# aalobaidi/ggRMCP

Measured on NVIDIA H100. Metric: tools_call_transcodes_per_sec, higher is better.
Workload: dtype u8

## Files before the change

__graft_entry__.py:

```python
import os
import subprocess
import sys

ROOT = os.path.dirname(os.path.abspath(__file__))
for p in (ROOT, os.path.join(ROOT, "tests")):
    if p not in sys.path:
        sys.path.insert(0, p)


def build():
    from ggrmcp_b200 import build as gbuild
    gbuild.build()
    subprocess.check_call(["make", "-s", "-C", os.path.join(ROOT, "oracle")])
    import benchgen
    benchgen.build()
    subprocess.check_call(["make", "-s", "-C", os.path.join(ROOT, "tests", "hostsim")])
    import ggrmcp_b200


def smoke():
    import numpy as np
    import cases
    import orc
    import ggrmcp_b200
    from ggrmcp_b200.engine import pack, unpack
    import benchgen

    fds = open(os.path.join(ROOT, "tests", "golden", "schemas.binpb"), "rb").read()
    eng = ggrmcp_b200.Engine(0)
    sch = eng.register(fds)
    O = orc.Schema(fds)
    ids = np.array([sch.message(n) for n, _, _ in cases.K_REQUESTS], np.int32)
    data, off = pack([j for _, j, _ in cases.K_REQUESTS])
    out, ooff, st = eng.encode_batch(sch, ids, data, off)
    assert list(st) == [0] * len(ids), st
    assert [o.hex() for o in unpack(out, ooff)] == [w for _, _, w in cases.K_REQUESTS]
    ids = np.array([sch.message(n) for n, _, _ in cases.K_REPLIES], np.int32)
    data, off = pack([bytes.fromhex(w) for _, w, _ in cases.K_REPLIES])
    out, ooff, st = eng.decode_batch(sch, ids, data, off)
    assert list(st) == [0] * len(ids), st
    assert unpack(out, ooff) == [j for _, _, j in cases.K_REPLIES]
    wl = benchgen.nested(512, sch.message)
    wire, woff, st = eng.encode_batch(sch, wl.req_msg, wl.req_json, wl.req_off)
    js, joff, st2 = eng.decode_batch(sch, wl.rep_msg, wl.rep_wire, wl.rep_off)
    assert (st == 0).all() and (st2 == 0).all()
    names = {sch.message(n): O.msg(n) for n in ("com.example.complex.ProcessNodeRequest", "com.example.complex.CreateDocumentRequest",
                                                 "com.example.complex.Node", "com.example.complex.GetUserProfileResponse")}
    ow, owoff, _ = O.encode_batch(np.array([names[int(i)] for i in wl.req_msg], np.int32), wl.req_json, wl.req_off)
    oj, ojoff, _ = O.decode_batch(np.array([names[int(i)] for i in wl.rep_msg], np.int32), wl.rep_wire, wl.rep_off)
    assert wire.tobytes() == ow.tobytes() and (woff == owoff).all()
    assert js.tobytes() == oj.tobytes() and (joff == ojoff).all()
    print("smoke ok: %d kernel launches, %d + %d items bit-exact vs oracle" % (eng.launch_count(), len(cases.K_REQUESTS) + len(cases.K_REPLIES), 2 * wl.n))
    eng.close()


if __name__ == "__main__":
    build()
    if "--smoke" in sys.argv:
        smoke()
```

ggrmcp_b200/csrc/ggr_engine.cu:

```cuda
#include <cuda_runtime.h>
#include <sched.h>

#include <cstdio>
#include <cstdlib>
#include <cstring>
#include <atomic>
#include <chrono>
#include <mutex>
#include <string>
#include <vector>

#include "../../include/ggrmcp_b200.h"
#include "ggr_kernels.h"
#include "ggr_schema.h"
#include "ggr_tables.h"

typedef uint8_t u8;
typedef uint32_t u32;
typedef uint64_t u64;
typedef int32_t i32;
#define GGR_BLOCK 128

__global__ void __launch_bounds__(1024) k_scan_blocks(u64* __restrict__ sums, long long nb, u64* __restrict__ total_out) {
  __shared__ u64 part[1024];
// ... 305 lines not shown
  int n = 0;
  for (int c : e->node_cpus)
    if (c < CPU_SETSIZE && CPU_ISSET(c, &old)) {
      CPU_SET(c, &want);
      n++;
    }
  if (n) sched_setaffinity(0, sizeof want, &want);
  return GGR_SUCCESS;
}
int ggr_host_alloc(ggr_engine* e, size_t bytes, void** out) {
  if (!e || !out) return GGR_ERR_INVALID_ARGUMENT;
  *out = nullptr;
  DeviceGuard dg(e->device);
  NodeBind nb(e);
  void* p = nullptr;
  if (!cuda_ok(e, cudaHostAlloc(&p, bytes ? bytes : 1, cudaHostAllocDefault), "cudaHostAlloc")) return GGR_ERR_CUDA;
  for (size_t o = 0; o < bytes; o += 4096) ((volatile char*)p)[o] = 0;
  *out = p;
  return GGR_SUCCESS;
}
void ggr_host_free(ggr_engine* e, void* p) {
  if (!e || !p) return;
  DeviceGuard dg(e->device);
  cudaFreeHost(p);
}

const char* ggr_status_string(int32_t st) {
  static const char* names[] = {"ok", "syntax", "unknown_field", "invalid_value", "range", "invalid_utf8", "duplicate",
                                "oneof_conflict", "depth", "too_large", "bad_wire", "unsupported", "no_space", "internal"};
  if (st < 0 || st > 13) return "?";
  return names[st];
}

int ggr_engine_create(const ggr_config* cfg, ggr_engine** out) {
  if (!out) return GGR_ERR_INVALID_ARGUMENT;
  *out = nullptr;
  int ndev = 0;
  if (cudaGetDeviceCount(&ndev) != cudaSuccess || ndev == 0) return GGR_ERR_NO_DEVICE;
  int dev = cfg ? cfg->device : 0;
  if (dev < 0 || dev >= ndev) return GGR_ERR_INVALID_ARGUMENT;
  if (cudaSetDevice(dev) != cudaSuccess) return GGR_ERR_NO_DEVICE;
  cudaFuncAttributes fa;
  if (cudaFuncGetAttributes(&fa, ggr_kernel_encode_parse()) != cudaSuccess) {
    cudaGetLastError();
    return GGR_ERR_NO_DEVICE;
  }
  ggr_engine* e = new ggr_engine();
  e->device = dev;
  cudaDeviceGetAttribute(&e->sm_count, cudaDevAttrMultiProcessorCount, dev);
  if (e->sm_count <= 0) e->sm_count = 132;
  find_numa(e);
  if (const char* nc = getenv("GGR_COOP")) e->use_coop = nc[0] != '0';
  if (const char* nc = getenv("GGR_COOP_ENC")) e->use_coop_enc = nc[0] != '0';
  if (const char* nc = getenv("GGR_WALK")) e->use_walk = nc[0] != '0';
  if (const char* pz = getenv("GGR_POISON")) e->poison = pz[0] == '1';
  if (const char* nc = getenv("GGR_TRACE")) e->trace = nc[0] != '0';
  if (const char* nc = getenv("GGR_LOCKSTEP_MIN_BYTES")) e->min_json = e->min_wire = (uint32_t)strtoul(nc, nullptr, 10);
  if (const char* nc = getenv("GGR_SPREAD_MIN_BYTES")) e->spread_min = (uint32_t)strtoul(nc, nullptr, 10);
  if (const char* nc = getenv("GGR_SLOTS")) {
    int v = atoi(nc);
    if (v >= 1 && v <= GGR_MAX_SLOTS) e->n_slots = v;
  }
  if (const char* nc = getenv("GGR_CHUNK_ITEMS")) {
    long long v = atoll(nc);
    if (v >= 128) e->chunk_items = v;
  }
  if (const char* nc = getenv("GGR_CHUNK_RAMP")) e->chunk_ramp = nc[0] != '0';
  e->blocking_sync = usable_cpus() < 4 * ndev;
  if (const char* nc = getenv("GGR_BLOCKING_SYNC")) e->blocking_sync = nc[0] != '0';
  if (const char* nc = getenv("GGR_CHUNK_BYTES")) {
    long long v = atoll(nc);
    if (v >= (1 << 16)) e->chunk_bytes = (uint64_t)v;
  }
  e->order = (cfg && cfg->wire_order == GGR_ORDER_GO_LEGACY) ? ggr::ORDER_GO_LEGACY : ggr::ORDER_FIELD_NUMBER;
  e->short_names = cfg && cfg->tool_naming == GGR_NAMES_DESCRIPTOR_SET;
  if (ggr_encode_coop_init() != 0 || ggr_encode_walk_init() != 0 || ggr_decode_coop_init() != 0) {
    cudaGetLastError();
    delete e;
    return GGR_ERR_CUDA;
  }
  if (cudaStreamCreateWithFlags(&e->stream, cudaStreamNonBlocking) != cudaSuccess) {
    delete e;
    return GGR_ERR_CUDA;
  }
  {
    size_t want = 4096 + (size_t)(ggr_decode_max_rec() + 1) * 4096, cur = 0;
    if (const char* ev = getenv("GGR_STACK_BYTES")) want = (size_t)strtoull(ev, nullptr, 10);
    cudaDeviceGetLimit(&cur, cudaLimitStackSize);
    if (cur < want) {
      cudaError_t rc = cudaDeviceSetLimit(cudaLimitStackSize, want);
      if (rc != cudaSuccess) {
        e->err = std::string("cudaDeviceSetLimit(stack): ") + cudaGetErrorString(rc);
        cudaStreamDestroy(e->stream);
        delete e;
        return GGR_ERR_CUDA;
      }
    }
    if (getenv("GGR_DEBUG")) {
      size_t now = 0;
      cudaDeviceGetLimit(&now, cudaLimitStackSize);
      fprintf(stderr, "[ggr] stack limit was %zu, wanted %zu, now %zu\n", cur, want, now);
    }
  }
  *out = e;
  return GGR_SUCCESS;
}

void ggr_engine_destroy(ggr_engine* e) {
  if (!e) return;
  cudaSetDevice(e->device);
  cudaStreamSynchronize(e->stream);
  auto free_scratch = [](Scratch& sc) {
    DevBuf* bufs[] = {&sc.ir, &sc.size, &sc.aux, &sc.sums, &sc.pend, &sc.ioff, &sc.nn, &sc.wtext, &sc.woff, &sc.wsize, &sc.sortpool, &sc.spread, &sc.tabpool, &sc.taboff};
    for (DevBuf* b : bufs)
      if (b->p) cudaFree(b->p);
  };
  free_scratch(e->dev_sc[0]);
  free_scratch(e->dev_sc[1]);

  for (int i = 0; i < 2 * GGR_MAX_SLOTS; i++) {
    Slot& sl = e->slots[i / GGR_MAX_SLOTS][i % GGR_MAX_SLOTS];
    if (sl.st) cudaStreamSynchronize(sl.st);
    free_scratch(sl.sc);
    DevBuf* bufs[] = {&sl.d_in, &sl.d_off, &sl.d_msg, &sl.d_out, &sl.d_out_off, &sl.d_status, &sl.d_ids, &sl.d_ids_off};
    for (DevBuf* b : bufs)
      if (b->p) cudaFree(b->p);
    if (sl.h_total) cudaFreeHost(sl.h_total);
    if (sl.ready) cudaEventDestroy(sl.ready);
    if (sl.ev_in) cudaEventDestroy(sl.ev_in);
    if (sl.ev_k) cudaEventDestroy(sl.ev_k);
    if (sl.ev_out) cudaEventDestroy(sl.ev_out);
    if (sl.st) cudaStreamDestroy(sl.st);
  }
  for (int d = 0; d < 2; d++) {
    if (e->s_in[d]) cudaStreamDestroy(e->s_in[d]);
    if (e->s_out[d]) cudaStreamDestroy(e->s_out[d]);
  }
  for (cudaEvent_t ev : e->ev_pool) cudaEventDestroy(ev);
  cudaStreamDestroy(e->stream);
  delete e;
}

const char* ggr_last_error(const ggr_engine* e) { return e ? e->err.c_str() : "null engine"; }
uint64_t ggr_launch_count(const ggr_engine* e) { return e ? e->launches.load() : 0; }

int ggr_schema_register(ggr_engine* e, const uint8_t* fds, size_t n, ggr_schema** out) {
  if (!e || !fds || !out) return GGR_ERR_INVALID_ARGUMENT;
  *out = nullptr;
  ggr_schema* s = new ggr_schema();
  s->eng = e;
  s->d_blob = nullptr;
  std::string err;
  if (!ggr::compile_schema(fds, n, e->order, &s->cs, &err, e->short_names)) {
    e->err = err;
    delete s;
    return GGR_ERR_SCHEMA;
  }
  cudaSetDevice(e->device);
  if (!cuda_ok(e, cudaMalloc((void**)&s->d_blob, s->cs.blob.size() + 256), "cudaMalloc(schema)") ||
      !cuda_ok(e, cudaMemset(s->d_blob, 0, s->cs.blob.size() + 256), "cudaMemset(schema)") ||
      !cuda_ok(e, cudaMemcpy(s->d_blob, s->cs.blob.data(), s->cs.blob.size(), cudaMemcpyHostToDevice), "cudaMemcpy(schema)")) {
    if (s->d_blob) cudaFree(s->d_blob);
    delete s;
    return GGR_ERR_CUDA;
  }
  *out = s;
  return GGR_SUCCESS;
}
void ggr_schema_release(ggr_schema* s) {
  if (!s) return;
  cudaSetDevice(s->eng->device);
  cudaStreamSynchronize(s->eng->stream);
  cudaFree(s->d_blob);
  delete s;
}
int32_t ggr_message_lookup(const ggr_schema* s, const char* full_name) {
  if (!s || !full_name) return -1;
  auto it = s->cs.msg_index.find(full_name);
  return it == s->cs.msg_index.end() ? -1 : it->second;
}
int32_t ggr_method_count(const ggr_schema* s) { return s ? (int32_t)s->cs.methods.size() : 0; }
int ggr_method_get(const ggr_schema* s, int32_t i, ggr_method_info* o) {
  if (!s || !o || i < 0 || i >= (int32_t)s->cs.methods.size()) return GGR_ERR_INVALID_ARGUMENT;
  const ggr::MethodInfo& m = s->cs.methods[i];
  o->name = m.name.c_str();
  o->full_name = m.full_name.c_str();
  o->service_name = m.service_name.c_str();
  o->tool_name = m.tool_name.c_str();
  o->grpc_path = m.grpc_path.c_str();
  o->input_msg = m.input_msg;
  o->output_msg = m.output_msg;
  o->client_streaming = m.client_streaming;
  o->server_streaming = m.server_streaming;
  return GGR_SUCCESS;
}
int32_t ggr_tool_lookup(const ggr_schema* s, const char* tool) {
  if (!s || !tool) return -1;
  auto it = s->cs.tool_index.find(tool);
  return it == s->cs.tool_index.end() ? -1 : it->second;
}

int ggr_profile_enable(ggr_engine* e, int on) {
  if (!e) return GGR_ERR_INVALID_ARGUMENT;
  std::lock_guard<std::mutex> g(e->mu);
  e->profiling = on != 0;
  return GGR_SUCCESS;
}
int ggr_profile_read(ggr_engine* e, double* ms, uint64_t* launches) {
  if (!e || !ms || !launches) return GGR_ERR_INVALID_ARGUMENT;
  std::lock_guard<std::mutex> g(e->mu);
  cudaSetDevice(e->device);
  cudaDeviceSynchronize();
  for (int i = 0; i < GGR_PROFILE_SLOTS; i++) { ms[i] = 0; launches[i] = 0; }
  for (auto& sp : e->spans) {
    float t = 0;
    if (cudaEventElapsedTime(&t, e->ev_pool[sp.a], e->ev_pool[sp.b]) == cudaSuccess) {
      ms[sp.slot] += t;
      launches[sp.slot]++;
    }
  }
  e->spans.clear();
  e->ev_used = 0;
  return GGR_SUCCESS;
}

int ggr_debug_paths(ggr_engine* e, int64_t n, uint32_t* reply_mode, uint32_t* request_counts) {
  if (!e) return GGR_ERR_INVALID_ARGUMENT;
  DeviceGuard dg(e->device);
  cudaDeviceSynchronize();
  if (reply_mode && e->dev_sc[1].aux.p && e->dev_sc[1].aux.cap >= (size_t)n * 4)
    cudaMemcpy(reply_mode, e->dev_sc[1].aux.p, (size_t)n * 4, cudaMemcpyDeviceToHost);
  if (request_counts && e->dev_sc[0].pend.p) {
    uint32_t c[16];
    cudaMemcpy(c, e->dev_sc[0].pend.p, sizeof c, cudaMemcpyDeviceToHost);
    request_counts[0] = c[0];
    request_counts[1] = c[4];
    request_counts[2] = c[8];
  }
  return GGR_SUCCESS;
}

int ggr_synchronize(ggr_engine* e) {
  if (!e) return GGR_ERR_INVALID_ARGUMENT;
  cudaSetDevice(e->device);
  return cuda_ok(e, cudaStreamSynchronize(e->stream), "cudaStreamSynchronize") ? GGR_SUCCESS : GGR_ERR_CUDA;
}

static int run_dev_kernels(ggr_engine* e, const ggr_schema* s, Scratch& sc, bool encode, int64_t n, const int32_t* msg_id, const uint8_t* in,
                           const uint64_t* in_off, uint64_t in_bytes, uint8_t* out, uint64_t out_cap, uint64_t* out_off,
                           int32_t* status, uint32_t flags, cudaStream_t st);
static int run_dev(ggr_engine* e, const ggr_schema* s, Scratch& sc, bool encode, int64_t n, const int32_t* msg_id, const uint8_t* in,
                   const uint64_t* in_off, uint64_t in_bytes, uint8_t* out, uint64_t out_cap, uint64_t* out_off,
                   int32_t* status, uint32_t flags, cudaStream_t st) {
  const int rc = run_dev_kernels(e, s, sc, encode, n, msg_id, in, in_off, in_bytes, out, out_cap, out_off, status, flags, st);
  if (e && e->poison) {
    DevBuf* bufs[] = {&sc.ir, &sc.size, &sc.aux, &sc.sums, &sc.pend, &sc.ioff, &sc.nn};
    for (DevBuf* b : bufs) {
      const size_t n16 = b->cap / 16;
      if (b->p && n16) k_poison<<<(unsigned)((n16 + 255) / 256), 256, 0, st>>>((uint4*)b->p, n16);
    }
  }
  return rc;
}
static int run_dev_kernels(ggr_engine* e, const ggr_schema* s, Scratch& sc, bool encode, int64_t n, const int32_t* msg_id, const uint8_t* in,
                           const uint64_t* in_off, uint64_t in_bytes, uint8_t* out, uint64_t out_cap, uint64_t* out_off,
                           int32_t* status, uint32_t flags, cudaStream_t st) {
  if (!e || !s || n < 0 || (n > 0 && (!msg_id || !in || !in_off || !out_off || !status))) return GGR_ERR_INVALID_ARGUMENT;
  if (((uintptr_t)in & 15) || ((uintptr_t)out & 7)) return GGR_ERR_INVALID_ARGUMENT;
  DeviceGuard dg(e->device);
  if (n == 0) {
    return cuda_ok(e, cudaMemsetAsync(out_off, 0, sizeof(uint64_t), st), "memset") ? GGR_SUCCESS : GGR_ERR_CUDA;
  }
  long long nb = (n + GGR_BLOCK - 1) / GGR_BLOCK;
  if (!ensure(e, sc.size, (size_t)n * 4) || !ensure(e, sc.aux, (size_t)n * 4) || !ensure(e, sc.sums, (size_t)nb * 8)) return GGR_ERR_CUDA;
  if (encode && !ensure(e, sc.ir, (size_t)in_bytes * 8 + (size_t)n * 128 + 256)) return GGR_ERR_CUDA;
  u32 n_msgs = (u32)s->cs.msg_names.size();
  const bool prof = e->profiling && e->ev_used + 16 <= 65536;
  const u32 frame = (encode && (flags & GGR_F_GRPC_FRAME)) ? 5u : 0u;
  size_t m0 = 0, m1 = 0, m2 = 0, m3 = 0, mx = 0;
  bool have_mx = false;
  if (prof) prof_mark(e, st, &m0);
  if (encode) {
    if (e->use_coop_enc) {
      if (!ensure(e, sc.pend, (size_t)n * 20 + 128) || !ensure(e, sc.ioff, (size_t)in_bytes * 2 + (size_t)n * 32 + 64) ||
          !ensure(e, sc.nn, (size_t)n * 4))
        return GGR_ERR_CUDA;
      u32* counters = (u32*)sc.pend.p;
      u32* big = counters + 32;
      u32* pend1 = big + n;
      u32* pend2 = pend1 + n;
      u32* pend1b = pend2 + n;
      u32* pend1c = pend1b + n;
      size_t c0 = 0, c1 = 0;
      if (!cuda_ok(e, cudaMemsetAsync(counters, 0, 128, st), "memset") ||
          !cuda_ok(e, cudaMemsetAsync(sc.nn.p, 0, (size_t)n * 4, st), "memset"))
        return GGR_ERR_CUDA;
      if (prof) prof_mark(e, st, &m0);
      k_route<<<(unsigned)((n + 255) / 256), 256, 0, st>>>(n, in_off, e->min_json, 65000u - 16u, big, counters, pend2, counters + 8, nullptr);
      size_t t1 = 0, t_tok = 0;
      if (e->use_walk) {
        ggr_launch_encode_tok2(st, n, in, in_off, (u8*)sc.ir.p, big, counters, e->sm_count);
        if (prof) prof_mark(e, st, &t1);
        t_tok = t1;
        ggr_launch_encode_place(st, n, in_off, (u8*)sc.ir.p, big, counters, e->sm_count);
        size_t t2 = 0, t3 = 0;
        if (prof) prof_mark(e, st, &t2);
        ggr_launch_encode_type(st, 0, n, s->d_blob, n_msgs, msg_id, in, in_off, (u8*)sc.ir.p, (u32*)sc.size.p, (u32*)sc.aux.p, status,
                               (u32*)sc.ioff.p, (u32*)sc.nn.p, big, counters, pend1b, counters + 12, e->sm_count);
        ggr_launch_encode_type(st, 1, n, s->d_blob, n_msgs, msg_id, in, in_off, (u8*)sc.ir.p, (u32*)sc.size.p, (u32*)sc.aux.p, status,
                               (u32*)sc.ioff.p, (u32*)sc.nn.p, pend1b, counters + 12, pend1c, counters + 16, e->sm_count);
        ggr_launch_encode_type(st, 2, n, s->d_blob, n_msgs, msg_id, in, in_off, (u8*)sc.ir.p, (u32*)sc.size.p, (u32*)sc.aux.p, status,
                               (u32*)sc.ioff.p, (u32*)sc.nn.p, pend1c, counters + 16, pend1, counters + 4, e->sm_count);
        if (prof) {
          prof_mark(e, st, &t3);
          e->spans.push_back({12, t1, t2});
          e->spans.push_back({13, t2, t3});
          t1 = t3;
        }
      } else {
        ggr_launch_encode_coop_tok(st, n, in, in_off, (u8*)sc.ir.p, big, counters, e->sm_count);
        if (prof) prof_mark(e, st, &t1);
        t_tok = t1;
        ggr_launch_encode_coop_parse(st, 0, n, s->d_blob, n_msgs, msg_id, in, in_off, (u8*)sc.ir.p, (u32*)sc.size.p,
                                     (u32*)sc.aux.p, status, (u32*)sc.ioff.p, (u32*)sc.nn.p, big, counters, pend1, counters + 4, e->sm_count, nullptr, nullptr, -1);
      }
      ggr_launch_encode_coop_parse(st, 1, n, s->d_blob, n_msgs, msg_id, in, in_off, (u8*)sc.ir.p, (u32*)sc.size.p,
                                   (u32*)sc.aux.p, status, (u32*)sc.ioff.p, (u32*)sc.nn.p, pend1, counters + 4, pend2, counters + 8, e->sm_count, nullptr, nullptr, -1);
      if (prof) prof_mark(e, st, &c0);
      if (e->spread_min) {
        size_t max_big = (size_t)(in_bytes / e->spread_min) + 1;
        if (max_big > GGR_SPREAD_CAP) max_big = GGR_SPREAD_CAP;
        if (!ensure(e, sc.spread, (max_big * 32 + (size_t)n) * 4 + 64)) return GGR_ERR_CUDA;
        u32* sp_cnt = (u32*)sc.spread.p;
        u32* sp_list = sp_cnt + 16;
        u32* sp_small = sp_list + max_big * 32;
        if (!cuda_ok(e, cudaMemsetAsync(sp_cnt, 0, 64, st), "memset") || !cuda_ok(e, cudaMemsetAsync(sp_list, 0xFF, max_big * 32 * 4, st), "memset"))
          return GGR_ERR_CUDA;
        for (int phase = 0; phase < 2; phase++)
          k_spread<<<(unsigned)((n + 255) / 256), 256, 0, st>>>(phase, n, in_off, e->spread_min, pend2, counters + 8, nullptr, sp_small, sp_list, sp_cnt, (u32)max_big);
        ggr_launch_encode_parse(st, (unsigned)((max_big * 32 + GGR_BLOCK - 1) / GGR_BLOCK), s->d_blob, n, n_msgs, msg_id, in, in_off, (u8*)sc.ir.p,
                                (u32*)sc.size.p, (u32*)sc.aux.p, status, (u64*)sc.sums.p, sp_list, sp_cnt);
        ggr_launch_encode_parse(st, (unsigned)nb, s->d_blob, n, n_msgs, msg_id, in, in_off, (u8*)sc.ir.p, (u32*)sc.size.p,
                                (u32*)sc.aux.p, status, (u64*)sc.sums.p, sp_small, sp_cnt + 1);
        e->launches += 3;
      } else {
        ggr_launch_encode_parse(st, (unsigned)nb, s->d_blob, n, n_msgs, msg_id, in, in_off, (u8*)sc.ir.p, (u32*)sc.size.p,
                                (u32*)sc.aux.p, status, (u64*)sc.sums.p, pend2, counters + 8);
      }
      if (prof) prof_mark(e, st, &c1);
      if (frame) ggr_launch_frame_sizes(st, n, (u32*)sc.size.p, status);
      ggr_launch_block_sums(st, (unsigned)nb, n, (const u32*)sc.size.p, (u64*)sc.sums.p);
      if (prof) {
        e->spans.push_back({11, m0, t_tok});
        e->spans.push_back({8, t1, c0});
        e->spans.push_back({0, c0, c1});
        prof_mark(e, st, &m1);
        e->spans.push_back({9, c1, m1});
      }
      e->launches += e->use_walk ? 8 : 5;
    } else {
      ggr_launch_encode_parse(st, (unsigned)nb, s->d_blob, n, n_msgs, msg_id, in, in_off, (u8*)sc.ir.p, (u32*)sc.size.p,
                              (u32*)sc.aux.p, status, (u64*)sc.sums.p, nullptr, nullptr);
      if (frame) {
        ggr_launch_frame_sizes(st, n, (u32*)sc.size.p, status);
        ggr_launch_block_sums(st, (unsigned)nb, n, (const u32*)sc.size.p, (u64*)sc.sums.p);
      }
      if (prof) prof_mark(e, st, &m1);
    }
    k_scan_blocks<<<1, 1024, 0, st>>>((u64*)sc.sums.p, nb, out_off + n);
    if (prof) prof_mark(e, st, &m2);
    ggr_launch_encode_emit(st, (unsigned)nb, n, in, in_off, (const u8*)sc.ir.p, (const u32*)sc.size.p,
                           (const u32*)sc.aux.p, status, (const u64*)sc.sums.p, out, out_cap, out_off,
                           e->use_coop_enc ? (const u32*)sc.nn.p : nullptr, frame);
    if (e->use_coop_enc) {
      size_t x1 = 0;
      if (prof) {
        prof_mark(e, st, &mx);
        have_mx = true;
      }
      ggr_launch_encode_coop_emit(st, n, in, in_off, (const u8*)sc.ir.p, (const u32*)sc.ioff.p, (const u32*)sc.nn.p,
                                  (const u32*)sc.size.p, status, out, out_off, e->sm_count, (const u32*)sc.pend.p + 32,
                                  (const u32*)sc.pend.p, frame);
      if (prof) {
        prof_mark(e, st, &x1);
        e->spans.push_back({10, mx, x1});
      }
      e->launches += 1;
    }
  } else {
    const bool coop = e->use_coop;
    size_t c0 = 0, c1 = 0;
    const uint64_t want_recs = in_bytes / 4 * 3 + 1024;
    const uint32_t sort_cap = (uint32_t)(want_recs > 0x3FFFFFFFull ? 0x3FFFFFFFull : want_recs);
    if (!ensure(e, sc.sortpool, (size_t)sort_cap * 16 + 16)) return GGR_ERR_CUDA;
    if (!cuda_ok(e, cudaMemsetAsync(sc.sortpool.p, 0, 16, st), "memset")) return GGR_ERR_CUDA;
    if (coop) {
      const uint64_t want_ent = in_bytes / 2 + 4096;
      const uint32_t pool_cap = (uint32_t)(want_ent > (4ull << 20) ? (4ull << 20) : want_ent);
      if (!ensure(e, sc.ir, ggr_decode_coop_table_bytes(n)) || !ensure(e, sc.nn, (size_t)n * 4) ||
          !ensure(e, sc.pend, (size_t)n * 8 + 64) || !ensure(e, sc.tabpool, (size_t)pool_cap * 32 + 32) || !ensure(e, sc.taboff, (size_t)n * 4))
        return GGR_ERR_CUDA;
      u32* counters = (u32*)sc.pend.p;
      u32* big = counters + 16;
      if (!cuda_ok(e, cudaMemsetAsync(counters, 0, 64, st), "memset") || !cuda_ok(e, cudaMemsetAsync(sc.tabpool.p, 0, 32, st), "memset")) return GGR_ERR_CUDA;
      k_route<<<(unsigned)((n + 255) / 256), 256, 0, st>>>(n, in_off, e->min_wire, 0x3FFFFF00u, big, counters, nullptr, nullptr, (u32*)sc.aux.p);
      ggr_launch_decode_coop_size(st, n, s->d_blob, n_msgs, msg_id, in, in_off, flags, (u32*)sc.size.p, (u32*)sc.aux.p, status,
                                  sc.ir.p, (u32*)sc.nn.p, e->sm_count, big, counters, big + n, counters + 4, sc.tabpool.p, pool_cap, (u32*)sc.taboff.p);
      if (prof) {
        prof_mark(e, st, &c0);
        e->spans.push_back({6, m0, c0});
        m0 = c0;
      }
    }
    const bool spread = coop && e->spread_min != 0;
    size_t max_big = spread ? (size_t)(in_bytes / e->spread_min) + 1 : 0;
    if (max_big > GGR_SPREAD_CAP) max_big = GGR_SPREAD_CAP;
    u32* sp_cnt = nullptr;
    if (spread) {
      if (!ensure(e, sc.spread, max_big * 32 * 4 + 64)) return GGR_ERR_CUDA;
      sp_cnt = (u32*)sc.spread.p;
      if (!cuda_ok(e, cudaMemsetAsync(sp_cnt, 0, 64, st), "memset") || !cuda_ok(e, cudaMemsetAsync(sp_cnt + 16, 0xFF, max_big * 32 * 4, st), "memset"))
        return GGR_ERR_CUDA;
      for (int phase = 0; phase < 2; phase++)
        k_spread<<<(unsigned)((n + 255) / 256), 256, 0, st>>>(phase, n, in_off, e->spread_min, nullptr, nullptr, (const u32*)sc.aux.p, nullptr, sp_cnt + 16, sp_cnt, (u32)max_big);
      ggr_launch_decode_size(st, (unsigned)((max_big * 32 + GGR_BLOCK - 1) / GGR_BLOCK), s->d_blob, n, n_msgs, msg_id, in, in_off, flags,
                             (u32*)sc.size.p, (u32*)sc.aux.p, status, (u64*)sc.sums.p, 1, sc.sortpool.p, sort_cap, sp_cnt + 16, sp_cnt);
      e->launches += 4;
    }
    ggr_launch_decode_size(st, (unsigned)nb, s->d_blob, n, n_msgs, msg_id, in, in_off, flags, (u32*)sc.size.p,
                           (u32*)sc.aux.p, status, (u64*)sc.sums.p, coop ? 1 : 0, sc.sortpool.p, sort_cap);
    if (prof) prof_mark(e, st, &m1);
    k_scan_blocks<<<1, 1024, 0, st>>>((u64*)sc.sums.p, nb, out_off + n);
    if (prof) prof_mark(e, st, &m2);
    ggr_launch_decode_write(st, (unsigned)nb, s->d_blob, n, msg_id, in, in_off, flags, (const u32*)sc.size.p,
                            (const u32*)sc.aux.p, status, (const u64*)sc.sums.p, out, out_cap, out_off, sc.sortpool.p, sort_cap);
    if (spread)
      ggr_launch_decode_write(st, (unsigned)((max_big * 32 + GGR_BLOCK - 1) / GGR_BLOCK), s->d_blob, n, msg_id, in, in_off, flags,
                              (const u32*)sc.size.p, (const u32*)sc.aux.p, status, (const u64*)sc.sums.p, out, out_cap, out_off, sc.sortpool.p,
                              sort_cap, sp_cnt + 16, sp_cnt);
    if (coop) {
      if (prof) prof_mark(e, st, &c1);
      ggr_launch_decode_coop_write(st, n, s->d_blob, in, in_off, flags, (const u32*)sc.size.p, (const u32*)sc.aux.p, status, sc.ir.p,
                                   (const u32*)sc.nn.p, out, out_off, e->sm_count, (const u32*)sc.pend.p + 16, (const u32*)sc.pend.p, sc.tabpool.p,
                                   (const u32*)sc.taboff.p);
      if (prof) {
        prof_mark(e, st, &m3);
        e->spans.push_back({3, m0, m1});
        e->spans.push_back({4, m1, m2});
        e->spans.push_back({5, m2, c1});
        e->spans.push_back({7, c1, m3});
      }
      e->launches += 7;
      return cuda_ok(e, cudaGetLastError(), "kernel launch") ? GGR_SUCCESS : GGR_ERR_CUDA;
    }
  }
  if (prof) {
    prof_mark(e, st, &m3);
    int base = encode ? 0 : 3;
    if (!(encode && e->use_coop_enc)) e->spans.push_back({base + 0, m0, m1});
    e->spans.push_back({base + 1, m1, m2});
    e->spans.push_back({base + 2, m2, have_mx ? mx : m3});
  }
  e->launches += 3;
  return cuda_ok(e, cudaGetLastError(), "kernel launch") ? GGR_SUCCESS : GGR_ERR_CUDA;
}

int ggr_encode_diagnose(ggr_engine* e, const ggr_schema* s, int32_t msg_id, const uint8_t* json, uint64_t json_len, uint32_t flags,
                        int32_t* status, uint32_t* err_pos, uint32_t* err_len, char* text, size_t text_cap) {
  (void)flags;
  if (!e || !s || (!json && json_len) || !status) return GGR_ERR_INVALID_ARGUMENT;
  if (json_len > 0x1FFFF0ull) return GGR_ERR_TOO_LARGE;
  std::lock_guard<std::mutex> g(e->mu);
  DeviceGuard dg(e->device);
  const size_t in_cap = ((size_t)json_len + 15) / 16 * 16 + 64;
  const size_t ir_bytes = (size_t)json_len * 8 + 128 + 256;
  const size_t o_off = in_cap, o_msg = o_off + 16, o_res = o_msg + 16, o_sums = o_res + 16, o_ir = o_sums + 16;
  uint8_t* d = nullptr;
  if (!cuda_ok(e, cudaMalloc((void**)&d, o_ir + ir_bytes), "cudaMalloc(diagnose)")) return GGR_ERR_CUDA;
  std::vector<uint8_t> h(o_ir, 0);
  if (json_len) memcpy(h.data(), json, (size_t)json_len);
  const uint64_t offs[2] = {0, json_len};
  memcpy(h.data() + o_off, offs, 16);
  memcpy(h.data() + o_msg, &msg_id, 4);
  cudaStream_t st = e->stream;
  int rc = GGR_SUCCESS;
  uint32_t res[4] = {0, 0, 0, 0};
  if (!cuda_ok(e, cudaMemcpyAsync(d, h.data(), o_ir, cudaMemcpyHostToDevice, st), "H2D(diagnose)")) rc = GGR_ERR_CUDA;
  if (rc == GGR_SUCCESS) {
    ggr_launch_encode_parse(st, 1, s->d_blob, 1, (u32)s->cs.msg_names.size(), (const int32_t*)(d + o_msg), d, (const uint64_t*)(d + o_off), d + o_ir,
                            (u32*)(d + o_res), (u32*)(d + o_res + 4), (int32_t*)(d + o_res + 8), (uint64_t*)(d + o_sums), nullptr, nullptr,
                            (u32*)(d + o_res + 12));
    e->launches += 1;
    if (!cuda_ok(e, cudaGetLastError(), "kernel launch") ||
        !cuda_ok(e, cudaMemcpyAsync(res, d + o_res, 16, cudaMemcpyDeviceToHost, st), "D2H(diagnose)") ||
        !cuda_ok(e, cudaStreamSynchronize(st), "sync(diagnose)"))
      rc = GGR_ERR_CUDA;
  }
  cudaFree(d);
  if (rc != GGR_SUCCESS) return rc;
  const int32_t stt = (int32_t)res[2];
  *status = stt;
  uint32_t pos = stt != GGR_ST_OK ? res[3] : 0, len = 0;
  if (pos > json_len) pos = (uint32_t)json_len;
  if (stt != GGR_ST_OK && pos < json_len && json[pos] == '"') {
    uint64_t q = pos + 1;
    while (q < json_len && json[q] != '"') q += json[q] == '\\' ? 2 : 1;
    if (q < json_len) len = (uint32_t)(q + 1 - pos);
  }
  if (err_pos) *err_pos = pos;
  if (err_len) *err_len = len;
  if (text && text_cap) {
    std::string t;
    if (stt == GGR_ST_OK) {
      t = "";
    } else {
      uint32_t line = 1, col = 1;
      for (uint32_t k = 0; k < pos; k++) {
        if (json[k] == '\n') { line++; col = 1; }
        else col++;
      }
      t = "proto: (line " + std::to_string(line) + ":" + std::to_string(col) + "): ";
      const std::string tok = len ? std::string((const char*)json + pos, len) : std::string();
      if (stt == GGR_ST_UNKNOWN_FIELD && len) t += "unknown field " + tok;
      else if (stt == GGR_ST_DUPLICATE && len) t += "duplicate field " + tok;
      else if (stt == GGR_ST_ONEOF && len) t += "error parsing " + tok + ", oneof is already set";
      else t += ggr_status_string(stt);
    }
    const size_t k = t.size() < text_cap - 1 ? t.size() : text_cap - 1;
    memcpy(text, t.data(), k);
    text[k] = 0;
  }
  return GGR_SUCCESS;
}

int ggr_encode_batch_dev(ggr_engine* e, const ggr_schema* s, int64_t n, const int32_t* msg_id, const uint8_t* in,
                         const uint64_t* in_off, uint64_t in_bytes, uint8_t* out, uint64_t out_cap, uint64_t* out_off,
                         int32_t* status, uint32_t flags, void* stream) {
  if (!e) return GGR_ERR_INVALID_ARGUMENT;
  std::lock_guard<std::mutex> g(e->mu);
  return run_dev(e, s, e->dev_sc[0], true, n, msg_id, in, in_off, in_bytes, out, out_cap, out_off, status, flags,
                 stream ? (cudaStream_t)stream : e->stream);
}
int ggr_decode_batch_dev(ggr_engine* e, const ggr_schema* s, int64_t n, const int32_t* msg_id, const uint8_t* in,
                         const uint64_t* in_off, uint64_t in_bytes, uint8_t* out, uint64_t out_cap, uint64_t* out_off,
                         int32_t* status, uint32_t flags, void* stream) {
  if (!e) return GGR_ERR_INVALID_ARGUMENT;
  std::lock_guard<std::mutex> g(e->mu);
  return run_dev(e, s, e->dev_sc[1], false, n, msg_id, in, in_off, in_bytes, out, out_cap, out_off, status, flags,
                 stream ? (cudaStream_t)stream : e->stream);
}

static int run_request_dev(ggr_engine* e, const ggr_schema* s, Scratch& sc, int64_t n, const uint8_t* in, const uint64_t* in_off,
                           uint64_t in_bytes, uint8_t* out, uint64_t out_cap, uint64_t* out_off, int32_t* method, uint32_t* id_span,
                           int32_t* status, cudaStream_t st) {
  if (!e || !s || n < 0 || (n > 0 && (!in || !in_off || !out_off || !status || !method || !id_span))) return GGR_ERR_INVALID_ARGUMENT;
  if (((uintptr_t)in & 15) || ((uintptr_t)out & 7)) return GGR_ERR_INVALID_ARGUMENT;
  DeviceGuard dg(e->device);
  if (n == 0) return cuda_ok(e, cudaMemsetAsync(out_off, 0, sizeof(uint64_t), st), "memset") ? GGR_SUCCESS : GGR_ERR_CUDA;
  const long long nb = (n + GGR_BLOCK - 1) / GGR_BLOCK;
  if (!ensure(e, sc.size, (size_t)n * 4) || !ensure(e, sc.aux, (size_t)n * 4) || !ensure(e, sc.sums, (size_t)nb * 8) ||
      !ensure(e, sc.ir, (size_t)in_bytes * 8 + (size_t)n * 128 + 256) || !ensure(e, sc.pend, (size_t)n * 12 + 64) ||
      !ensure(e, sc.ioff, (size_t)in_bytes * 2 + (size_t)n * 32 + 64) || !ensure(e, sc.nn, (size_t)n * 4))
    return GGR_ERR_CUDA;
  u32* counters = (u32*)sc.pend.p;
  u32* big = counters + 16;
  u32* pend1 = big + n;
  u32* rest = pend1 + n;
  if (!cuda_ok(e, cudaMemsetAsync(counters, 0, 64, st), "memset") || !cuda_ok(e, cudaMemsetAsync(sc.nn.p, 0, (size_t)n * 4, st), "memset"))
    return GGR_ERR_CUDA;
  const u32 n_msgs = (u32)s->cs.msg_names.size();
  k_route<<<(unsigned)((n + 255) / 256), 256, 0, st>>>(n, in_off, 0u, 65000u - 16u, big, counters, rest, counters + 8, nullptr);
  ggr_launch_encode_coop_tok(st, n, in, in_off, (u8*)sc.ir.p, big, counters, e->sm_count);
  ggr_launch_encode_coop_parse(st, 0, n, s->d_blob, n_msgs, nullptr, in, in_off, (u8*)sc.ir.p, (u32*)sc.size.p, (u32*)sc.aux.p, status,
                               (u32*)sc.ioff.p, (u32*)sc.nn.p, big, counters, pend1, counters + 4, e->sm_count, method, id_span, -1);
  ggr_launch_encode_coop_parse(st, 1, n, s->d_blob, n_msgs, nullptr, in, in_off, (u8*)sc.ir.p, (u32*)sc.size.p, (u32*)sc.aux.p, status,
                               (u32*)sc.ioff.p, (u32*)sc.nn.p, pend1, counters + 4, rest, counters + 8, e->sm_count, method, id_span,
                               GGR_ST_UNSUPPORTED);
  k_mark<<<(unsigned)((n + 255) / 256), 256, 0, st>>>(rest, counters + 8, status, (u32*)sc.size.p, (u32*)sc.aux.p, GGR_ST_UNSUPPORTED);
  ggr_launch_block_sums(st, (unsigned)nb, n, (const u32*)sc.size.p, (u64*)sc.sums.p);
  k_scan_blocks<<<1, 1024, 0, st>>>((u64*)sc.sums.p, nb, out_off + n);
  ggr_launch_encode_emit(st, (unsigned)nb, n, in, in_off, (const u8*)sc.ir.p, (const u32*)sc.size.p, (const u32*)sc.aux.p, status,
                         (const u64*)sc.sums.p, out, out_cap, out_off, (const u32*)sc.nn.p, 0);
  ggr_launch_encode_coop_emit(st, n, in, in_off, (const u8*)sc.ir.p, (const u32*)sc.ioff.p, (const u32*)sc.nn.p, (const u32*)sc.size.p,
                              status, out, out_off, e->sm_count, big, counters, 0);
  e->launches += 9;
  return cuda_ok(e, cudaGetLastError(), "kernel launch") ? GGR_SUCCESS : GGR_ERR_CUDA;
}

static int run_wrap_dev(ggr_engine* e, const ggr_schema* s, Scratch& sc, int64_t n, const int32_t* msg_id, const uint8_t* in,
                        const uint64_t* in_off, uint64_t in_bytes, const uint8_t* ids, const uint64_t* ids_off, uint8_t* out,
                        uint64_t out_cap, uint64_t* out_off, int32_t* status, uint32_t flags, cudaStream_t st) {
  if (n > 0 && (!ids || !ids_off)) return GGR_ERR_INVALID_ARGUMENT;
  if (n == 0) return run_dev(e, s, sc, false, n, msg_id, in, in_off, in_bytes, out, out_cap, out_off, status, flags, st);
  if (!ensure(e, sc.wtext, (size_t)out_cap + 64) || !ensure(e, sc.woff, (size_t)(n + 1) * 8) || !ensure(e, sc.wsize, (size_t)n * 4))
    return GGR_ERR_CUDA;
  int rc = run_dev(e, s, sc, false, n, msg_id, in, in_off, in_bytes, (uint8_t*)sc.wtext.p, out_cap, (uint64_t*)sc.woff.p, status, flags, st);
  if (rc != GGR_SUCCESS) return rc;
  const long long nb = (n + GGR_BLOCK - 1) / GGR_BLOCK;
  ggr_launch_wrap_size(st, n, (const uint8_t*)sc.wtext.p, (const uint64_t*)sc.woff.p, status, ids_off, (u32*)sc.wsize.p, e->sm_count);
  ggr_launch_block_sums(st, (unsigned)nb, n, (const u32*)sc.wsize.p, (u64*)sc.sums.p);
  k_scan_blocks<<<1, 1024, 0, st>>>((u64*)sc.sums.p, nb, out_off + n);
  ggr_launch_offsets(st, (unsigned)nb, n, (const u32*)sc.wsize.p, (const u64*)sc.sums.p, out_off);
  ggr_launch_wrap_write(st, n, (const uint8_t*)sc.wtext.p, (const uint64_t*)sc.woff.p, status, ids, ids_off, (const u32*)sc.wsize.p, out,
                        out_cap, out_off, e->sm_count);
  e->launches += 5;
  return cuda_ok(e, cudaGetLastError(), "kernel launch") ? GGR_SUCCESS : GGR_ERR_CUDA;
}
// ... 323 lines not shown
```

ggrmcp_b200/csrc/ggr_kernels.h:

```cpp
#pragma once
#include <cuda_runtime.h>
#include <stdint.h>

void ggr_launch_encode_parse(cudaStream_t st, unsigned nb, const uint8_t* blob, long long n, uint32_t n_msgs, const int32_t* msg_id,
                             const uint8_t* in, const uint64_t* in_off, uint8_t* ir, uint32_t* size, uint32_t* first,
                             int32_t* status, uint64_t* block_sums, const uint32_t* list, const uint32_t* list_n,
                             uint32_t* err_pos = nullptr);
void ggr_launch_block_sums(cudaStream_t st, unsigned nb, long long n, const uint32_t* size, uint64_t* block_sums);
void ggr_launch_encode_coop_tok(cudaStream_t st, long long n, const uint8_t* in, const uint64_t* in_off, uint8_t* ir,
                                const uint32_t* list, const uint32_t* list_n, int sm_count);
void ggr_launch_encode_coop_parse(cudaStream_t st, int tier, long long n, const uint8_t* blob, uint32_t n_msgs,
                                  const int32_t* msg_id, const uint8_t* in, const uint64_t* in_off, uint8_t* ir, uint32_t* size,
                                  uint32_t* first, int32_t* status, uint32_t* ioff, uint32_t* nnodes, const uint32_t* list,
                                  const uint32_t* list_n, uint32_t* pending, uint32_t* n_pending, int sm_count, int32_t* method,
                                  uint32_t* id_span, int32_t final_status);
void ggr_launch_encode_coop_emit(cudaStream_t st, long long n, const uint8_t* in, const uint64_t* in_off, const uint8_t* ir,
                                 const uint32_t* ioff, const uint32_t* nnodes, const uint32_t* size, const int32_t* status,
                                 uint8_t* out, const uint64_t* out_off, int sm_count, const uint32_t* list,
                                 const uint32_t* list_n, uint32_t frame);
void ggr_launch_encode_tok2(cudaStream_t st, long long n, const uint8_t* in, const uint64_t* in_off, uint8_t* ir, const uint32_t* list,
                            const uint32_t* list_n, int sm_count);
void ggr_launch_encode_place(cudaStream_t st, long long n, const uint64_t* in_off, uint8_t* ir, const uint32_t* list, const uint32_t* list_n,
                             int sm_count);
void ggr_launch_encode_type(cudaStream_t st, int tier, long long n, const uint8_t* blob, uint32_t n_msgs, const int32_t* msg_id, const uint8_t* in,
                            const uint64_t* in_off, uint8_t* ir, uint32_t* size, uint32_t* first, int32_t* status, uint32_t* ioff,
                            uint32_t* nnodes, const uint32_t* list, const uint32_t* list_n, uint32_t* pending, uint32_t* n_pending,
                            int sm_count);
int ggr_encode_walk_init();
int ggr_encode_coop_init();
void ggr_launch_encode_emit(cudaStream_t st, unsigned nb, long long n, const uint8_t* in, const uint64_t* in_off, const uint8_t* ir,
                            const uint32_t* size, const uint32_t* first, int32_t* status, const uint64_t* block_prefix,
                            uint8_t* out, uint64_t out_cap, uint64_t* out_off, const uint32_t* skip, uint32_t frame);
void ggr_launch_frame_sizes(cudaStream_t st, long long n, uint32_t* size, const int32_t* status);
void ggr_launch_decode_size(cudaStream_t st, unsigned nb, const uint8_t* blob, long long n, uint32_t n_msgs, const int32_t* msg_id,
                            const uint8_t* in, const uint64_t* in_off, uint32_t flags, uint32_t* size, uint32_t* mode,
                            int32_t* status, uint64_t* block_sums, int after_coop, void* sort_pool, uint32_t sort_cap,
                            const uint32_t* list = nullptr, const uint32_t* list_n = nullptr);
void ggr_launch_decode_write(cudaStream_t st, unsigned nb, const uint8_t* blob, long long n, const int32_t* msg_id,
                             const uint8_t* in, const uint64_t* in_off, uint32_t flags, const uint32_t* size,
                             const uint32_t* mode, int32_t* status, const uint64_t* block_prefix, uint8_t* out,
                             uint64_t out_cap, uint64_t* out_off, void* sort_pool, uint32_t sort_cap, const uint32_t* list = nullptr,
                             const uint32_t* list_n = nullptr);
void ggr_launch_decode_coop_size(cudaStream_t st, long long n, const uint8_t* blob, uint32_t n_msgs, const int32_t* msg_id,
                                 const uint8_t* in, const uint64_t* in_off, uint32_t flags, uint32_t* size, uint32_t* mode,
                                 int32_t* status, void* tab, uint32_t* nent, int sm_count, const uint32_t* list,
                                 const uint32_t* list_n, uint32_t* pending, uint32_t* n_pending, void* pool, uint32_t pool_cap,
                                 uint32_t* tab_off);
void ggr_launch_decode_coop_write(cudaStream_t st, long long n, const uint8_t* blob, const uint8_t* in, const uint64_t* in_off,
                                  uint32_t flags, const uint32_t* size, const uint32_t* mode, int32_t* status, const void* tab,
                                  const uint32_t* nent, uint8_t* out, const uint64_t* out_off, int sm_count,
                                  const uint32_t* list, const uint32_t* list_n, const void* pool, const uint32_t* tab_off);
size_t ggr_decode_coop_table_bytes(long long n);
int ggr_decode_coop_init();
void ggr_launch_wrap_size(cudaStream_t st, long long n, const uint8_t* text, const uint64_t* text_off, const int32_t* status,
                          const uint64_t* ids_off, uint32_t* size, int sm_count);
void ggr_launch_offsets(cudaStream_t st, unsigned nb, long long n, const uint32_t* size, const uint64_t* block_prefix,
                        uint64_t* out_off);
void ggr_launch_wrap_write(cudaStream_t st, long long n, const uint8_t* text, const uint64_t* text_off, int32_t* status,
                           const uint8_t* ids, const uint64_t* ids_off, const uint32_t* size, uint8_t* out, uint64_t out_cap,
                           const uint64_t* out_off, int sm_count);
const void* ggr_kernel_encode_parse();
int ggr_decode_max_rec();
```

ggrmcp_b200/csrc/ggr_kernels_walk.cu:

```cuda
#include "ggr_kernels.h"
#include "ggr_walk.cuh"

#define CW_WARPS 4
#define CW_TOK_BLOCKS 8
#define CW_PLACE_BLOCKS 12
#define CW_WALK_BLOCKS 6

__global__ void __launch_bounds__(CW_WARPS * 32, CW_TOK_BLOCKS)
k_encode_tok3(const u8* __restrict__ in, const u64* __restrict__ in_off, u8* __restrict__ ir, const u32* __restrict__ list,
              const u32* __restrict__ list_n) {
  __shared__ CwLut lut;
  __shared__ CwTile tiles[CW_WARPS];
  const u32 warp = threadIdx.x >> 5;
  cw_lut_init(lut, threadIdx.x, CW_WARPS * 32);
  if ((threadIdx.x & 31u) == 0) cw_tile_init(&tiles[warp]);
  __syncthreads();
  u32 ph = 0;
  const long long total = (long long)*list_n;
  const u64 a0 = in_off[0];
  u32* ticket = const_cast<u32*>(list_n) + 1;
  u32 drawn = wp_ticket_draw(ticket);
  for (long long slot = wp_ticket_take(drawn); slot < total; slot = wp_ticket_take(drawn)) {
    drawn = wp_ticket_draw(ticket);
    const long long item = (long long)list[slot];
    const u64 a = in_off[item], b = in_off[item + 1];
    if (b < a || b - a > (u64)CE_MAX_INPUT - 16u) continue;
    const u64 node_off = ((a - a0) >> 1) + 8ull * (u64)item;
    const u32 cap = (u32)((((b - a0) >> 1) + 8ull * (u64)(item + 1)) - node_off);
    const u32 s0 = (u32)(a & 15ull);
    cw_tok_item(&tiles[warp], ph, lut, in + (a & ~15ull), s0, s0 + (u32)(b - a), ir + node_off * 16, cap);
  }
}

__global__ void __launch_bounds__(CW_WARPS * 32, CW_PLACE_BLOCKS)
k_encode_place(const u64* __restrict__ in_off, u8* __restrict__ ir, const u32* __restrict__ list, const u32* __restrict__ list_n) {
  __shared__ CwPlaceSh S[CW_WARPS];
  const u32 warp = threadIdx.x >> 5;
  const long long total = (long long)*list_n;
  const u64 a0 = in_off[0];
  u32* ticket = const_cast<u32*>(list_n) + 3;
  u32 drawn = wp_ticket_draw(ticket);
  for (long long slot = wp_ticket_take(drawn); slot < total; slot = wp_ticket_take(drawn)) {
    drawn = wp_ticket_draw(ticket);
    const long long item = (long long)list[slot];
    const u64 a = in_off[item], b = in_off[item + 1];
    if (b <= a || b - a > (u64)CE_MAX_INPUT - 16u) continue;
    const u64 node_off = ((a - a0) >> 1) + 8ull * (u64)item;
    const u32 cap = (u32)((((b - a0) >> 1) + 8ull * (u64)(item + 1)) - node_off);
    cw_place_item(S[warp], ir + node_off * 16, cap, CoopWalkHuge::MAX_NODE);
  }
}

template <class SH, bool FULL, int WARPS>
__global__ void __launch_bounds__(WARPS * 32, FULL ? 1 : CW_WALK_BLOCKS)
k_encode_type(const u8* __restrict__ blob, u32 n_msgs, const i32* __restrict__ msg_id, const u8* __restrict__ in,
              const u64* __restrict__ in_off, u8* __restrict__ ir, u32* __restrict__ size, u32* __restrict__ first,
              i32* __restrict__ status, u32* __restrict__ ioff, u32* __restrict__ nnodes, const u32* __restrict__ list,
              const u32* __restrict__ list_n, u32* __restrict__ pending, u32* __restrict__ n_pending) {
  extern __shared__ __align__(16) unsigned char smem[];
  SH* S = reinterpret_cast<SH*>(smem);
  const u32 warp = threadIdx.x >> 5, lane = threadIdx.x & 31;
  const long long total = (long long)*list_n;
  const Tables T = ggr_tables(blob);
  const u64 a0 = in_off[0];
  u32* ticket = const_cast<u32*>(list_n) + 2;
  u32 drawn = wp_ticket_draw(ticket);
  long long slot = wp_ticket_take(drawn);
  drawn = wp_ticket_draw(ticket);
  while (slot < total) {
    const long long next = wp_ticket_take(drawn);
    drawn = wp_ticket_draw(ticket);
    const long long item = (long long)list[slot];
    const u64 a = in_off[item], b = in_off[item + 1];
    const i32 m = msg_id[item];
    bool ok = false;
    EncResult res;
    res.size = 0;
    res.n_nodes = 0;
    res.method = 0;
    if (m >= 0 && (u32)m < n_msgs && b >= a && b - a <= (u64)CE_MAX_INPUT - 16u) {
      const u64 node_off = ((a - a0) >> 1) + 8ull * (u64)item;
      const u32 cap = (u32)((((b - a0) >> 1) + 8ull * (u64)(item + 1)) - node_off);
      const u32 s0 = (u32)(a & 15ull);
      ok = cw_type_item<SH, FULL>(S[warp], T, (u32)m, in + (a & ~15ull), s0, s0 + (u32)(b - a), ir + node_off * 16, ioff + node_off, cap, &res);
    }
    if (lane == 0) {
      if (ok) {
        size[item] = res.size;
        first[item] = GGR_NIL;
        status[item] = GST_OK;
        nnodes[item] = res.n_nodes | (res.method << 16);
      } else {
        size[item] = 0;
        nnodes[item] = 0;
        first[item] = GGR_NIL;
        pending[atomicAdd(n_pending, 1u)] = (u32)item;
      }
    }
    slot = next;
  }
}

int ggr_encode_walk_init() {
  return (cudaFuncSetAttribute(k_encode_type<CoopWalk, false, CW_WARPS>, cudaFuncAttributeMaxDynamicSharedMemorySize, (int)(sizeof(CoopWalk) * CW_WARPS)) == cudaSuccess &&
          cudaFuncSetAttribute(k_encode_type<CoopWalkBig, true, CW_WARPS>, cudaFuncAttributeMaxDynamicSharedMemorySize, (int)(sizeof(CoopWalkBig) * CW_WARPS)) == cudaSuccess &&
          cudaFuncSetAttribute(k_encode_type<CoopWalkHuge, true, 1>, cudaFuncAttributeMaxDynamicSharedMemorySize, (int)sizeof(CoopWalkHuge)) == cudaSuccess)
             ? 0
             : -1;
}

static unsigned cw_grid(const void* fn, int threads, size_t smem, long long n, int sm_count) {
  int per_sm = 0;
  if (cudaOccupancyMaxActiveBlocksPerMultiprocessor(&per_sm, fn, threads, smem) != cudaSuccess || per_sm < 1) per_sm = 1;
  const long long want = (n + CW_WARPS - 1) / CW_WARPS, cap = (long long)sm_count * per_sm;
  return (unsigned)(want < cap ? (want > 0 ? want : 1) : cap);
}

void ggr_launch_encode_tok2(cudaStream_t st, long long n, const uint8_t* in, const uint64_t* in_off, uint8_t* ir, const uint32_t* list,
                            const uint32_t* list_n, int sm_count) {
  static unsigned per_sm = 0;
  if (!per_sm) per_sm = cw_grid((const void*)k_encode_tok3, CW_WARPS * 32, 0, 1ll << 40, 1);
  const long long want = (n + CW_WARPS - 1) / CW_WARPS, cap = (long long)sm_count * per_sm;
  k_encode_tok3<<<(unsigned)(want < cap ? want : cap), CW_WARPS * 32, 0, st>>>(in, (const u64*)in_off, ir, list, list_n);
}

void ggr_launch_encode_place(cudaStream_t st, long long n, const uint64_t* in_off, uint8_t* ir, const uint32_t* list, const uint32_t* list_n,
                             int sm_count) {
  static unsigned per_sm = 0;
  if (!per_sm) per_sm = cw_grid((const void*)k_encode_place, CW_WARPS * 32, 0, 1ll << 40, 1);
  const long long want = (n + CW_WARPS - 1) / CW_WARPS, cap = (long long)sm_count * per_sm;
  k_encode_place<<<(unsigned)(want < cap ? want : cap), CW_WARPS * 32, 0, st>>>((const u64*)in_off, ir, list, list_n);
}

void ggr_launch_encode_type(cudaStream_t st, int tier, long long n, const uint8_t* blob, uint32_t n_msgs, const int32_t* msg_id, const uint8_t* in,
                            const uint64_t* in_off, uint8_t* ir, uint32_t* size, uint32_t* first, int32_t* status, uint32_t* ioff,
                            uint32_t* nnodes, const uint32_t* list, const uint32_t* list_n, uint32_t* pending, uint32_t* n_pending,
                            int sm_count) {
  if (tier == 0) {
    static unsigned per_sm = 0;
    const size_t smem = sizeof(CoopWalk) * CW_WARPS;
    if (!per_sm) per_sm = cw_grid((const void*)k_encode_type<CoopWalk, false, CW_WARPS>, CW_WARPS * 32, smem, 1ll << 40, 1);
    const long long want = (n + CW_WARPS - 1) / CW_WARPS, cap = (long long)sm_count * per_sm;
    k_encode_type<CoopWalk, false, CW_WARPS><<<(unsigned)(want < cap ? want : cap), CW_WARPS * 32, smem, st>>>(
        blob, n_msgs, msg_id, in, (const u64*)in_off, ir, size, first, status, ioff, nnodes, list, list_n, pending, n_pending);
  } else if (tier == 2) {
    k_encode_type<CoopWalkHuge, true, 1><<<(unsigned)sm_count, 32, sizeof(CoopWalkHuge), st>>>(
        blob, n_msgs, msg_id, in, (const u64*)in_off, ir, size, first, status, ioff, nnodes, list, list_n, pending, n_pending);
  } else {
    static unsigned per_sm = 0;
    const size_t smem = sizeof(CoopWalkBig) * CW_WARPS;
    if (!per_sm) per_sm = cw_grid((const void*)k_encode_type<CoopWalkBig, true, CW_WARPS>, CW_WARPS * 32, smem, 1ll << 40, 1);
    k_encode_type<CoopWalkBig, true, CW_WARPS><<<(unsigned)sm_count * per_sm, CW_WARPS * 32, smem, st>>>(
        blob, n_msgs, msg_id, in, (const u64*)in_off, ir, size, first, status, ioff, nnodes, list, list_n, pending, n_pending);
  }
}
```

ggrmcp_b200/csrc/ggr_prim.cuh:

```cuda
#pragma once
#include <stdint.h>
#include <string.h>

#include "ggr_tables.h"

#if defined(__CUDACC__)
#define GGR_DEV __device__ __forceinline__
#define GGR_DEVN static __device__ __noinline__
#else
#define GGR_DEV inline
#define GGR_DEVN inline
#endif

#if defined(__CUDA_ARCH__)
#define GGR_FULL_MASK 0xFFFFFFFFu
__device__ __forceinline__ bool ggr_any(unsigned mask, bool p) { return __any_sync(mask, p) != 0; }
__device__ __forceinline__ unsigned ggr_activemask() { return __activemask(); }
#else
#define GGR_FULL_MASK 1u
inline bool ggr_any(unsigned, bool p) { return p; }
inline unsigned ggr_activemask() { return 1u; }
#endif
#define GGR_STEP_CONT (-1)

typedef uint8_t u8;
typedef uint16_t u16;
typedef uint32_t u32;
typedef uint64_t u64;
typedef int32_t i32;
typedef int64_t i64;

struct U4 {
  u32 x, y, z, w;
};

GGR_DEV U4 ggr_ld16(const u8* p) {
#if defined(__CUDA_ARCH__)
  uint4 v = __ldg(reinterpret_cast<const uint4*>(p));
  U4 r = {v.x, v.y, v.z, v.w};
  return r;
#else
  U4 r;
  memcpy(&r, p, 16);
  return r;
#endif
}
GGR_DEV U4 ggr_ld16_rw(const u8* p) {
#if defined(__CUDA_ARCH__)
  uint4 v = *reinterpret_cast<const uint4*>(p);
  U4 r = {v.x, v.y, v.z, v.w};
  return r;
#else
  U4 r;
  memcpy(&r, p, 16);
  return r;
#endif
}
GGR_DEV void ggr_st16(u8* p, U4 v) {
#if defined(__CUDA_ARCH__)
  *reinterpret_cast<uint4*>(p) = make_uint4(v.x, v.y, v.z, v.w);
#else
  memcpy(p, &v, 16);
#endif
}
GGR_DEV void ggr_st8(u8* p, u64 v) {
#if defined(__CUDA_ARCH__)
  *reinterpret_cast<unsigned long long*>(p) = v;
#else
  memcpy(p, &v, 8);
#endif
}
GGR_DEV u32 ggr_ld4_rw(const u8* p) {
#if defined(__CUDA_ARCH__)
  return *reinterpret_cast<const u32*>(p);
#else
  u32 v;
  memcpy(&v, p, 4);
  return v;
#endif
}
GGR_DEV void ggr_st4(u8* p, u32 v) {
#if defined(__CUDA_ARCH__)
  *reinterpret_cast<u32*>(p) = v;
#else
  memcpy(p, &v, 4);
#endif
}
GGR_DEV u32 ggr_ld4(const u8* p) {
#if defined(__CUDA_ARCH__)
  return __ldg(reinterpret_cast<const u32*>(p));
#else
  u32 v;
  memcpy(&v, p, 4);
  return v;
#endif
}
GGR_DEV u32 ggr_ld2(const u8* p) {
#if defined(__CUDA_ARCH__)
  return __ldg(reinterpret_cast<const u16*>(p));
#else
  u16 v;
  memcpy(&v, p, 2);
  return v;
#endif
}
GGR_DEV int ggr_clz64(u64 v) {
#if defined(__CUDA_ARCH__)
  return __clzll((long long)v);
#else
  return v ? __builtin_clzll(v) : 64;
#endif
}
GGR_DEV int ggr_ctz32(u32 v) {
#if defined(__CUDA_ARCH__)
  return __ffs((int)v) - 1;
#else
  return __builtin_ctz(v);
#endif
}
GGR_DEV u64 ggr_mulhi64(u64 a, u64 b) {
#if defined(__CUDA_ARCH__)
  return __umul64hi(a, b);
#else
  return (u64)(((unsigned __int128)a * b) >> 64);
#endif
}

struct Rd {
  const u8* base;
  u32 pos, end;
  u32 fetch;
  int avail;
  u64 cur;
  U4 ch;
  u32 rw;

  GGR_DEV u32 word() const {
    u32 i = (fetch >> 2) & 3u;
    u32 lo = (i & 1u) ? ch.y : ch.x;
    u32 hi = (i & 1u) ? ch.w : ch.z;
    return (i & 2u) ? hi : lo;
  }
  GGR_DEV void fill() {
    if (avail <= 4) {
      if ((fetch & 15u) == 0) ch = rw ? ggr_ld16_rw(base + fetch) : ggr_ld16(base + fetch);
      u32 w = word();
      fetch += 4;
      cur |= (u64)w << (8 * avail);
      avail += 4;
    }
  }
  GGR_DEV void init(const u8* b, u32 start, u32 e, u32 written_by_me = 0) {
    base = b;
    pos = start;
    end = e;
    rw = written_by_me;
    fetch = start & ~3u;
    ch = rw ? ggr_ld16_rw(base + (start & ~15u)) : ggr_ld16(base + (start & ~15u));
    u32 w = word();
    fetch += 4;
    int drop = (int)(start & 3u);
    cur = (u64)(w >> (8 * drop));
    avail = 4 - drop;
    fill();
  }
  GGR_DEV bool eof() const { return pos >= end; }
  GGR_DEV u32 left() const { return end - pos; }
  GGR_DEV u32 peek() const { return (u32)cur & 0xFFu; }
  GGR_DEV u32 peek4() const { return (u32)cur; }
  GGR_DEV void skip(int k) {
    cur >>= 8 * k;
    avail -= k;
    pos += (u32)k;
    fill();
  }
  GGR_DEV u32 get() const { return eof() ? 0u : peek(); }
};

GGR_DEVN void wr_flush_partial(u8* a, u64 acc, u32 skip) {
  for (u32 i = skip; i < 8; i++) a[i] = (u8)(acc >> (8 * i));
}
struct Wr {
  u8* base;
  u32 pos;
  int n;
  u32 skip;
  u64 acc;

  GGR_DEV void init(u8* b, u32 start) {
    base = b;
    pos = start;
    n = (int)(start & 7u);
    skip = (u32)n;
    acc = 0;
  }
  GGR_DEV void flush_group() {
    u8* a = base + (pos - (u32)n);
    if (skip) {
      wr_flush_partial(a, acc, skip);
      skip = 0;
    } else {
      ggr_st8(a, acc);
    }
  }
  GGR_DEV void put(u32 v, int k) {
    acc |= (u64)v << (8 * n);
    int n2 = n + k;
    if (n2 >= 8) {
      flush_group();
      acc = (n2 > 8) ? (u64)(v >> (8 * (8 - n))) : 0ull;
      n2 -= 8;
    }
    pos += (u32)k;
    n = n2;
  }
  GGR_DEV void put1(u32 b) { put(b & 0xFFu, 1); }
  GGR_DEV void finish() {
    if ((u32)n > skip) {
      u8* a = base + (pos - (u32)n);
      for (u32 i = skip; i < (u32)n; i++) a[i] = (u8)(acc >> (8 * i));
    }
  }
};

struct Cnt {
  u32 pos;
  GGR_DEV void init(u8*, u32 start) { pos = start; }
  GGR_DEV void put(u32, int k) { pos += (u32)k; }
  GGR_DEV void put1(u32) { pos += 1; }
  GGR_DEV void finish() {}
};

template <class W>
GGR_DEV void put_varint(W& w, u64 v) {
  while (v >= 0x80) {
    w.put1((u32)(v & 0x7F) | 0x80u);
    v >>= 7;
  }
  w.put1((u32)v);
}
GGR_DEV u32 varint_size(u64 v) {
  int bits = 64 - ggr_clz64(v | 1);
  return (u32)((bits * 9 + 64) >> 6);
}
template <class W>
GGR_DEV void put_lit(W& w, const char* s, int n) {
  for (int i = 0; i < n; i++) w.put1((u32)(u8)s[i]);
}

struct Tables {
  const u8* msgs;
  const u8* fields;
  const u8* enums;
  const u8* evals;
  const u8* hash;
  const u8* u16s;
  const u8* pool;
  const u8* tools;
};
GGR_DEV Tables ggr_tables(const u8* blob) {
  U4 h0 = ggr_ld16(blob), h1 = ggr_ld16(blob + 16), h2 = ggr_ld16(blob + 32), h3 = ggr_ld16(blob + 48);
  Tables t;
  t.tools = blob + h0.y - 16;
  t.msgs = blob + h0.w;
  t.fields = blob + h1.y;
  t.enums = blob + h1.w;
  t.evals = blob + h2.y;
  t.hash = blob + h2.w;
  t.u16s = blob + h3.y;
  t.pool = blob + h3.w;
  return t;
}
struct MsgD {
  u32 field_first, n_fields, wkt, flags, key_hash_first, key_hash_mask, decl_first, lut_first, lut_n, n_oneofs;
};
GGR_DEV MsgD ggr_msg(const Tables& t, u32 idx) {
  const u8* p = t.msgs + (size_t)idx * 32;
  U4 a = ggr_ld16(p), b = ggr_ld16(p + 16);
  MsgD m;
  m.field_first = a.x;
  m.n_fields = a.y & 0xFFFFu;
  m.wkt = (a.y >> 16) & 0xFFu;
  m.flags = a.y >> 24;
  m.key_hash_first = a.z;
  m.key_hash_mask = a.w;
  m.decl_first = b.x;
  m.lut_first = b.y;
  m.lut_n = b.z;
  m.n_oneofs = b.w;
  return m;
}
struct FieldD {
  u32 number, tag, tag_len, kind, flags, wt, decl_index;
  i32 oneof, child;
  u32 name_off, name_len;
};
GGR_DEV FieldD ggr_field(const Tables& t, u32 idx) {
  const u8* p = t.fields + (size_t)idx * 32;
  U4 a = ggr_ld16(p), b = ggr_ld16(p + 16);
  FieldD f;
  f.number = a.x;
  f.tag = a.y;
  f.tag_len = a.z & 0xFFu;
  f.kind = (a.z >> 8) & 0xFFu;
  f.flags = (a.z >> 16) & 0xFFu;
  f.wt = a.z >> 24;
  f.oneof = (i32)(int16_t)(a.w & 0xFFFFu);
  f.decl_index = a.w >> 16;
  f.child = (i32)b.x;
  f.name_off = b.y;
  f.name_len = b.z & 0xFFFFu;
  return f;
}
GGR_DEV u32 ggr_u16(const Tables& t, u32 idx) { return ggr_ld2(t.u16s + (size_t)idx * 2); }

GGR_DEV u32 ggr_atomic_add_u32(u32* p, u32 v) {
#if defined(__CUDA_ARCH__)
  return atomicAdd(p, v);
#else
  u32 o = *p;
  *p = o + v;
  return o;
#endif
}

GGR_DEV int ggr_frame_check(const u8* in, u64 a, u64 b) {
  if (b - a < 5ull) return GST_BAD_WIRE;
  const u8* p = in + a;
  if (p[0] == 1u) return GST_UNSUPPORTED;
  if (p[0] != 0u) return GST_BAD_WIRE;
  const u64 len = ((u64)p[1] << 24) | ((u64)p[2] << 16) | ((u64)p[3] << 8) | (u64)p[4];
  return len == b - a - 5ull ? GST_OK : GST_BAD_WIRE;
}
GGR_DEV bool ggr_is_ws(u32 c) { return c == ' ' || c == '\n' || c == '\r' || c == '\t'; }
GGR_DEV bool ggr_not_delim(u32 c) {
  return c == '-' || c == '+' || c == '.' || c == '_' || (c - 'a') < 26u || (c - 'A') < 26u || (c - '0') < 10u;
}
```

ggrmcp_b200/csrc/ggr_schema.cc:

```cpp
#include "ggr_schema.h"

#include <algorithm>
#include <cstring>

namespace ggr {

uint32_t key_hash(const uint8_t* p, size_t n) {
  uint32_t h = 0x811C9DC5u;
  for (size_t i = 0; i < n; i += 4) {
    uint32_t w = 0;
    for (size_t j = 0; j < 4 && i + j < n; j++) w |= (uint32_t)p[i + j] << (8 * j);
    h = (h ^ w) * 0x9E3779B1u;
    h ^= h >> 15;
  }
  h ^= (uint32_t)n;
  h *= 0x85EBCA6Bu;
  return h ^ (h >> 13);
}

namespace {

struct Cur {
  const uint8_t* p;
  const uint8_t* e;
  bool ok = true;
  Cur(const uint8_t* b, size_t n) : p(b), e(b + n) {}
  bool more() const { return ok && p < e; }
  uint64_t varint() {
    uint64_t v = 0;
    for (int s = 0; s < 70; s += 7) {
      if (p >= e) { ok = false; return 0; }
      uint8_t c = *p++;
      v |= (uint64_t)(c & 0x7f) << s;
      if (!(c & 0x80)) return v;
    }
    ok = false;
    return 0;
  }
  bool field(uint32_t* num, int* wt, uint64_t* val, const uint8_t** lp, size_t* ln) {
    uint64_t tag = varint();
    if (!ok) return false;
    *num = (uint32_t)(tag >> 3);
    *wt = (int)(tag & 7);
    *val = 0; *lp = nullptr; *ln = 0;
    switch (*wt) {
      case 0: *val = varint(); return ok;
      case 1: if (e - p < 8) return ok = false; memcpy(val, p, 8); p += 8; return true;
      case 5: if (e - p < 4) return ok = false; { uint32_t x; memcpy(&x, p, 4); *val = x; } p += 4; return true;
      case 2: {
        uint64_t l = varint();
        if (!ok || (uint64_t)(e - p) < l) return ok = false;
        *lp = p; *ln = (size_t)l; p += l;
        return true;
      }
      default: return ok = false;
    }
  }
};
#define FOR_FIELDS(cur) \
  uint32_t num; int wt; uint64_t val; const uint8_t* lp; size_t ln; \
  while ((cur).more() && (cur).field(&num, &wt, &val, &lp, &ln))

struct FieldIn {
  std::string name, json_name, type_name;
  int32_t number = 0;
  int label = 1, type = 0;
  int oneof_index = -1;
  bool proto3_optional = false, have_json = false;
  int packed_opt = 0;
  int decl = 0;
  int child = -1;
};
struct MsgIn {
  std::string full_name;
  std::vector<FieldIn> fields;
  int n_oneofs = 0;
  bool map_entry = false, proto3 = true;
};
struct EnumIn {
  std::string full_name;
  std::vector<std::pair<std::string, int32_t>> values;
};
struct MethodIn {
  std::string service, name, in, out;
  bool cs = false, ss = false;
};

struct Parser {
  std::vector<MsgIn> msgs;
  std::vector<EnumIn> enums;
  std::vector<MethodIn> methods;
  bool bad = false;

  static std::string str(const uint8_t* p, size_t n) { return std::string((const char*)p, n); }
  static std::string join(const std::string& scope, const std::string& name) { return scope.empty() ? name : scope + "." + name; }

  void parse_enum(const uint8_t* b, size_t n, const std::string& scope) {
    EnumIn e;
    Cur c(b, n);
    FOR_FIELDS(c) {
      if (num == 1 && wt == 2) e.full_name = join(scope, str(lp, ln));
      else if (num == 2 && wt == 2) {
        Cur v(lp, ln);
        std::string nm; int32_t number = 0;
        { FOR_FIELDS(v) { if (num == 1 && wt == 2) nm = str(lp, ln); else if (num == 2 && wt == 0) number = (int32_t)val; } }
        if (!v.ok) bad = true;
        e.values.push_back({nm, number});
      }
    }
    if (!c.ok) bad = true;
    enums.push_back(e);
  }

  void parse_field(const uint8_t* b, size_t n, FieldIn& f) {
    Cur c(b, n);
    FOR_FIELDS(c) {
      switch (num) {
        case 1: f.name = str(lp, ln); break;
        case 3: f.number = (int32_t)val; break;
        case 4: f.label = (int)val; break;
        case 5: f.type = (int)val; break;
        case 6: f.type_name = str(lp, ln); break;
        case 8: {
          Cur o(lp, ln);
          { FOR_FIELDS(o) { if (num == 2 && wt == 0) f.packed_opt = val ? 1 : 2; } }
          break;
        }
        case 9: f.oneof_index = (int)val; break;
        case 10: f.json_name = str(lp, ln); f.have_json = true; break;
        case 17: f.proto3_optional = val != 0; break;
        default: break;
      }
    }
    if (!c.ok) bad = true;
  }

  void parse_message(const uint8_t* b, size_t n, const std::string& scope, bool proto3) {
    MsgIn m;
    m.proto3 = proto3;
    std::vector<std::pair<const uint8_t*, size_t>> nested, nenums;
    Cur c(b, n);
    std::string simple;
    FOR_FIELDS(c) {
      switch (num) {
        case 1: simple = str(lp, ln); break;
        case 2: {
          FieldIn f;
          parse_field(lp, ln, f);
          f.decl = (int)m.fields.size();
          m.fields.push_back(f);
          break;
        }
        case 3: nested.push_back({lp, ln}); break;
        case 4: nenums.push_back({lp, ln}); break;
        case 7: {
          Cur o(lp, ln);
          { FOR_FIELDS(o) { if (num == 7 && wt == 0) m.map_entry = val != 0; } }
          break;
        }
        case 8: m.n_oneofs++; break;
        default: break;
      }
    }
    if (!c.ok) bad = true;
    m.full_name = join(scope, simple);
    std::string fq = m.full_name;
    msgs.push_back(m);
    for (auto& e : nenums) parse_enum(e.first, e.second, fq);
    for (auto& s : nested) parse_message(s.first, s.second, fq, proto3);
  }

  void parse_file(const uint8_t* b, size_t n) {
    std::string pkg, syntax;
    {
      Cur c(b, n);
      FOR_FIELDS(c) {
        if (num == 2 && wt == 2) pkg = str(lp, ln);
        else if (num == 12 && wt == 2) syntax = str(lp, ln);
      }
      if (!c.ok) bad = true;
    }
    bool proto3 = syntax == "proto3";
    Cur c(b, n);
    FOR_FIELDS(c) {
      if (num == 4 && wt == 2) parse_message(lp, ln, pkg, proto3);
      else if (num == 5 && wt == 2) parse_enum(lp, ln, pkg);
      else if (num == 6 && wt == 2) {
        std::string sname;
        std::vector<std::pair<const uint8_t*, size_t>> ms;
        Cur s(lp, ln);
        { FOR_FIELDS(s) { if (num == 1 && wt == 2) sname = str(lp, ln); else if (num == 2 && wt == 2) ms.push_back({lp, ln}); } }
        for (auto& mm : ms) {
          MethodIn mi;
          mi.service = join(pkg, sname);
          Cur q(mm.first, mm.second);
          FOR_FIELDS(q) {
            if (num == 1 && wt == 2) mi.name = str(lp, ln);
            else if (num == 2 && wt == 2) mi.in = str(lp, ln);
            else if (num == 3 && wt == 2) mi.out = str(lp, ln);
            else if (num == 5 && wt == 0) mi.cs = val != 0;
            else if (num == 6 && wt == 0) mi.ss = val != 0;
          }
          methods.push_back(mi);
        }
      }
    }
  }
};

std::string default_json_name(const std::string& s) {
  std::string o;
  bool up = false;
  for (char ch : s) {
    if (ch == '_') { up = true; continue; }
    if (up && ch >= 'a' && ch <= 'z') ch = (char)(ch - 32);
    up = false;
    o.push_back(ch);
  }
  return o;
}

std::string json_quote(const std::string& s) {
  static const char hex[] = "0123456789abcdef";
  std::string o = "\"";
  for (unsigned char c : s) {
    if (c == '"' || c == '\\') { o.push_back('\\'); o.push_back((char)c); }
    else if (c == '\b') o += "\\b";
    else if (c == '\f') o += "\\f";
    else if (c == '\n') o += "\\n";
    else if (c == '\r') o += "\\r";
    else if (c == '\t') o += "\\t";
    else if (c < 0x20) { o += "\\u00"; o.push_back(hex[c >> 4]); o.push_back(hex[c & 15]); }
    else o.push_back((char)c);
  }
  o.push_back('"');
  return o;
}

int wire_type_for(int kind) {
  switch (kind) {
    case GK_DOUBLE: case GK_FIXED64: case GK_SFIXED64: return 1;
    case GK_FLOAT: case GK_FIXED32: case GK_SFIXED32: return 5;
    case GK_STRING: case GK_BYTES: case GK_MESSAGE: return 2;
    case GK_GROUP: return 3;
    default: return 0;
  }
}
int varint_len(uint64_t v) { int n = 1; while (v >= 0x80) { v >>= 7; n++; } return n; }

struct Blob {
  std::vector<GgrMsg> msgs;
  std::vector<GgrField> fields;
  std::vector<GgrEnum> enums;
  std::vector<GgrEnumValue> evals;
  std::vector<GgrHashEnt> hash;
  std::vector<uint16_t> u16;
  std::string pool;
  uint32_t intern(const std::string& s) {
    uint32_t off = (uint32_t)pool.size();
    pool += s;
    return off;
  }
  uint32_t add_table(const std::vector<std::pair<std::string, int32_t>>& items, uint32_t* mask) {
    uint32_t size = 4;
    while (size < items.size() * 2 + 1) size <<= 1;
    uint32_t first = (uint32_t)hash.size();
    GgrHashEnt empty = {0, 0, 0xFFFFFFFFu, -1, {0, 0, 0, 0}};
    hash.resize(first + size, empty);
    for (auto& it : items) {
      uint32_t h = key_hash((const uint8_t*)it.first.data(), it.first.size());
      uint32_t slot = h & (size - 1);
      while (hash[first + slot].name_len != 0xFFFFFFFFu) slot = (slot + 1) & (size - 1);
      GgrHashEnt& e = hash[first + slot];
      e.hash = h;
      e.name_off = intern(it.first);
      e.name_len = (uint32_t)it.first.size();
      e.value = it.second;
      for (size_t j = 0; j < 16 && j < it.first.size(); j++) e.w[j / 4] |= (uint32_t)(uint8_t)it.first[j] << (8 * (j % 4));
    }
    *mask = size - 1;
    return first;
  }
};

template <class T>
uint32_t append_section(std::vector<uint8_t>& out, const T* p, size_t n_bytes) {
  while (out.size() % 16) out.push_back(0);
  uint32_t off = (uint32_t)out.size();
  out.insert(out.end(), (const uint8_t*)p, (const uint8_t*)p + n_bytes);
  return off;
}

}

bool compile_schema(const uint8_t* fds, size_t n, WireOrder order, CompiledSchema* out, std::string* err, bool short_service_names) {
  Parser P;
  {
    Cur c(fds, n);
    FOR_FIELDS(c) {
      if (num == 1 && wt == 2) P.parse_file(lp, ln);
    }
    if (!c.ok || P.bad) { *err = "malformed FileDescriptorSet"; return false; }
  }
  if (P.msgs.size() > 65535) { *err = "too many message types"; return false; }
  std::map<std::string, int> msg_by, enum_by;
  for (size_t i = 0; i < P.msgs.size(); i++) msg_by[P.msgs[i].full_name] = (int)i;
  for (size_t i = 0; i < P.enums.size(); i++) enum_by[P.enums[i].full_name] = (int)i;
  auto strip = [](const std::string& s) { return (!s.empty() && s[0] == '.') ? s.substr(1) : s; };

  Blob B;
  for (auto& e : P.enums) {
    GgrEnum ge;
    std::vector<std::pair<int32_t, std::string>> by_num;
    for (auto& v : e.values) {
      bool seen = false;
      for (auto& x : by_num) if (x.first == v.second) seen = true;
      if (!seen) by_num.push_back({v.second, v.first});
    }
    std::stable_sort(by_num.begin(), by_num.end(), [](const std::pair<int32_t, std::string>& a, const std::pair<int32_t, std::string>& b) { return a.first < b.first; });
    ge.val_first = (uint32_t)B.evals.size();
    ge.n_vals = (uint32_t)by_num.size();
    for (auto& x : by_num) {
      GgrEnumValue ev = {x.first, B.intern(x.second), (uint32_t)x.second.size(), 0};
      B.evals.push_back(ev);
    }
    std::vector<std::pair<std::string, int32_t>> items;
    for (auto& v : e.values) {
      bool dup = false;
      for (auto& it : items) if (it.first == v.first) dup = true;
      if (!dup) items.push_back({v.first, v.second});
    }
    ge.hash_first = B.add_table(items, &ge.hash_mask);
    B.enums.push_back(ge);
  }
  out->max_msg_fields = 0;
  for (size_t mi = 0; mi < P.msgs.size(); mi++) {
    MsgIn& m = P.msgs[mi];
    if (m.fields.size() > 4096) { *err = "message " + m.full_name + " has too many fields"; return false; }
    for (auto& f : m.fields) {
      if (f.type == GK_MESSAGE || f.type == GK_GROUP) {
        auto it = msg_by.find(strip(f.type_name));
        if (it == msg_by.end()) { *err = "unresolved type " + f.type_name; return false; }
        f.child = it->second;
      } else if (f.type == GK_ENUM) {
        auto it = enum_by.find(strip(f.type_name));
        if (it == enum_by.end()) { *err = "unresolved enum " + f.type_name; return false; }
        f.child = it->second;
      }
      if (!f.have_json) f.json_name = default_json_name(f.name);
    }
  }
  for (size_t mi = 0; mi < P.msgs.size(); mi++) {
    MsgIn& m = P.msgs[mi];
    GgrMsg gm;
    memset(&gm, 0, sizeof gm);
    std::vector<int> emit(m.fields.size());
    for (size_t i = 0; i < emit.size(); i++) emit[i] = (int)i;
    auto real_oneof = [&](const FieldIn& f) { return f.oneof_index >= 0 && !f.proto3_optional; };
    if (order == ORDER_GO_LEGACY) {
      std::stable_sort(emit.begin(), emit.end(), [&](int a, int b) {
        const FieldIn& x = m.fields[a]; const FieldIn& y = m.fields[b];
        bool ox = real_oneof(x), oy = real_oneof(y);
        if (ox != oy) return !ox && oy;
        if (ox && oy && x.oneof_index != y.oneof_index) return x.oneof_index < y.oneof_index;
        return x.number < y.number;
      });
    } else {
      std::stable_sort(emit.begin(), emit.end(), [&](int a, int b) { return m.fields[a].number < m.fields[b].number; });
    }
    gm.field_first = (uint32_t)B.fields.size();
    gm.n_fields = (uint16_t)m.fields.size();
    gm.n_oneofs = (uint32_t)m.n_oneofs;
    if (m.map_entry) gm.flags |= GM_MAP_ENTRY;
    if (m.full_name == "google.protobuf.Timestamp") gm.wkt = GGR_WKT_TIMESTAMP;
    else if (m.full_name == "google.protobuf.Duration") gm.wkt = GGR_WKT_DURATION;
    else if (m.full_name == "google.protobuf.Empty") gm.wkt = GGR_WKT_EMPTY;
    else if (m.full_name == "google.protobuf.FieldMask" && m.fields.size() == 1 && m.fields[0].number == 1) gm.wkt = GGR_WKT_FIELDMASK;
    else if (m.full_name.rfind("google.protobuf.", 0) == 0) {
      static const char* wr[] = {"DoubleValue", "FloatValue", "Int64Value", "UInt64Value", "Int32Value", "UInt32Value", "BoolValue",
                                 "StringValue", "BytesValue"};
      for (const char* w : wr)
        if (m.full_name == std::string("google.protobuf.") + w && m.fields.size() == 1 && m.fields[0].number == 1) gm.wkt = GGR_WKT_WRAPPER;
      static const char* wk[] = {"Any", "Struct", "Value", "ListValue"};
      for (const char* w : wk) if (m.full_name == std::string("google.protobuf.") + w) gm.wkt = GGR_WKT_UNSUPPORTED;
    }
    bool decl_is_emit = true;
    std::vector<uint16_t> decl_perm(m.fields.size());
    uint32_t max_num = 0;
    for (size_t ei = 0; ei < emit.size(); ei++) {
      const FieldIn& f = m.fields[emit[ei]];
      if ((size_t)f.decl != ei) decl_is_emit = false;
      decl_perm[f.decl] = (uint16_t)ei;
      GgrField gf;
      memset(&gf, 0, sizeof gf);
      gf.number = (uint32_t)f.number;
      gf.kind = (uint8_t)f.type;
      gf.wt = (uint8_t)wire_type_for(f.type);
      bool repeated = f.label == 3;
      bool is_map = repeated && f.type == GK_MESSAGE && P.msgs[f.child].map_entry;
      bool packable = repeated && f.type != GK_STRING && f.type != GK_BYTES && f.type != GK_MESSAGE && f.type != GK_GROUP;
      bool packed = packable && (m.proto3 ? f.packed_opt != 2 : f.packed_opt == 1);
      if (repeated) gf.flags |= GF_REPEATED;
      if (is_map) gf.flags |= GF_MAP;
      if (packable) gf.flags |= GF_PACKABLE;
      if (packed) gf.flags |= GF_PACKED;
      if (!repeated) {
        if (f.type == GK_MESSAGE || f.type == GK_GROUP || f.oneof_index >= 0 || !m.proto3) gf.flags |= GF_PRESENCE;
      }
      gf.tag = ((uint32_t)f.number << 3) | (uint32_t)(packed ? 2 : gf.wt);
      gf.tag_len = (uint8_t)varint_len(gf.tag);
      gf.oneof = real_oneof(f) ? (int16_t)f.oneof_index : (int16_t)-1;
      gf.decl_index = (uint16_t)f.decl;
      gf.child = f.child;
      std::string key = json_quote(f.json_name) + ":";
      gf.name_off = B.intern(key);
      gf.name_len = (uint16_t)key.size();
      B.fields.push_back(gf);
      if ((uint32_t)f.number > max_num) max_num = (uint32_t)f.number;
    }
    if (decl_is_emit) gm.flags |= GM_DECL_IS_EMIT;
    gm.decl_first = (uint32_t)B.u16.size();
    B.u16.insert(B.u16.end(), decl_perm.begin(), decl_perm.end());
    uint32_t lut_n = max_num + 1 > 1024 ? 1024 : max_num + 1;
    gm.lut_first = (uint32_t)B.u16.size();
    gm.lut_n = lut_n;
    B.u16.resize(B.u16.size() + lut_n, 0);
    for (size_t ei = 0; ei < emit.size(); ei++) {
      const FieldIn& f = m.fields[emit[ei]];
      if ((uint32_t)f.number < lut_n && B.u16[gm.lut_first + f.number] == 0) B.u16[gm.lut_first + f.number] = (uint16_t)(ei + 1);
    }
    std::map<std::string, int> by_json, by_text;
    for (auto& f : m.fields) {
      if (!by_json.count(f.json_name)) by_json[f.json_name] = f.decl;
      if (!by_text.count(f.name)) by_text[f.name] = f.decl;
    }
    std::vector<std::pair<std::string, int32_t>> items;
    for (auto& kv : by_json) items.push_back({kv.first, (int32_t)decl_perm[kv.second]});
    for (auto& kv : by_text) if (!by_json.count(kv.first)) items.push_back({kv.first, (int32_t)decl_perm[kv.second]});
    gm.key_hash_first = B.add_table(items, &gm.key_hash_mask);
    B.msgs.push_back(gm);
    if (m.fields.size() > out->max_msg_fields) out->max_msg_fields = (uint32_t)m.fields.size();
    out->msg_index[m.full_name] = (int32_t)mi;
    out->msg_names.push_back(m.full_name);
  }
  for (auto& mi : P.methods) {
    MethodInfo M;
    M.name = mi.name;
    M.service_name = mi.service;
    if (short_service_names) {
      size_t d2 = mi.service.rfind('.');
      if (d2 != std::string::npos && d2 > 0) {
        size_t d1 = mi.service.rfind('.', d2 - 1);
        if (d1 != std::string::npos) M.service_name = mi.service.substr(d1 + 1);
      }
    }
    M.full_name = mi.service + "." + mi.name;
    M.input_type = mi.in;
    M.output_type = mi.out;
    auto a = msg_by.find(strip(mi.in));
    auto b = msg_by.find(strip(mi.out));
    if (a == msg_by.end() || b == msg_by.end()) { *err = "unresolved method type in " + M.full_name; return false; }
    M.input_msg = a->second;
    M.output_msg = b->second;
    M.client_streaming = mi.cs;
    M.server_streaming = mi.ss;
    std::string t = M.service_name;
    for (auto& ch : t) { if (ch == '.') ch = '_'; else if (ch >= 'A' && ch <= 'Z') ch = (char)(ch + 32); }
    std::string mn = mi.name;
    for (auto& ch : mn) if (ch >= 'A' && ch <= 'Z') ch = (char)(ch + 32);
    M.tool_name = t + "_" + mn;
    M.grpc_path = "/" + mi.service + "/" + mi.name;
    out->tool_index[M.tool_name] = (int32_t)out->methods.size();
    out->methods.push_back(M);
  }
  uint32_t tool_hash_first = 0, tool_hash_mask = 0, tool_methods_first = 0;
  {
    std::vector<std::pair<std::string, int32_t>> items;
    for (size_t m = 0; m < out->methods.size(); m++) items.push_back({out->methods[m].tool_name, (int32_t)m});
    tool_hash_first = B.add_table(items, &tool_hash_mask);
    tool_methods_first = (uint32_t)B.u16.size();
    for (auto& M : out->methods)
      B.u16.push_back((M.client_streaming || M.server_streaming || M.input_msg >= 0xFFFF) ? (uint16_t)0xFFFF : (uint16_t)M.input_msg);
  }
  GgrSchemaHdr h;
  memset(&h, 0, sizeof h);
  std::vector<uint8_t>& o = out->blob;
  o.clear();
  o.resize(sizeof h, 0);
  h.magic = GGR_SCHEMA_MAGIC;
  h.n_msgs = (uint32_t)B.msgs.size();
  h.msgs_off = append_section(o, B.msgs.data(), B.msgs.size() * sizeof(GgrMsg));
  h.n_fields = (uint32_t)B.fields.size();
  h.fields_off = append_section(o, B.fields.data(), B.fields.size() * sizeof(GgrField));
  h.n_enums = (uint32_t)B.enums.size();
  h.enums_off = append_section(o, B.enums.data(), B.enums.size() * sizeof(GgrEnum));
  h.n_evals = (uint32_t)B.evals.size();
  h.evals_off = append_section(o, B.evals.data(), B.evals.size() * sizeof(GgrEnumValue));
  h.n_hash = (uint32_t)B.hash.size();
  h.hash_off = append_section(o, B.hash.data(), B.hash.size() * sizeof(GgrHashEnt));
  h.n_u16 = (uint32_t)B.u16.size();
  h.u16_off = append_section(o, B.u16.data(), B.u16.size() * sizeof(uint16_t));
  B.pool.append(32, '\0');
  h.pool_bytes = (uint32_t)B.pool.size();
  h.pool_off = append_section(o, B.pool.data(), B.pool.size());
  while (o.size() % 16) o.push_back(0);
  {
    GgrToolsTrailer tt = {tool_hash_first, tool_hash_mask, tool_methods_first, (uint32_t)out->methods.size()};
    append_section(o, &tt, sizeof tt);
  }
  h.total_bytes = (uint32_t)o.size();
  memcpy(o.data(), &h, sizeof h);
  return true;
}

}
```

ggrmcp_b200/csrc/ggr_tables.h:

```cpp
#pragma once
#include <stdint.h>

#define GGR_SCHEMA_MAGIC 0x47475231u

enum {
  GK_DOUBLE = 1, GK_FLOAT = 2, GK_INT64 = 3, GK_UINT64 = 4, GK_INT32 = 5, GK_FIXED64 = 6,
  GK_FIXED32 = 7, GK_BOOL = 8, GK_STRING = 9, GK_GROUP = 10, GK_MESSAGE = 11, GK_BYTES = 12,
  GK_UINT32 = 13, GK_ENUM = 14, GK_SFIXED32 = 15, GK_SFIXED64 = 16, GK_SINT32 = 17, GK_SINT64 = 18
};

enum { GGR_WKT_NONE = 0, GGR_WKT_TIMESTAMP = 1, GGR_WKT_DURATION = 2, GGR_WKT_WRAPPER = 3, GGR_WKT_EMPTY = 4, GGR_WKT_FIELDMASK = 5, GGR_WKT_UNSUPPORTED = 99 };

#define GF_REPEATED 0x01u
#define GF_PACKED 0x02u
#define GF_MAP 0x04u
#define GF_PRESENCE 0x08u
#define GF_PACKABLE 0x10u

#define GM_MAP_ENTRY 0x01u
#define GM_DECL_IS_EMIT 0x02u

struct GgrSchemaHdr {
  uint32_t magic;
  uint32_t total_bytes;
  uint32_t n_msgs, msgs_off;
  uint32_t n_fields, fields_off;
  uint32_t n_enums, enums_off;
  uint32_t n_evals, evals_off;
  uint32_t n_hash, hash_off;
  uint32_t n_u16, u16_off;
  uint32_t pool_bytes, pool_off;
};

struct GgrToolsTrailer {
  uint32_t hash_first, hash_mask;
  uint32_t methods_first;
  uint32_t n_methods;
};

struct GgrMsg {
  uint32_t field_first;
  uint16_t n_fields;
  uint8_t wkt;
  uint8_t flags;
  uint32_t key_hash_first;
  uint32_t key_hash_mask;
  uint32_t decl_first;
  uint32_t lut_first;
  uint32_t lut_n;
  uint32_t n_oneofs;
};

struct GgrField {
  uint32_t number;
  uint32_t tag;
  uint8_t tag_len;
  uint8_t kind;
  uint8_t flags;
  uint8_t wt;
  int16_t oneof;
  uint16_t decl_index;
  int32_t child;
  uint32_t name_off;
  uint16_t name_len;
  uint16_t pad0;
  uint32_t pad1;
};

struct GgrEnum {
  uint32_t val_first;
  uint32_t n_vals;
  uint32_t hash_first;
  uint32_t hash_mask;
};

struct GgrEnumValue {
  int32_t number;
  uint32_t name_off;
  uint32_t name_len;
  uint32_t pad;
};

struct GgrHashEnt {
  uint32_t hash;
  uint32_t name_off;
  uint32_t name_len;
  int32_t value;
  uint32_t w[4];
};

#define GGR_DF_COMMA_SPACE 0x1u
#define GGR_DF_GRPC_FRAME 0x2u
#define GGR_FRAME_BYTES 5u

enum {
  GST_OK = 0, GST_SYNTAX = 1, GST_UNKNOWN_FIELD = 2, GST_INVALID_VALUE = 3, GST_RANGE = 4,
  GST_INVALID_UTF8 = 5, GST_DUPLICATE = 6, GST_ONEOF = 7, GST_DEPTH = 8, GST_TOO_LARGE = 9,
  GST_BAD_WIRE = 10, GST_UNSUPPORTED = 11, GST_NO_SPACE = 12,
  GST_INTERNAL = 13
};
```

ggrmcp_b200/csrc/ggr_walk.cuh:

```cuda
#pragma once
#include "ggr_coop_enc.cuh"

#define CW_LEVELS 16
#if defined(__CUDA_ARCH__) || defined(__CUDACC__)
#define CW_WHY(code) ((void)0)
#else
extern int g_cw_why;
#define CW_WHY(code) (g_cw_why = (code))
#endif
#define CW_NONE 0xFFFFu

enum { K3_LBRACE = 1, K3_RBRACE = 2, K3_LBRACK = 3, K3_RBRACK = 4, K3_STR = 5, K3_SCALAR = 6 };
#define K3_POS(t) ((t) & 0xFFFFu)
#define K3_KIND(t) (((t) >> 16) & 7u)
#define K3_C(t) (((t) >> 19) & 1u)
#define K3_V(t) (((t) >> 20) & 1u)
#define K3_Q(t) (((t) >> 21) << 1)
#define K3_MAX_STR 2047u

struct CwIndex {
  const u32* tok;
  const u8* qend;
  u32 n_tok, n_q;
};
GGR_DEV u32 cw_tok_cap(u32 cap) { return cap >= 4u ? (cap * 8u - 16u) / 4u : 0u; }
GGR_DEV u32 cw_q_cap(u32 cap) { return cap < 2u * K3_MAX_STR ? cap : 2u * K3_MAX_STR; }
GGR_DEV u32 cw_ldg(const u32* p) {
#if defined(__CUDA_ARCH__)
  return __ldg(p);
#else
  return *p;
#endif
}
struct CwQ {
  u32 pos, esc, slow;
};
GGR_DEV CwQ cw_q(const CwIndex& X, u32 k) {
  const u32* p = reinterpret_cast<const u32*>(X.qend - 8u * (k + 1u));
  const u32 a = cw_ldg(p), b = cw_ldg(p + 1);
  CwQ q = {a & 0xFFFFu, a >> 16, b};
  return q;
}
GGR_DEV u32 cw_key_pack(const CwIndex& X, u32 i) {
  const u32 kt = cw_ldg(X.tok + i - 1u);
  const CwQ q0 = cw_q(X, K3_Q(kt)), q1 = cw_q(X, K3_Q(kt) + 1u);
  const u32 kp = K3_POS(kt), len = (q1.pos - kp - 1u) & 0xFFFFu;
  const bool plain = K3_KIND(kt) == K3_STR && q0.slow == q1.slow && q0.esc == q1.esc && len < 0x8000u;
  return plain ? (((kp + 1u) & 0xFFFFu) | (len << 16) | 0x80000000u) : 0u;
}
GGR_DEV u32 cw_rec_off(u32 n_tok) { return (16u + 4u * n_tok + 15u) & ~15u; }

#define CW_LO 0x00000001u
#define CW_LC 0x00000100u
#define CW_LY 0x00010000u
#define CW_LN 0x01000000u
struct CwLut {
  CeLut base;
  u32 cls2[256];
};
GGR_DEV void cw_lut_init(CwLut& L, u32 first, u32 step) {
  ce_lut_init(L.base, first, step);
  for (u32 b = first; b < 256; b += step) {
    u32 c = 0;
    if (b == '{' || b == '[') c |= CW_LO;
    if (b == '}' || b == ']') c |= CW_LC;
    if (b == '{' || b == '}') c |= CW_LY;
    if (b == ':') c |= CW_LN;
    L.cls2[b] = c;
  }
}

GGR_DEV u32 cw_next(u32 T, u32 A) { return ((~T & 0x3FFFFu) + (A << 1)) & T; }

#define CW_TILE 2048u
#define CW_TILE_CHUNKS (CW_TILE / 16u)
struct
#if defined(__CUDACC__)
    __align__(128)
#else
    alignas(128)
#endif
        CwTile {
  u8 buf[2][CW_TILE];
  unsigned long long bar[2];
};
#if defined(__CUDACC__)
GGR_DEV void cw_tile_init(CwTile* tl) {
#if defined(__CUDA_ARCH__)
  const unsigned b0 = (unsigned)__cvta_generic_to_shared(&tl->bar[0]), b1 = (unsigned)__cvta_generic_to_shared(&tl->bar[1]);
  asm volatile("mbarrier.init.shared::cta.b64 [%0], 1;" ::"r"(b0) : "memory");
  asm volatile("mbarrier.init.shared::cta.b64 [%0], 1;" ::"r"(b1) : "memory");
  asm volatile("fence.mbarrier_init.release.cluster;" ::: "memory");
  asm volatile("fence.proxy.async.shared::cta;" ::: "memory");
#endif
}
GGR_DEV void cw_tile_issue(CwTile* tl, u32 stg, const u8* src, u32 bytes) {
#if defined(__CUDA_ARCH__)
  const unsigned bar = (unsigned)__cvta_generic_to_shared(&tl->bar[stg]);
  const unsigned dst = (unsigned)__cvta_generic_to_shared(&tl->buf[stg][0]);
  asm volatile("mbarrier.arrive.expect_tx.shared::cta.b64 _, [%0], %1;" ::"r"(bar), "r"(bytes) : "memory");
  asm volatile("cp.async.bulk.shared::cluster.global.mbarrier::complete_tx::bytes [%0], [%1], %2, [%3];" ::"r"(dst), "l"(src), "r"(bytes),
               "r"(bar)
               : "memory");
#endif
}
GGR_DEV void cw_tile_wait(CwTile* tl, u32 stg, u32 parity) {
#if defined(__CUDA_ARCH__)
  const unsigned bar = (unsigned)__cvta_generic_to_shared(&tl->bar[stg]);
  asm volatile(
      "{\n"
      ".reg .pred p;\n"
      "CW_TILE_WAIT:\n"
      "mbarrier.try_wait.parity.shared::cta.b64 p, [%0], %1;\n"
      "@p bra CW_TILE_DONE;\n"
      "bra CW_TILE_WAIT;\n"
      "CW_TILE_DONE:\n"
      "}\n" ::"r"(bar),
      "r"(parity)
      : "memory");
#endif
}
#endif

GGR_DEV void cw_tok_item(CwTile* tl, u32& ph, const CwLut& LT, const u8* in, u32 start, u32 end, u8* region, u32 cap) {
  const u32 lane = wp_lane();
  if (end > CE_MAX_INPUT || cap < 8u || end == start) return;
  const u32* lut = LT.base.cls;
  const u32* lut2 = LT.cls2;
  u32* const gt = reinterpret_cast<u32*>(region) + 4;
  u8* const gqend = region + (size_t)cap * 16u;
  const u32 tcap = cw_tok_cap(cap), qcap = cw_q_cap(cap);
  const u32 lt = (1u << lane) - 1u;
  const u32 nchunks = (end + 15u) >> 4;
  u32 c_carry = 0, in_carry = 0, n_carry = 0, u_carry = 0;
  u32 k_carry = 0;
  u32 tbase = 0, qbase = 0, dbase = 0, ebase = 0;
  u32 bail = 0;
#if defined(__CUDA_ARCH__)
  const u32 ntiles = (nchunks + CW_TILE_CHUNKS - 1u) / CW_TILE_CHUNKS;
  if (lane == 0) {
    cw_tile_issue(tl, 0, in, (nchunks < CW_TILE_CHUNKS ? nchunks : CW_TILE_CHUNKS) << 4);
    if (ntiles > 1u) cw_tile_issue(tl, 1, in + CW_TILE, ((nchunks - CW_TILE_CHUNKS) < CW_TILE_CHUNKS ? (nchunks - CW_TILE_CHUNKS) : CW_TILE_CHUNKS) << 4);
  }
#else
  (void)tl;
  (void)ph;
  U4 vn;
  vn.x = vn.y = vn.z = vn.w = 0;
  if (lane < nchunks) vn = ggr_ld16(in + (lane << 4));
#endif
  for (u32 cb = 0; cb < nchunks; cb += 32) {
    const u32 ci = cb + lane;
    const u32 off = ci << 4;
    u32 Q = 0, B = 0, X = 0, W = 0xFFFFu, D = 0, HI = 0, XO = 0, XC = 0, XY = 0, XN = 0;
#if defined(__CUDA_ARCH__)
    U4 v;
    v.x = v.y = v.z = v.w = 0;
    {
      const u32 tile = cb / CW_TILE_CHUNKS, stg = tile & 1u, in_tile = cb & (CW_TILE_CHUNKS - 1u);
      if (in_tile == 0) {
        cw_tile_wait(tl, stg, (ph >> stg) & 1u);
        ph ^= 1u << stg;
      }
      if (ci < nchunks) {
        const uint4 q = *reinterpret_cast<const uint4*>(&tl->buf[stg][(in_tile + lane) << 4]);
        v.x = q.x; v.y = q.y; v.z = q.z; v.w = q.w;
      }
      if ((in_tile == CW_TILE_CHUNKS - 32u || cb + 32u >= nchunks) && tile + 2u < ntiles) {
        __syncwarp();
        if (lane == 0) {
          const u32 c0 = (tile + 2u) * CW_TILE_CHUNKS, left = nchunks - c0;
          cw_tile_issue(tl, stg, in + ((size_t)c0 << 4), (left < CW_TILE_CHUNKS ? left : CW_TILE_CHUNKS) << 4);
        }
      }
    }
#else
    const U4 v = vn;
    vn.x = vn.y = vn.z = vn.w = 0;
    if (ci + 32u < nchunks) vn = ggr_ld16(in + off + 512u);
#endif
    if (ci < nchunks) {
      u32 lo = 0, hi = 0, lo2 = 0, hi2 = 0;
#pragma unroll
      for (int j = 0; j < 4; j++) {
        const u32 b0 = (v.x >> (8 * j)) & 0xFFu, b1 = (v.y >> (8 * j)) & 0xFFu, b2 = (v.z >> (8 * j)) & 0xFFu, b3 = (v.w >> (8 * j)) & 0xFFu;
        lo |= lut[b0] << j;
        lo |= lut[b1] << (j + 4);
        hi |= lut[b2] << j;
        hi |= lut[b3] << (j + 4);
        lo2 |= lut2[b0] << j;
        lo2 |= lut2[b1] << (j + 4);
        hi2 |= lut2[b2] << j;
        hi2 |= lut2[b3] << (j + 4);
      }
      Q = (lo & 0xFFu) | ((hi & 0xFFu) << 8);
      B = ((lo >> 8) & 0xFFu) | (((hi >> 8) & 0xFFu) << 8);
      X = ((lo >> 16) & 0xFFu) | (((hi >> 16) & 0xFFu) << 8);
      W = ((lo >> 24) & 0xFFu) | (((hi >> 24) & 0xFFu) << 8);
      XO = (lo2 & 0xFFu) | ((hi2 & 0xFFu) << 8);
      XC = ((lo2 >> 8) & 0xFFu) | (((hi2 >> 8) & 0xFFu) << 8);
      XY = ((lo2 >> 16) & 0xFFu) | (((hi2 >> 16) & 0xFFu) << 8);
      XN = ((lo2 >> 24) & 0xFFu) | (((hi2 >> 24) & 0xFFu) << 8);
      u32 valid = 0xFFFFu;
      if (off < start) valid &= 0xFFFFu << (start - off);
      if (off + 16u > end) valid &= 0xFFFFu >> (off + 16u - end);
      Q &= valid;
      B &= valid;
      X &= valid;
      W = (W | ~valid) & 0xFFFFu;
      D = (ce_pack4(ce_ctrl_flags(v.x)) | (ce_pack4(ce_ctrl_flags(v.y)) << 4) | (ce_pack4(ce_ctrl_flags(v.z)) << 8) |
           (ce_pack4(ce_ctrl_flags(v.w)) << 12)) & valid;
      HI = (ce_pack4(v.x & 0x80808080u) | (ce_pack4(v.y & 0x80808080u) << 4) | (ce_pack4(v.z & 0x80808080u) << 8) |
            (ce_pack4(v.w & 0x80808080u) << 12)) & valid;
    }
    if (WP_ANY(HI != 0) || u_carry) {
      u32 C6 = 0, EC = 0;
      if (HI) {
        C6 = (ce_pack4((v.x << 1) & 0x80808080u) | (ce_pack4((v.y << 1) & 0x80808080u) << 4) |
              (ce_pack4((v.z << 1) & 0x80808080u) << 8) | (ce_pack4((v.w << 1) & 0x80808080u) << 12));
        for (u32 m = HI & C6; m; m &= m - 1u) {
          const u32 j = wp_ffs0(m);
          const u32 b0 = ce_byte16(v, j);
          const u32 b1 = j < 15 ? ce_byte16(v, j + 1) : (ggr_ld4(in + off + 16) & 0xFFu);
          u32 len = b0 < 0xC2u ? 0u : b0 < 0xE0u ? 2u : b0 < 0xF0u ? 3u : b0 < 0xF5u ? 4u : 0u;
          if ((b0 == 0xE0u && b1 < 0xA0u) || (b0 == 0xEDu && b1 >= 0xA0u) || (b0 == 0xF0u && b1 < 0x90u) || (b0 == 0xF4u && b1 >= 0x90u)) len = 0;
          if (len == 0) bail = 1;
          else EC |= ((1u << (len - 1u)) - 1u) << (j + 1u);
        }
      }
      u32 cin = WP_SHFL_UP(EC >> 16, 1);
      if (lane == 0) cin = u_carry;
      u_carry = WP_SHFL(EC >> 16, 31);
      if (((EC & 0xFFFFu) | cin) != (HI & ~C6)) bail = 1;
    }
    u32 E = 0;
    if (WP_ANY(B != 0) || c_carry) {
      u32 co0, co1;
      u32 E0 = ce_escaped(B, 0, &co0);
      u32 E1 = ce_escaped(B, 1, &co1);
      u32 Pm = WP_BALLOT(co0 != co1);
      u32 Gm = WP_BALLOT(co0 != 0);
      u32 np = ~Pm & lt;
      u32 cin = np ? ((Gm >> (31u - wp_clz(np))) & 1u) : c_carry;
      E = cin ? E1 : E0;
      u32 cout = cin ? co1 : co0;
      c_carry = WP_SHFL(cout, 31);
    }
    const u32 RQ = Q & ~E;
    const u32 EI = B & ~E;
    for (u32 m = E; m; m &= m - 1u) {
      u32 j = wp_ffs0(m);
      if (!(LT.base.kind[ce_byte16(v, j)] & 0x80u)) D |= 1u << j;
    }
    const u32 PB = WP_BALLOT((wp_popc(RQ) & 1u) != 0);
    const u32 in0 = (wp_popc(PB & lt) + in_carry) & 1u;
    in_carry = (in_carry + wp_popc(PB)) & 1u;
    const u32 IS = ce_prefix_xor16(RQ) ^ (in0 ? 0xFFFFu : 0u);
    const u32 SO = RQ & IS, SC = RQ & ~IS;
    const u32 ST = X & ~IS;
    const u32 N = ~(W | X | IS | SC) & 0xFFFFu;
    u32 pn = WP_SHFL_UP(N >> 15, 1);
    if (lane == 0) pn = n_carry;
    n_carry = WP_SHFL(N >> 15, 31);
    const u32 NS = N & ~((N << 1) | pn);
    const u32 TF = ST | SO | NS;
    const u32 K1 = ST & XO & XY, K2 = ST & XC & XY, K3 = ST & XO & ~XY, K4 = ST & XC & ~XY, KN = ST & XN;
    const u32 KM = ST & ~(XO | XC | XN);
    u32 lastk = 0;
    if (TF) {
      const u32 top = 1u << (31u - wp_clz(TF));
      lastk = (top & K1) ? 1u : (top & K2) ? 2u : (top & K3) ? 3u : (top & K4) ? 4u : (top & SO) ? 5u : (top & NS) ? 6u : (top & KN) ? 7u : 8u;
    }
    const u32 NZ = WP_BALLOT(TF != 0);
    const u32 below = NZ & lt;
    const u32 src_k = WP_SHFL(lastk, below ? 31u - wp_clz(below) : 0u);
    const u32 kin = below ? src_k : k_carry;
    {
      const u32 last_any = WP_SHFL(lastk, NZ ? 31u - wp_clz(NZ) : 0u);
      if (NZ) k_carry = last_any;
    }
    const u32 T17 = (TF << 1) | 1u;
    const u32 a1 = (K1 << 1) | (kin == 1u), a3 = (K3 << 1) | (kin == 3u), a5 = (SO << 1) | (kin == 5u);
    const u32 ae = ((K2 | K4 | NS) << 1) | (kin == 2u || kin == 4u || kin == 6u);
    const u32 an = (KN << 1) | (kin == 7u), am = (KM << 1) | (kin == 8u);
    const u32 vstart = (SO | NS | K1 | K3) << 1, vfollow = (KM | K2 | K4) << 1;
    const u32 nx_n = cw_next(T17, an), nx_m = cw_next(T17, am);
    u32 wrong = cw_next(T17, a1) & ~((SO | K2) << 1);
    wrong |= cw_next(T17, a3) & ~(vstart | (K4 << 1));
    wrong |= cw_next(T17, a5) & ~(vfollow | (KN << 1));
    wrong |= cw_next(T17, ae) & ~vfollow;
    wrong |= (nx_n | nx_m) & ~vstart;
    if (kin == 0u) wrong |= (T17 & ~1u) & (0u - (T17 & ~1u)) & ~(K1 << 1);
    if (wrong & 0x1FFFEu) bail = 1;
    const u32 CF = (nx_m >> 1) & 0xFFFFu, VF = (nx_n >> 1) & 0xFFFFu;
    const u32 TE = TF & ~(KN | KM);
    u32 tot;
    const u32 ex = WP_EXCL_SCAN(wp_popc(TE) | (wp_popc(RQ) << 16), &tot);
    u32 ti = tbase + (ex & 0xFFFFu), qi = qbase + (ex >> 16);
    tbase += tot & 0xFFFFu;
    qbase += tot >> 16;
    u32 ei = ebase, di = dbase;
    if (WP_ANY((EI | D) != 0)) {
      u32 tot2;
      const u32 ex2 = WP_EXCL_SCAN(wp_popc(EI) | (wp_popc(D) << 16), &tot2);
      ei += ex2 & 0xFFFFu;
      di += ex2 >> 16;
      ebase += tot2 & 0xFFFFu;
      dbase += tot2 >> 16;
    }
    const u32 qi0 = qi;
    for (u32 m = RQ; m; m &= m - 1u) {
      const u32 j = wp_ffs0(m), below_j = (1u << j) - 1u;
      if (qi < qcap) {
        u32* p = reinterpret_cast<u32*>(gqend - 8u * (qi + 1u));
        p[0] = ((off + j) & 0xFFFFu) | ((ei + wp_popc(EI & below_j)) << 16);
        p[1] = (di + wp_popc(D & below_j)) & 0xFFFFu;
      }
      qi++;
    }
    const u32 CL = K2 | K4, SQ = K3 | K4;
    for (u32 m = TE; m; m &= m - 1u) {
      const u32 j = wp_ffs0(m), bit = 1u << j;
      u32 kind = 1u + ((CL >> j) & 1u) + (((SQ >> j) & 1u) << 1);
      if (SO & bit) kind = K3_STR;
      if (NS & bit) kind = K3_SCALAR;
      const u32 sn = (qi0 + wp_popc(RQ & (bit - 1u))) >> 1;
      if (ti < tcap) gt[ti] = (off + j) | (kind << 16) | (((CF >> j) & 1u) << 19) | (((VF >> j) & 1u) << 20) | (sn << 21);
      ti++;
    }
  }
  const bool fail = WP_ANY(bail != 0) || in_carry || u_carry || tbase == 0 || tbase > tcap || qbase > qcap || k_carry != 2u;
  if (lane == 0) {
    U4 h = {tbase, qbase, fail ? 1u : 0u, 0xFFFFFFFFu};
    ggr_st16(region, h);
  }
}

struct CwPlaceSh {
  u32 lo[CW_LEVELS + 2];
};

GGR_DEV bool cw_context_ok(u32 k, u32 c, u32 v, u32 pk, u32 pv, u32 bk, u32 nv) {
  const bool pk_close = pk == K3_RBRACE || pk == K3_RBRACK;
  const bool pk_leaf = pk == K3_STR || pk == K3_SCALAR;
  const bool in_obj = bk == K3_LBRACE, in_arr = bk == K3_LBRACK;
  const bool val_end = pk_close || (pk_leaf && (in_arr || pv));
  const bool first = pk == bk && !c;
  const bool next = val_end && c;
  const bool closes = (k == K3_RBRACE && in_obj) || (k == K3_RBRACK && in_arr);
  const bool is_close = k == K3_RBRACE || k == K3_RBRACK;
  const bool r_close = closes && !c && !v && (pk == bk || val_end);
  const bool r_objval = in_obj && v && !c && pk == K3_STR && !pv;
  const bool r_key = in_obj && !v && k == K3_STR && nv && (first || next);
  const bool r_elem = in_arr && !v && (first || next);
  return is_close ? r_close : (r_objval || r_key || r_elem);
}

GGR_DEV void cw_place_item(CwPlaceSh& S, u8* region, u32 cap, u32 max_rec) {
  const u32 lane = wp_lane();
  const u32 lt = (1u << lane) - 1u, le = lt | (1u << lane);
  if (cap < 8u) return;
  const U4 h = ggr_ld16(region);
  if (h.z != 0 || h.x < 2u || h.x > 0xFFF0u) return;
  const u32 n = h.x;
  const u32* tok = reinterpret_cast<const u32*>(region) + 4;
  const u32 rec_off = cw_rec_off(n);
  const u32 q_bytes = 8u * h.y;
  if (rec_off + q_bytes + 64u >= cap * 16u) return;
  u32 rec_cap = (cap * 16u - q_bytes - rec_off - 32u) / 8u;
  if (rec_cap > max_rec) rec_cap = max_rec;
  u32* recs = reinterpret_cast<u32*>(region + rec_off);
  WP_SYNC();
  if (lane < CW_LEVELS + 2) S.lo[lane] = 0;
  WP_SYNC();
  i32 depth = 0;
  u32 cnt = 0, c_pk = 0, c_pv = 0, c_x = CW_NONE, c_xk = 0, bad = 0;
  for (u32 base = 0; base < n; base += 32) {
    const u32 i = base + lane;
    const bool act = i < n;
    const u32 t = act ? cw_ldg(tok + i) : 0u;
    const u32 k = K3_KIND(t), c = K3_C(t), v = K3_V(t);
    u32 nv = WP_SHFL(v, lane + 1u);
    if (lane == 31) nv = i + 1u < n ? K3_V(cw_ldg(tok + i + 1u)) : 0u;
    u32 pk = WP_SHFL_UP(k, 1), pv = WP_SHFL_UP(v, 1);
    if (lane == 0) { pk = c_pk; pv = c_pv; }
    const bool op = k == K3_LBRACE || k == K3_LBRACK, cl = k == K3_RBRACE || k == K3_RBRACK;
    const u32 OM = WP_BALLOT(op), CM = WP_BALLOT(cl);
    const i32 Ls = depth + (i32)wp_popc(OM & lt) - (i32)wp_popc(CM & lt);
    if (act && (Ls < 0 || Ls >= CW_LEVELS - 1)) bad = 1;
    const u32 L = (u32)Ls & 31u;
    const bool isval = act && (k == K3_STR || k == K3_SCALAR || op) && !(k == K3_STR && nv);
    const u32 VM = WP_BALLOT(isval);
    const u32 r = isval ? cnt + wp_popc(VM & lt) : CW_NONE;
    const u32 mv = act ? (op ? L + 1u : L) : 0x100u + lane;
    const u32 m = WP_MATCH_ANY(mv);
    const u32 cand = m & OM & lt;
    const u32 pl = cand ? 31u - wp_clz(cand) : 0u;
    const u32 r_pl = WP_SHFL(r, pl), k_pl = WP_SHFL(k, pl);
    u32 e_rec = CW_NONE, e_k = 0;
    if (!op && act) {
      if (cand) {
        e_rec = r_pl;
        e_k = k_pl;
      } else if (L >= 1u && L < CW_LEVELS) {
        const u32 w = S.lo[L];
        e_rec = w & 0xFFFFu;
        e_k = w >> 16;
      }
    }
    const u32 mw = (act && (op || cl)) ? (op ? L + 1u : L - 1u) : 0x100u + lane;
    const u32 m2 = WP_MATCH_ANY(mw);
    const u32 cand2 = m2 & OM & lt;
    const u32 pl2 = cand2 ? 31u - wp_clz(cand2) : 0u;
    const u32 r_pl2 = WP_SHFL(r, pl2), k_pl2 = WP_SHFL(k, pl2);
    u32 o_rec = CW_NONE, o_k = 0;
    if (cl) {
      if (cand2) {
        o_rec = r_pl2;
        o_k = k_pl2;
      } else if (L >= 2u && L <= CW_LEVELS) {
        const u32 w = S.lo[L - 1u];
        o_rec = w & 0xFFFFu;
        o_k = w >> 16;
      }
    }
    const u32 x = op ? r : (cl ? o_rec : e_rec), xk = op ? k : (cl ? o_k : e_k);
    u32 px = WP_SHFL_UP(x, 1), pxk = WP_SHFL_UP(xk, 1);
    if (lane == 0) { px = c_x; pxk = c_xk; }
    const u32 bk = op ? pxk : e_k;
    const u32 prec = op ? px : e_rec;
    if (act) {
      if (i == 0) {
        if (k != K3_LBRACE) bad = 1;
      } else if (!cw_context_ok(k, c, v, pk, pv, bk, nv)) {
        bad = 1;
      }
      if (op && !isval) bad = 1;
      if (i == n - 1u && !(k == K3_RBRACE && e_rec == 0u)) bad = 1;
      if (isval && i != 0 && prec == CW_NONE) bad = 1;
    }
    if (isval && r < rec_cap) {
      recs[2u * r] = i | (prec << 16);
      recs[2u * r + 1u] = L;
    }
    if (op && act && L + 1u < CW_LEVELS && (m & OM & ~le) == 0u) S.lo[L + 1u] = (r & 0xFFFFu) | (k << 16);
    WP_SYNC();
    depth += (i32)wp_popc(OM) - (i32)wp_popc(CM);
    cnt += wp_popc(VM);
    c_pk = WP_SHFL(k, 31);
    c_pv = WP_SHFL(v, 31);
    c_x = WP_SHFL(x, 31);
    c_xk = WP_SHFL(xk, 31);
  }
  const bool fail = WP_ANY(bad != 0) || depth != 0 || cnt == 0 || cnt > rec_cap;
  if (lane == 0 && !fail) reinterpret_cast<u32*>(region)[3] = cnt;
}

enum {
  CW_MSG = 0, CW_LIST = 1, CW_LISTP = 2, CW_MAP = 3, CW_EMSG = 4,
  CW_LEAF = 5, CW_ELEAF = 6, CW_SKIP = 7
};

template <int MN>
struct CoopWalkT {
  static const u32 MAX_NODE = MN;
  u16 vtok[MN];
  u16 par[MN];
  u16 first[MN];
  u16 slot[MN];
  u16 gfield[MN];
  u16 aux[MN];
  u8 cls[MN];
  u8 hdr[MN];
  u32 body[MN];
  u32 ssz[MN];
  u32 lvl_beg[CW_LEVELS + 2], lvl_cur[CW_LEVELS + 2];
  u32 bail, n_extra, cap;
};
typedef CoopWalkT<256> CoopWalk;
typedef CoopWalkT<1024> CoopWalkBig;
typedef CoopWalkT<8192> CoopWalkHuge;

GGR_DEVN bool cw_long_name_equals(const u8* in, u32 quote_pos, u32 end, const u8* pool, u32 off, u32 len) {
  return str_equals_pool(in, quote_pos, end, pool, off, len);
}
GGR_DEVN int cw_cmp_decoded(const u8* in, u32 a_pos, u32 b_pos, u32 end) { return cmp_str_tokens(in, a_pos, b_pos, end); }

GGR_DEV u32 cw_funnel(u32 lo, u32 hi, u32 sh) {
#if defined(__CUDA_ARCH__)
  return __funnelshift_r(lo, hi, sh);
#else
  return sh ? (lo >> sh) | (hi << (32u - sh)) : lo;
#endif
}
GGR_DEV void cw_key_info(const u8* in, u32 p, u32 n, KeyInfo* k) {
  const u8* base = in + (p & ~3u);
  const u32 sh = (p & 3u) * 8u;
  u32 h = GGR_KHASH_SEED;
  u32 w[4] = {0, 0, 0, 0};
  const u32 nw = (n + 3u) >> 2;
  u32 lo = ggr_ld4(base);
  for (u32 i = 0; i < nw; i++) {
    const u32 hi = ggr_ld4(base + 4u * (i + 1u));
    u32 x = cw_funnel(lo, hi, sh);
    lo = hi;
    const u32 left = n - 4u * i;
    if (left < 4u) x &= 0xFFFFFFFFu >> (8u * (4u - left));
    h = khash_mix(h, x);
    if (i == 0) w[0] = x;
    else if (i == 1) w[1] = x;
    else if (i == 2) w[2] = x;
    else if (i == 3) w[3] = x;
  }
  k->len = n;
  k->hash = khash_finish(h, n);
  k->w[0] = w[0];
  k->w[1] = w[1];
  k->w[2] = w[2];
  k->w[3] = w[3];
}
GGR_DEV bool cw_hash_lookup(const Tables& t, u32 first, u32 mask, const KeyInfo& k, const u8* in, u32 quote_pos, u32 end, i32* value) {
  u32 slot = k.hash & mask;
  for (u32 probes = 0; probes <= mask; probes++) {
    const u8* ep = t.hash + (size_t)(first + slot) * 32;
    const U4 e = ggr_ld16(ep);
    if (e.z == 0xFFFFFFFFu) return false;
    if (e.x == k.hash && e.z == k.len) {
      const U4 nm = ggr_ld16(ep + 16);
      if (nm.x == k.w[0] && nm.y == k.w[1] && nm.z == k.w[2] && nm.w == k.w[3]) {
        if (k.len <= 16 || cw_long_name_equals(in, quote_pos, end, t.pool, e.y, k.len)) {
          *value = (i32)e.w;
          return true;
        }
      }
    }
    slot = (slot + 1) & mask;
  }
  return false;
}
GGR_DEVN bool cw_enum_by_name(const Tables& T, const u8* in, u32 end, i32 child, u32 pos, u32 close, i32* num) {
  KeyInfo ki;
  cw_key_info(in, pos + 1u, close - pos - 1u, &ki);
  const U4 e = ggr_ld16(T.enums + (size_t)child * 16);
  return cw_hash_lookup(T, e.z, e.w, ki, in, pos, end, num);
}

struct CwLeaf {
  u32 type, a, b, flags, body;
  bool zero;
};

GGR_DEV bool cw_int_literal(const u8* in, u32 pos, u32 end, bool* neg, u64* mag) {
  u32 j = pos;
  const bool n = in[j] == '-';
  if (n) j++;
  const u32 d0 = j;
  u64 v = 0;
  u32 nd = 0;
  while (j < end && nd < 20u) {
    const u32 c = (u32)in[j] - '0';
    if (c >= 10u) break;
    v = v * 10u + c;
    j++;
    nd++;
  }
  if (nd == 0 || nd > 19u || (nd > 1u && in[d0] == '0')) return false;
  if (j < end) {
    const u32 c = in[j];
    if (!(ggr_is_ws(c) || c == ',' || c == '}' || c == ']')) return false;
  }
  *neg = n;
  *mag = v;
  return true;
}
GGR_DEV bool cw_int_value(u32 kind, bool neg, u64 mag, u64* out) {
  const bool sg = kind_is_signed(kind) || kind == GK_ENUM;
  const int bits = kind == GK_ENUM ? 32 : kind_bits(kind);
  if (sg) {
    const u64 lim = bits == 32 ? 0x80000000ull : 0x8000000000000000ull;
    if (neg ? mag > lim : mag >= lim) return false;
    *out = neg ? (u64)(0 - mag) : mag;
    return true;
  }
  if (neg) return false;
  if (bits == 32 && mag > 0xFFFFFFFFull) return false;
  *out = mag;
  return true;
}
GGR_DEV bool cw_scalar_is(const u8* in, u32 pos, u32 end, const char* lit, u32 n) {
  if (end - pos < n) return false;
  for (u32 j = 0; j < n; j++)
    if (in[pos + j] != (u8)lit[j]) return false;
  if (pos + n >= end) return true;
  const u32 c = in[pos + n];
  return ggr_is_ws(c) || c == ',' || c == '}' || c == ']';
}

GGR_DEV bool cw_int_quoted(const u8* in, u32 pos, u32 close, bool* neg, u64* mag) {
  u32 j = pos + 1u;
  const bool n = j < close && in[j] == '-';
  if (n) j++;
  const u32 d0 = j;
  u64 v = 0;
  u32 nd = 0;
  while (j < close && nd < 20u) {
    const u32 c = (u32)in[j] - '0';
    if (c >= 10u) return false;
    v = v * 10u + c;
    j++;
    nd++;
  }
  if (j != close || nd == 0 || nd > 19u || (nd > 1u && in[d0] == '0')) return false;
  *neg = n;
  *mag = v;
  return true;
}

GGR_DEVN bool cw_float_literal(const u8* in, u32 pos, u32 end, u32 lim, bool is32, u64* bits) {
  static const double P10[23] = {1e0, 1e1, 1e2, 1e3, 1e4, 1e5, 1e6, 1e7, 1e8, 1e9, 1e10, 1e11, 1e12, 1e13, 1e14, 1e15, 1e16, 1e17, 1e18, 1e19, 1e20, 1e21, 1e22};
  const u32 stop = lim ? lim : end;
  u32 j = pos;
  bool neg = false;
  if (j < stop && in[j] == '-') { neg = true; j++; }
  u64 m = 0;
  u32 sig = 0, nint = 0;
  const u32 i0 = j;
  while (j < stop && (u32)(in[j] - '0') < 10u) {
    const u32 c = in[j] - '0';
    if (sig || c) { if (sig >= 15u) return false; m = m * 10u + c; sig++; }
    j++;
    nint++;
  }
  if (nint == 0 || (nint > 1u && in[i0] == '0')) return false;
  i32 e10 = 0;
  if (j < stop && in[j] == '.') {
    j++;
    u32 nfrac = 0;
    while (j < stop && (u32)(in[j] - '0') < 10u) {
      const u32 c = in[j] - '0';
      if (sig || c) { if (sig >= 15u) return false; m = m * 10u + c; sig++; }
      e10--;
      j++;
      nfrac++;
    }
    if (nfrac == 0) return false;
  }
  if (j < stop && (in[j] == 'e' || in[j] == 'E')) {
    j++;
    bool eneg = false;
    if (j < stop && (in[j] == '+' || in[j] == '-')) { eneg = in[j] == '-'; j++; }
    u32 ne = 0, ev = 0;
    while (j < stop && (u32)(in[j] - '0') < 10u && ne < 4u) { ev = ev * 10u + (in[j] - '0'); j++; ne++; }
    if (ne == 0 || (j < stop && (u32)(in[j] - '0') < 10u)) return false;
    e10 += eneg ? -(i32)ev : (i32)ev;
  }
  if (lim) {
    if (j != lim) return false;
  } else if (j < end) {
    const u32 c = in[j];
    if (!(ggr_is_ws(c) || c == ',' || c == '}' || c == ']')) return false;
  }
  double d;
  if (m == 0) d = 0.0;
  else if (e10 >= 0 && e10 <= 22) d = (double)m * P10[e10];
  else if (e10 < 0 && e10 >= -22) d = (double)m / P10[-e10];
  else return false;
  if (neg) d = -d;
  if (is32) {
    const float f = (float)d;
    if ((double)f != d) return false;
    u32 b;
    memcpy(&b, &f, 4);
    *bits = b;
  } else {
    memcpy(bits, &d, 8);
  }
  return true;
}

GGR_DEVN bool cw_bytes_leaf(const u8* in, u32 pos, u32 end, u32* n_out, u32* flags) {
  Rd r;
  r.init(in, pos, end);
  StrInfo si;
  if (scan_string<true>(r, &si) != GST_OK) return false;
  StrIter it;
  it.init(in, pos, end);
  const bool url = (si.flags & SF_URLSAFE) != 0;
  u32 n;
  if (!b64_run<false, Cnt>(it, url, si.dec_len, (Cnt*)0, &n)) return false;
  *n_out = n;
  *flags = (url ? NF_URL : 0u) | ((si.dec_len & 3u) ? 0u : NF_PADDED);
  return true;
}

GGR_DEVN bool cw_timestamp(const u8* in, u32 pos, u32 end, i64* secs, i32* nanos) {
  StrIter it;
  it.init(in, pos, end);
  return parse_timestamp(it, secs, nanos) == GST_OK;
}

GGR_DEVN bool cw_slow_key(const u8* in, u32 key_pos, u32 end, u32* dec_len, u32* flags) {
  Rd r;
  r.init(in, key_pos, end);
  StrInfo si;
  if (scan_string<false>(r, &si) != GST_OK) return false;
  *dec_len = si.dec_len;
  *flags = (si.flags & SF_ESCAPES) ? NF_ESC : 0u;
  return true;
}

GGR_DEVN bool cw_leaf_rare(const Tables& T, const CwIndex& X, const u8* in, u32 end, const FieldD& f, u32 t, CwLeaf* l) {
  const u32 k = K3_KIND(t), pos = K3_POS(t);
  switch (f.kind) {
    case GK_STRING: {
      if (k != K3_STR) return false;
      const CwQ q0 = cw_q(X, K3_Q(t)), q1 = cw_q(X, K3_Q(t) + 1u);
      if (q0.slow != q1.slow) {
        Rd r;
        r.init(in, pos, end);
        StrInfo si;
        if (scan_string<false>(r, &si) != GST_OK) return false;
        l->type = N_STR;
        l->a = pos;
        l->b = si.dec_len;
        l->flags = (si.flags & SF_ESCAPES) ? NF_ESC : 0u;
        l->body = varint_size(si.dec_len) + si.dec_len;
        l->zero = si.dec_len == 0;
        return true;
      }
      const u32 nesc = (q1.esc - q0.esc) & 0xFFFFu;
      const u32 len = q1.pos - pos - 1u - nesc;
      l->type = N_STR;
      l->a = pos;
      l->b = len;
      l->flags = nesc ? (NF_ESC | NF_SIMPLE) : 0u;
      l->body = varint_size(len) + len;
      l->zero = len == 0;
      return true;
    }
    case GK_BOOL: {
      if (k != K3_SCALAR) return false;
      Leaf x;
      if (cw_scalar_is(in, pos, end, "true", 4)) leaf_from_int(GK_BOOL, 1, &x);
      else if (cw_scalar_is(in, pos, end, "false", 5)) leaf_from_int(GK_BOOL, 0, &x);
      else return false;
      l->type = x.type; l->a = x.a; l->b = x.b; l->flags = 0; l->body = x.body; l->zero = x.zero;
      return true;
    }
    case GK_INT32: case GK_INT64: case GK_UINT32: case GK_UINT64: case GK_SINT32: case GK_SINT64:
    case GK_FIXED32: case GK_FIXED64: case GK_SFIXED32: case GK_SFIXED64: case GK_ENUM: {
      u64 v;
      if (k == K3_SCALAR) {
        bool neg;
        u64 mag;
        if (!cw_int_literal(in, pos, end, &neg, &mag) || !cw_int_value(f.kind, neg, mag, &v)) return false;
      } else if (k == K3_STR && f.kind != GK_ENUM) {
        const CwQ q0 = cw_q(X, K3_Q(t)), q1 = cw_q(X, K3_Q(t) + 1u);
        bool neg;
        u64 mag;
        if (q0.slow != q1.slow || q0.esc != q1.esc || !cw_int_quoted(in, pos, q1.pos, &neg, &mag) || !cw_int_value(f.kind, neg, mag, &v)) return false;
      } else if (k == K3_STR && f.kind == GK_ENUM) {
        const CwQ q0 = cw_q(X, K3_Q(t)), q1 = cw_q(X, K3_Q(t) + 1u);
        if (q0.slow != q1.slow || q0.esc != q1.esc) return false;
        i32 num;
        if (!cw_enum_by_name(T, in, end, f.child, pos, q1.pos, &num)) return false;
        v = (u64)(i64)num;
      } else {
        return false;
      }
      Leaf x;
      leaf_from_int(f.kind, v, &x);
      l->type = x.type; l->a = x.a; l->b = x.b; l->flags = 0; l->body = x.body; l->zero = x.zero;
      return true;
    }
    case GK_FLOAT: case GK_DOUBLE: {
      const bool is32 = f.kind == GK_FLOAT;
      u64 bits;
      if (k == K3_SCALAR) {
        if (!cw_float_literal(in, pos, end, 0u, is32, &bits)) return false;
      } else if (k == K3_STR) {
        const CwQ q0 = cw_q(X, K3_Q(t)), q1 = cw_q(X, K3_Q(t) + 1u);
        if (q0.slow != q1.slow || q0.esc != q1.esc || q1.pos <= pos + 1u || !cw_float_literal(in, pos + 1u, end, q1.pos, is32, &bits)) return false;
      } else {
        return false;
      }
      l->flags = 0;
      l->zero = bits == 0;
      l->a = (u32)bits;
      if (is32) { l->type = N_FIX32; l->b = 0; l->body = 4; }
      else { l->type = N_FIX64; l->b = (u32)(bits >> 32); l->body = 8; }
      return true;
    }
    case GK_BYTES: {
      if (k != K3_STR) return false;
      u32 n, fl;
      if (!cw_bytes_leaf(in, pos, end, &n, &fl)) return false;
      l->type = N_BYTES;
      l->a = pos;
      l->b = n;
      l->flags = fl;
      l->body = varint_size(n) + n;
      l->zero = n == 0;
      return true;
    }
    default:
      return false;
  }
}

GGR_DEV u32 cw_str_pack(const CwIndex& X, u32 t) {
  const CwQ q0 = cw_q(X, K3_Q(t)), q1 = cw_q(X, K3_Q(t) + 1u);
  const u32 nesc = (q1.esc - q0.esc) & 0xFFFFu, raw = (q1.pos - K3_POS(t) - 1u) & 0xFFFFu;
  return (q0.slow == q1.slow && nesc < 0x8000u) ? (raw | (nesc << 16) | 0x80000000u) : 0u;
}
template <bool FULL>
GGR_DEV bool cw_leaf(const Tables& T, const CwIndex& X, const u8* in, u32 end, const FieldD& f, u32 t, CwLeaf* l) {
  const u32 k = K3_KIND(t), pos = K3_POS(t);
  if (f.kind == GK_STRING) {
    if (k != K3_STR) return false;
    const u32 vinf = cw_str_pack(X, t);
    if (!(vinf >> 31)) return FULL ? cw_leaf_rare(T, X, in, end, f, t, l) : false;
    const u32 nesc = (vinf >> 16) & 0x7FFFu;
    const u32 len = (vinf & 0xFFFFu) - nesc;
    l->type = N_STR;
    l->a = pos;
    l->b = len;
    l->flags = nesc ? (NF_ESC | NF_SIMPLE) : 0u;
    l->body = varint_size(len) + len;
    l->zero = len == 0;
    return true;
  }
  if (k == K3_SCALAR && f.kind != GK_FLOAT && f.kind != GK_DOUBLE && f.kind != GK_BOOL && f.kind != GK_BYTES) {
    bool neg;
    u64 mag, v;
    if (cw_int_literal(in, pos, end, &neg, &mag) && cw_int_value(f.kind, neg, mag, &v)) {
      Leaf x;
      leaf_from_int(f.kind, v, &x);
      l->type = x.type; l->a = x.a; l->b = x.b; l->flags = 0; l->body = x.body; l->zero = x.zero;
      return true;
    }
    return false;
  }
  if (!FULL) return false;
  return cw_leaf_rare(T, X, in, end, f, t, l);
}

GGR_DEV bool cw_plain_less(const u8* in, u32 a_pos, u32 a_end, u32 b_pos, u32 b_end) {
  const u32 na = a_end - a_pos - 1u, nb = b_end - b_pos - 1u;
  const u32 n = na < nb ? na : nb;
  const u8* a = in + a_pos + 1u;
  const u8* b = in + b_pos + 1u;
  for (u32 j = 0; j < n; j++) {
    const u32 x = a[j], y = b[j];
    if (x != y) return x < y;
  }
  return na < nb;
}

GGR_DEVN bool cw_ts_leaf(const CwIndex& X, const u8* in, u32 end, u32 t, u32 tag, u32 tag_len, u8* ir, u32* io, u32 r, u32 n_rec,
                         u32* n_extra, u32 cap, u32* body) {
  const CwQ q0 = cw_q(X, K3_Q(t)), q1 = cw_q(X, K3_Q(t) + 1u);
  i64 secs = 0;
  i32 nanos = 0;
  if (K3_KIND(t) != K3_STR || q0.slow != q1.slow || q0.esc != q1.esc || !cw_timestamp(in, K3_POS(t), end, &secs, &nanos)) return false;
  const u32 x = wp_atomic_add(n_extra, 2u);
  if (n_rec + x + 2u > cap) return false;
  const u32 sidx = n_rec + x, nidx = n_rec + x + 1u;
  u32 payload = 0;
  if (nanos != 0) payload += 1u + varint_size((u64)(u32)nanos);
  if (secs != 0) payload += 1u + varint_size((u64)secs);
  node_store(ir, nidx, (u32)nanos, 0, GGR_NIL, 1, nanos != 0 ? node_meta(N_VARINT, 0, 16) : node_meta(N_SKIP, 0, 0));
  node_store(ir, sidx, (u32)(u64)secs, (u32)((u64)secs >> 32), nanos != 0 ? nidx : GGR_NIL, 0,
             secs != 0 ? node_meta(N_VARINT, 0, 8) : node_meta(N_SKIP, 0, 0));
  const u32 first_child = secs != 0 ? sidx : (nanos != 0 ? nidx : GGR_NIL);
  node_store(ir, r, payload, first_child, GGR_NIL, 0, node_meta(N_MSG, 0, tag));
  io[sidx] = 0xFFFFFFFFu;
  io[nidx] = 0xFFFFFFFFu;
  *body = tag_len + varint_size(payload) + payload;
  return true;
}

GGR_DEV u32 cw_keypart_of(const u8* ir, u32 x) {
  const u32 klen = node_load(ir, x).y;
  return 1u + varint_size(klen) + klen;
}

template <class SH, bool FULL>
GGR_DEV bool cw_type_item(SH& S, const Tables& T, u32 root_msg, const u8* in, u32 start, u32 end, u8* region, u32* ioff, u32 cap,
                          EncResult* res) {
  const u32 lane = wp_lane();
  const u32 lt = (1u << lane) - 1u, le = lt | (1u << lane);
  res->size = 0;
  res->first = GGR_NIL;
  res->n_nodes = 0;
  res->method = 0;
  res->id_pos = res->id_len = 0;
  if (end > CE_MAX_INPUT || cap < 8u || root_msg >= 0xFFFFu) return (CW_WHY(1), false);
  if (end == start) return true;
  CwIndex X;
  u32 n_rec;
  {
    const U4 h = ggr_ld16(region);
    if (h.z != 0 || h.w == 0xFFFFFFFFu || h.w == 0u || h.w > SH::MAX_NODE) return (CW_WHY(2), false);
    X.n_tok = h.x;
    X.n_q = h.y;
    X.tok = reinterpret_cast<const u32*>(region) + 4;
    X.qend = region + (size_t)cap * 16u;
    n_rec = h.w;
  }
  const u32 rec_off = cw_rec_off(X.n_tok);
  const u32 shift = (rec_off + 8u * n_rec + 15u) >> 4;
  const u32 q_nodes = (8u * X.n_q + 15u) >> 4;
  if (shift + q_nodes + 2u >= cap) return (CW_WHY(3), false);
  const u32 node_cap = cap - shift - q_nodes - 1u;
  if (n_rec > node_cap) return (CW_WHY(4), false);
  u8* ir = region + (size_t)shift * 16u;
  u32* io = ioff + shift;
  WP_SYNC();
  if (lane == 0) {
    S.bail = 0;
    S.n_extra = 0;
    S.cap = node_cap;
  }
  if (lane < CW_LEVELS + 2) S.lvl_cur[lane] = 0;
  WP_SYNC();
  {
    const u32* recs = reinterpret_cast<const u32*>(region + rec_off);
    for (u32 r = lane; r < n_rec; r += 32) {
      const u32 a = cw_ldg(recs + 2u * r), l = cw_ldg(recs + 2u * r + 1u) & 15u;
      S.gfield[r] = (u16)a;
      S.aux[r] = (u16)(a >> 16);
      S.cls[r] = (u8)l;
      wp_atomic_add(&S.lvl_cur[l], 1u);
    }
  }
  WP_SYNC();
  u32 max_level;
  {
    const u32 c = lane < CW_LEVELS ? S.lvl_cur[lane] : 0u;
    u32 tot;
    const u32 ex = WP_EXCL_SCAN(c, &tot);
    max_level = 31u - wp_clz(WP_BALLOT(c != 0) | 1u);
    WP_SYNC();
    if (lane <= CW_LEVELS) {
      S.lvl_beg[lane] = ex;
      S.lvl_cur[lane] = ex;
    }
  }
  WP_SYNC();
  if (S.lvl_beg[1] != 1u) return (CW_WHY(5), false);
  for (u32 rb = 0; rb < n_rec; rb += 32) {
    const u32 r = rb + lane;
    const bool act = r < n_rec;
    const u32 l = act ? (u32)S.cls[r] : 0xFFu;
    u32 pos = 0;
    for (u32 rem = WP_BALLOT(act); rem;) {
      const u32 ld = wp_ffs0(rem);
      const u32 lv = WP_SHFL(l, ld);
      const u32 mk = WP_BALLOT(l == lv);
      const u32 b = S.lvl_cur[lv];
      if (l == lv) pos = b + wp_popc(mk & lt);
      WP_SYNC();
      if (lane == ld) S.lvl_cur[lv] = b + wp_popc(mk);
      rem &= ~mk;
    }
    WP_SYNC();
    if (act) {
      S.slot[r] = (u16)pos;
      S.vtok[pos] = S.gfield[r];
    }
  }
  WP_SYNC();
  for (u32 r = lane; r < n_rec; r += 32) {
    const u32 pos = S.slot[r];
    const u32 pd = S.aux[r];
    S.par[pos] = pd == CW_NONE ? (u16)CW_NONE : S.slot[pd];
    if (r + 1u < n_rec && (u32)S.aux[r + 1u] == r) S.first[pos] = S.slot[r + 1u];
  }
  WP_SYNC();
  if (lane == 0) {
    S.cls[0] = CW_MSG;
    S.aux[0] = (u16)root_msg;
    S.gfield[0] = 0;
    S.hdr[0] = 0;
    S.body[0] = 0;
    S.ssz[0] = 0;
    S.slot[0] = 0;
  }
  WP_SYNC();
  if (ggr_msg(T, root_msg).wkt != GGR_WKT_NONE) return (CW_WHY(7), false);
  for (u32 d = 1; d <= max_level; d++) {
    const u32 lb = S.lvl_beg[d], le_ = S.lvl_beg[d + 1];
    for (u32 rb = lb; rb < le_; rb += 32) {
      const u32 r = rb + lane;
      const bool act = r < le_;
      u32 emit = 0, p = 0, pc = CW_SKIP;
      if (act) {
        const u32 i = S.vtok[r];
        p = S.par[r];
        pc = S.cls[p];
        const u32 t = cw_ldg(X.tok + i);
        const u32 k = K3_KIND(t);
        bool ok = true;
        u32 gf = 0, cls = CW_SKIP, aux = 0, hdr = 0, body = 0;
        FieldD f;
        bool in_list = false;
        u32 key_pos = 0, key_end = 0, key_esc = 0, key_dec = 0, key_flags = 0;
        bool key_slow = false;
        bool is_ts = false;
        if (pc == CW_MSG || pc == CW_EMSG) {
          const u32 kinf = cw_key_pack(X, i);
          if (!(kinf >> 31)) ok = (CW_WHY(101), false);
          const MsgD md = ggr_msg(T, S.aux[p]);
          i32 ei = 0;
          if (ok) {
            KeyInfo ki;
            const u32 kpos = kinf & 0xFFFFu;
            cw_key_info(in, kpos, (kinf >> 16) & 0x7FFFu, &ki);
            ok = cw_hash_lookup(T, md.key_hash_first, md.key_hash_mask, ki, in, kpos - 1u, end, &ei);
          }
          if (ok && (u32)ei >= 32u) ok = (CW_WHY(102), false);
          if (ok) {
            emit = (u32)ei;
            gf = md.field_first + emit;
            f = ggr_field(T, gf);
            const u32 bit = 1u << emit;
            if (wp_atomic_or(&S.ssz[p], bit) & bit) ok = (CW_WHY(103), false);
          }
          if (ok) {
            if (gf >= 0xFFFFu) {
              ok = (CW_WHY(104), false);
            } else if (k == K3_SCALAR && cw_scalar_is(in, K3_POS(t), end, "null", 4)) {
              cls = CW_SKIP;
            } else {
              if (f.oneof >= 0 && !(f.flags & (GF_MAP | GF_REPEATED))) {
                const u32 ob = 1u << (f.oneof & 31);
                if (wp_atomic_or(&S.body[p], ob) & ob) ok = (CW_WHY(105), false);
              }
              if (f.flags & GF_MAP) {
                const MsgD ed = ggr_msg(T, (u32)f.child);
                const FieldD kf = ggr_field(T, ed.field_first);
                if (k != K3_LBRACE || kf.kind != GK_STRING) ok = (CW_WHY(106), false);
                cls = CW_MAP;
              } else if (f.flags & GF_REPEATED) {
                if (k != K3_LBRACK) ok = (CW_WHY(107), false);
                if (f.kind == GK_MESSAGE) {
                  const u32 w = ggr_msg(T, (u32)f.child).wkt;
                  if (w != GGR_WKT_NONE && w != GGR_WKT_TIMESTAMP) ok = (CW_WHY(108), false);
                }
                cls = (f.flags & GF_PACKED) ? CW_LISTP : CW_LIST;
                hdr = f.tag_len;
              } else if (f.kind == GK_MESSAGE && ggr_msg(T, (u32)f.child).wkt == GGR_WKT_TIMESTAMP) {
                cls = CW_LEAF;
                is_ts = true;
              } else if (f.kind == GK_MESSAGE) {
                if (k != K3_LBRACE || (u32)f.child >= 0xFFFFu || ggr_msg(T, (u32)f.child).wkt != GGR_WKT_NONE) ok = (CW_WHY(109), false);
                cls = CW_MSG;
                aux = (u32)f.child;
                hdr = f.tag_len;
              } else {
                cls = CW_LEAF;
              }
            }
          }
        } else if (pc == CW_LIST || pc == CW_LISTP) {
          gf = S.gfield[p];
          f = ggr_field(T, gf);
          in_list = true;
          if (f.kind == GK_MESSAGE && ggr_msg(T, (u32)f.child).wkt == GGR_WKT_TIMESTAMP) {
            cls = CW_LEAF;
            is_ts = true;
          } else if (f.kind == GK_MESSAGE) {
            if (k != K3_LBRACE || (u32)f.child >= 0xFFFFu) ok = (CW_WHY(110), false);
            cls = CW_MSG;
            aux = (u32)f.child;
            hdr = f.tag_len;
          } else {
            if (k == K3_SCALAR && cw_scalar_is(in, K3_POS(t), end, "null", 4)) ok = (CW_WHY(111), false);
            cls = CW_LEAF;
          }
        } else if (pc == CW_MAP) {
          gf = S.gfield[p];
          const FieldD mapf = ggr_field(T, gf);
          const MsgD ed = ggr_msg(T, (u32)mapf.child);
          f = ggr_field(T, ed.field_first + 1u);
          const u32 kt = cw_ldg(X.tok + i - 1u);
          const CwQ q0 = cw_q(X, K3_Q(kt)), q1 = cw_q(X, K3_Q(kt) + 1u);
          key_pos = K3_POS(kt);
          key_end = q1.pos;
          key_esc = (q1.esc - q0.esc) & 0xFFFFu;
          key_slow = q0.slow != q1.slow;
          if (key_slow && (!FULL || !cw_slow_key(in, key_pos, end, &key_dec, &key_flags))) ok = (CW_WHY(112), false);
          if (ok && r > (u32)S.first[p]) {
            const u32 pt = cw_ldg(X.tok + (u32)S.vtok[r - 1u] - 1u);
            const CwQ p0 = cw_q(X, K3_Q(pt)), p1 = cw_q(X, K3_Q(pt) + 1u);
            if (p0.slow != p1.slow && !FULL) ok = (CW_WHY(113), false);
            else if (p0.slow == p1.slow && !key_slow && p0.esc == p1.esc && key_esc == 0u) ok = cw_plain_less(in, K3_POS(pt), p1.pos, key_pos, key_end);
            else ok = cw_cmp_decoded(in, K3_POS(pt), key_pos, end) < 0;
          }
          in_list = true;
          if (f.kind == GK_MESSAGE) {
            if (k != K3_LBRACE || (u32)f.child >= 0xFFFFu || ggr_msg(T, (u32)f.child).wkt != GGR_WKT_NONE) ok = (CW_WHY(114), false);
            cls = CW_EMSG;
            aux = (u32)f.child;
          } else {
            if (k == K3_SCALAR && cw_scalar_is(in, K3_POS(t), end, "null", 4)) ok = (CW_WHY(115), false);
            cls = CW_ELEAF;
          }
        } else {
          ok = (CW_WHY(116), false);
        }
        if (ok && is_ts) {
          if (!FULL || !cw_ts_leaf(X, in, end, t, f.tag, f.tag_len, ir, io, r, n_rec, &S.n_extra, S.cap, &body)) ok = (CW_WHY(119), false);
        } else if (ok && (cls == CW_LEAF || cls == CW_ELEAF)) {
          CwLeaf l;
          if ((k != K3_STR && k != K3_SCALAR) || !cw_leaf<FULL>(T, X, in, end, f, t, &l)) {
            ok = (CW_WHY(117), false);
          } else if (cls == CW_LEAF) {
            const bool packed = pc == CW_LISTP;
            const u32 tag = packed ? 0u : f.tag, tag_len = packed ? 0u : f.tag_len;
            const bool live = in_list || (f.flags & GF_PRESENCE) || !l.zero;
            node_store(ir, r, l.a, l.b, GGR_NIL, 0, live ? node_meta(l.type, l.flags, tag) : node_meta(N_SKIP, 0, 0));
            body = live ? tag_len + l.body : 0u;
          } else {
            const u32 x = wp_atomic_add(&S.n_extra, 2u);
            const u32 klen = key_slow ? key_dec : key_end - key_pos - 1u - key_esc;
            const u32 keypart = 1u + varint_size(klen) + klen;
            const u32 payload = keypart + f.tag_len + l.body;
            const FieldD mapf = ggr_field(T, gf);
            if (n_rec + x + 2u > S.cap) {
              ok = (CW_WHY(118), false);
            } else {
              node_store(ir, r, payload, GGR_NIL, GGR_NIL, 0, node_meta(N_ENTRY, 0, mapf.tag));
              node_store(ir, n_rec + x, key_pos, klen, GGR_NIL, 0, node_meta(N_STR, key_slow ? key_flags : (key_esc ? (NF_ESC | NF_SIMPLE) : 0u), 0x0Au));
              node_store(ir, n_rec + x + 1u, l.a, l.b, GGR_NIL, 1, node_meta(l.type, l.flags, f.tag));
              aux = x;
              hdr = mapf.tag_len + varint_size(payload);
              body = mapf.tag_len + varint_size(payload) + payload;
            }
          }
        }
        if (ok && cls == CW_SKIP) node_store(ir, r, 0, 0, GGR_NIL, 0, node_meta(N_SKIP, 0, 0));
        if (!ok) S.bail = 1;
        S.gfield[r] = (u16)gf;
        S.cls[r] = (u8)cls;
        S.aux[r] = (u16)aux;
        S.hdr[r] = (u8)hdr;
        S.body[r] = body;
        S.ssz[r] = 0;
        S.slot[r] = (u16)emit;
      }
    }
    WP_SYNC();
    if (S.bail) return false;
    for (u32 r = lb + lane; r < le_; r += 32) {
      const u32 p = S.par[r];
      const u32 pc = S.cls[p];
      if (pc == CW_MSG || pc == CW_EMSG) S.slot[r] = (u16)((u32)S.first[p] + wp_popc(S.ssz[p] & ((1u << S.slot[r]) - 1u)));
      else S.slot[r] = (u16)r;
    }
    WP_SYNC();
  }
  for (u32 r = lane; r < n_rec; r += 32) {
    const u32 c = S.cls[r];
    if (c <= CW_EMSG) S.body[r] = 0;
  }
  WP_SYNC();
  for (u32 d = max_level; d >= 1; d--) {
    const u32 lb = S.lvl_beg[d], le_ = S.lvl_beg[d + 1];
    for (u32 r = lb + lane; r < le_; r += 32) {
      const u32 c = S.cls[r];
      u32 full;
      if (c >= CW_LEAF) {
        full = S.body[r];
      } else {
        const u32 payload = S.body[r];
        const u32 gf = S.gfield[r];
        const u32 tag = ggr_ld4(T.fields + (size_t)gf * 32 + 4);
        u32 h;
        if (c == CW_MSG) {
          h = (u32)S.hdr[r] + varint_size(payload);
          node_store(ir, r, payload, GGR_NIL, GGR_NIL, 0, node_meta(N_MSG, 0, tag));
          full = h + payload;
        } else if (c == CW_LIST || c == CW_MAP) {
          h = 0;
          node_store(ir, r, payload, GGR_NIL, GGR_NIL, 0, node_meta(payload ? (c == CW_LIST ? N_LIST : N_MAP) : N_SKIP, 0, 0));
          full = payload;
        } else if (c == CW_LISTP) {
          const bool empty = payload == 0;
          h = empty ? 0u : (u32)S.hdr[r] + varint_size(payload);
          node_store(ir, r, payload, GGR_NIL, GGR_NIL, 0, empty ? node_meta(N_SKIP, 0, 0) : node_meta(N_LIST, NF_PACKED, tag));
          full = h + payload;
        } else {
          const u32 i = S.vtok[r];
          const u32 kt = cw_ldg(X.tok + i - 1u);
          const CwQ q0 = cw_q(X, K3_Q(kt)), q1 = cw_q(X, K3_Q(kt) + 1u);
          const u32 key_esc = (q1.esc - q0.esc) & 0xFFFFu;
          const u32 key_pos = K3_POS(kt);
          const bool kslow = q0.slow != q1.slow;
          u32 kdec = 0, kflags = 0;
          if (kslow && (!FULL || !cw_slow_key(in, key_pos, end, &kdec, &kflags))) S.bail = 1;
          const u32 klen = kslow ? kdec : q1.pos - key_pos - 1u - key_esc;
          const u32 keypart = 1u + varint_size(klen) + klen;
          const FieldD mapf = ggr_field(T, gf);
          const MsgD ed = ggr_msg(T, (u32)mapf.child);
          const FieldD vf = ggr_field(T, ed.field_first + 1u);
          const u32 vfull = vf.tag_len + varint_size(payload) + payload;
          const u32 ent = keypart + vfull;
          const u32 x = wp_atomic_add(&S.n_extra, 2u);
          if (n_rec + x + 2u > S.cap) {
            S.bail = 1;
            h = 0;
          } else {
            const u32 eh = mapf.tag_len + varint_size(ent);
            node_store(ir, r, ent, GGR_NIL, GGR_NIL, 0, node_meta(N_ENTRY, 0, mapf.tag));
            node_store(ir, n_rec + x, key_pos, klen, GGR_NIL, 0, node_meta(N_STR, kslow ? kflags : (key_esc ? (NF_ESC | NF_SIMPLE) : 0u), 0x0Au));
            node_store(ir, n_rec + x + 1u, payload, GGR_NIL, GGR_NIL, 1, node_meta(N_MSG, 0, vf.tag));
            S.aux[r] = (u16)x;
            h = eh + keypart + vf.tag_len + varint_size(payload);
            if (h > 255u) S.bail = 1;
            S.vtok[r] = (u16)eh;
          }
          full = h + payload;
        }
        S.hdr[r] = (u8)h;
      }
      S.ssz[S.slot[r]] = full;
    }
    WP_SYNC();
    if (S.bail) return false;
    for (u32 sb = lb; sb < le_; sb += 32) {
      const u32 s = sb + lane;
      const bool act = s < le_;
      const u32 p = act ? (u32)S.par[s] : 0x10000u + lane;
      const u32 v = act ? S.ssz[s] : 0u;
      u32 tot;
      const u32 ex = WP_EXCL_SCAN(v, &tot);
      u32 pp = WP_SHFL_UP(p, 1);
      const bool head = lane == 0 || pp != p;
      const u32 HM = WP_BALLOT(head);
      const u32 s0 = 31u - wp_clz(HM & le);
      const u32 ex0 = WP_SHFL(ex, s0);
      const u32 before = act ? S.body[p] : 0u;
      const bool last = act && (lane == 31 || ((HM >> (lane + 1u)) & 1u) || s + 1u == le_);
      WP_SYNC();
      if (act) S.ssz[s] = before + ex - ex0;
      if (last) S.body[p] = before + ex - ex0 + v;
      WP_SYNC();
    }
  }
  const u32 total = S.body[0];
  if (total > (FULL ? 0x0FFFFFFFu : CE_STAGE)) return (CW_WHY(10), false);
  WP_SYNC();
  if (lane == 0) S.body[0] = 0;
  WP_SYNC();
  for (u32 d = 1; d <= max_level; d++) {
    const u32 lb = S.lvl_beg[d], le_ = S.lvl_beg[d + 1];
    for (u32 r = lb + lane; r < le_; r += 32) {
      const u32 p = S.par[r];
      const u32 a = S.body[p] + (u32)S.hdr[p] + S.ssz[S.slot[r]];
      const u32 c = S.cls[r];
      io[r] = a;
      if (c == CW_ELEAF) {
        const u32 x = n_rec + S.aux[r];
        io[x] = a + (u32)S.hdr[r];
        io[x + 1u] = a + (u32)S.hdr[r] + cw_keypart_of(ir, x);
      } else if (c == CW_EMSG) {
        const u32 x = n_rec + S.aux[r];
        const u32 eh = S.vtok[r];
        io[x] = a + eh;
        io[x + 1u] = a + eh + cw_keypart_of(ir, x);
      }
      if (c <= CW_EMSG) S.body[r] = a;
    }
    WP_SYNC();
  }
  res->size = total;
  res->first = GGR_NIL;
  res->n_nodes = n_rec + S.n_extra;
  res->method = shift;
  return true;
}
```

Measured before the change: 18.81 million.

## Precompute key name IDs in place pass and use schema-wide member hash

The place kernel now hashes each object key once against a global interned-name table and stores a name ID per record. The walk/type kernel then looks up (message, name-id) in a compact member hash instead of rehashing key bytes against per-message tables, falling back to the old path when no ID exists. Field descriptors also gain flags marking Timestamp and other well-known child types, so the message table no longer has to be read just to check wkt. The cost is extra hashing work and table reads in the place kernel, a larger schema blob, and slightly lower place occupancy.

After: 18.98 million (median of 6 runs). Within noise of the previous version (+1.0%).

```diff
diff --git a/__graft_entry__.py b/__graft_entry__.py
--- a/__graft_entry__.py
+++ b/__graft_entry__.py
@@ -15,6 +15,7 @@
     import benchgen
     benchgen.build()
     subprocess.check_call(["make", "-s", "-C", os.path.join(ROOT, "tests", "hostsim")])
+    subprocess.check_call(["make", "-s", "-C", os.path.join(ROOT, "tests", "walknames")])
     import ggrmcp_b200
 
 
diff --git a/ggrmcp_b200/csrc/ggr_engine.cu b/ggrmcp_b200/csrc/ggr_engine.cu
--- a/ggrmcp_b200/csrc/ggr_engine.cu
+++ b/ggrmcp_b200/csrc/ggr_engine.cu
@@ -631,7 +631,7 @@
         ggr_launch_encode_tok2(st, n, in, in_off, (u8*)sc.ir.p, big, counters, e->sm_count);
         if (prof) prof_mark(e, st, &t1);
         t_tok = t1;
-        ggr_launch_encode_place(st, n, in_off, (u8*)sc.ir.p, big, counters, e->sm_count);
+        ggr_launch_encode_place(st, n, s->d_blob, in, in_off, (u8*)sc.ir.p, big, counters, e->sm_count);
         size_t t2 = 0, t3 = 0;
         if (prof) prof_mark(e, st, &t2);
         ggr_launch_encode_type(st, 0, n, s->d_blob, n_msgs, msg_id, in, in_off, (u8*)sc.ir.p, (u32*)sc.size.p, (u32*)sc.aux.p, status,
diff --git a/ggrmcp_b200/csrc/ggr_kernels.h b/ggrmcp_b200/csrc/ggr_kernels.h
--- a/ggrmcp_b200/csrc/ggr_kernels.h
+++ b/ggrmcp_b200/csrc/ggr_kernels.h
@@ -20,8 +20,8 @@
                                  const uint32_t* list_n, uint32_t frame);
 void ggr_launch_encode_tok2(cudaStream_t st, long long n, const uint8_t* in, const uint64_t* in_off, uint8_t* ir, const uint32_t* list,
                             const uint32_t* list_n, int sm_count);
-void ggr_launch_encode_place(cudaStream_t st, long long n, const uint64_t* in_off, uint8_t* ir, const uint32_t* list, const uint32_t* list_n,
-                             int sm_count);
+void ggr_launch_encode_place(cudaStream_t st, long long n, const uint8_t* blob, const uint8_t* in, const uint64_t* in_off, uint8_t* ir,
+                             const uint32_t* list, const uint32_t* list_n, int sm_count);
 void ggr_launch_encode_type(cudaStream_t st, int tier, long long n, const uint8_t* blob, uint32_t n_msgs, const int32_t* msg_id, const uint8_t* in,
                             const uint64_t* in_off, uint8_t* ir, uint32_t* size, uint32_t* first, int32_t* status, uint32_t* ioff,
                             uint32_t* nnodes, const uint32_t* list, const uint32_t* list_n, uint32_t* pending, uint32_t* n_pending,
diff --git a/ggrmcp_b200/csrc/ggr_kernels_walk.cu b/ggrmcp_b200/csrc/ggr_kernels_walk.cu
--- a/ggrmcp_b200/csrc/ggr_kernels_walk.cu
+++ b/ggrmcp_b200/csrc/ggr_kernels_walk.cu
@@ -3,7 +3,7 @@
 
 #define CW_WARPS 4
 #define CW_TOK_BLOCKS 8
-#define CW_PLACE_BLOCKS 12
+#define CW_PLACE_BLOCKS 10
 #define CW_WALK_BLOCKS 6
 
 __global__ void __launch_bounds__(CW_WARPS * 32, CW_TOK_BLOCKS)
@@ -33,9 +33,11 @@
 }
 
 __global__ void __launch_bounds__(CW_WARPS * 32, CW_PLACE_BLOCKS)
-k_encode_place(const u64* __restrict__ in_off, u8* __restrict__ ir, const u32* __restrict__ list, const u32* __restrict__ list_n) {
+k_encode_place(const u8* __restrict__ blob, const u8* __restrict__ in, const u64* __restrict__ in_off, u8* __restrict__ ir,
+               const u32* __restrict__ list, const u32* __restrict__ list_n) {
   __shared__ CwPlaceSh S[CW_WARPS];
   const u32 warp = threadIdx.x >> 5;
+  const Tables T = ggr_tables(blob);
   const long long total = (long long)*list_n;
   const u64 a0 = in_off[0];
   u32* ticket = const_cast<u32*>(list_n) + 3;
@@ -47,7 +49,8 @@
     if (b <= a || b - a > (u64)CE_MAX_INPUT - 16u) continue;
     const u64 node_off = ((a - a0) >> 1) + 8ull * (u64)item;
     const u32 cap = (u32)((((b - a0) >> 1) + 8ull * (u64)(item + 1)) - node_off);
-    cw_place_item(S[warp], ir + node_off * 16, cap, CoopWalkHuge::MAX_NODE);
+    const u32 s0 = (u32)(a & 15ull);
+    cw_place_item(S[warp], T, in + (a & ~15ull), s0 + (u32)(b - a), ir + node_off * 16, cap, CoopWalkHuge::MAX_NODE);
   }
 }
 
@@ -124,12 +127,12 @@
   k_encode_tok3<<<(unsigned)(want < cap ? want : cap), CW_WARPS * 32, 0, st>>>(in, (const u64*)in_off, ir, list, list_n);
 }
 
-void ggr_launch_encode_place(cudaStream_t st, long long n, const uint64_t* in_off, uint8_t* ir, const uint32_t* list, const uint32_t* list_n,
-                             int sm_count) {
+void ggr_launch_encode_place(cudaStream_t st, long long n, const uint8_t* blob, const uint8_t* in, const uint64_t* in_off, uint8_t* ir,
+                             const uint32_t* list, const uint32_t* list_n, int sm_count) {
   static unsigned per_sm = 0;
   if (!per_sm) per_sm = cw_grid((const void*)k_encode_place, CW_WARPS * 32, 0, 1ll << 40, 1);
   const long long want = (n + CW_WARPS - 1) / CW_WARPS, cap = (long long)sm_count * per_sm;
-  k_encode_place<<<(unsigned)(want < cap ? want : cap), CW_WARPS * 32, 0, st>>>((const u64*)in_off, ir, list, list_n);
+  k_encode_place<<<(unsigned)(want < cap ? want : cap), CW_WARPS * 32, 0, st>>>(blob, in, (const u64*)in_off, ir, list, list_n);
 }
 
 void ggr_launch_encode_type(cudaStream_t st, int tier, long long n, const uint8_t* blob, uint32_t n_msgs, const int32_t* msg_id, const uint8_t* in,
diff --git a/ggrmcp_b200/csrc/ggr_prim.cuh b/ggrmcp_b200/csrc/ggr_prim.cuh
--- a/ggrmcp_b200/csrc/ggr_prim.cuh
+++ b/ggrmcp_b200/csrc/ggr_prim.cuh
@@ -257,10 +257,16 @@
   const u8* u16s;
   const u8* pool;
   const u8* tools;
+  const u8* members;
+  u32 name_first, name_mask, member_mask;
 };
 GGR_DEV Tables ggr_tables(const u8* blob) {
-  U4 h0 = ggr_ld16(blob), h1 = ggr_ld16(blob + 16), h2 = ggr_ld16(blob + 32), h3 = ggr_ld16(blob + 48);
+  U4 h0 = ggr_ld16(blob), h1 = ggr_ld16(blob + 16), h2 = ggr_ld16(blob + 32), h3 = ggr_ld16(blob + 48), h4 = ggr_ld16(blob + 64);
   Tables t;
+  t.name_first = h4.x;
+  t.name_mask = h4.y;
+  t.member_mask = h4.z;
+  t.members = blob + h4.w;
   t.tools = blob + h0.y - 16;
   t.msgs = blob + h0.w;
   t.fields = blob + h1.y;
diff --git a/ggrmcp_b200/csrc/ggr_schema.cc b/ggrmcp_b200/csrc/ggr_schema.cc
--- a/ggrmcp_b200/csrc/ggr_schema.cc
+++ b/ggrmcp_b200/csrc/ggr_schema.cc
@@ -237,6 +237,23 @@
   return o;
 }
 
+uint8_t wkt_of(const MsgIn& m) {
+  uint8_t wkt = GGR_WKT_NONE;
+  if (m.full_name == "google.protobuf.Timestamp") wkt = GGR_WKT_TIMESTAMP;
+  else if (m.full_name == "google.protobuf.Duration") wkt = GGR_WKT_DURATION;
+  else if (m.full_name == "google.protobuf.Empty") wkt = GGR_WKT_EMPTY;
+  else if (m.full_name == "google.protobuf.FieldMask" && m.fields.size() == 1 && m.fields[0].number == 1) wkt = GGR_WKT_FIELDMASK;
+  else if (m.full_name.rfind("google.protobuf.", 0) == 0) {
+    static const char* wr[] = {"DoubleValue", "FloatValue", "Int64Value", "UInt64Value", "Int32Value", "UInt32Value", "BoolValue",
+                               "StringValue", "BytesValue"};
+    for (const char* w : wr)
+      if (m.full_name == std::string("google.protobuf.") + w && m.fields.size() == 1 && m.fields[0].number == 1) wkt = GGR_WKT_WRAPPER;
+    static const char* wk[] = {"Any", "Struct", "Value", "ListValue"};
+    for (const char* w : wk) if (m.full_name == std::string("google.protobuf.") + w) wkt = GGR_WKT_UNSUPPORTED;
+  }
+  return wkt;
+}
+
 int wire_type_for(int kind) {
   switch (kind) {
     case GK_DOUBLE: case GK_FIXED64: case GK_SFIXED64: return 1;
@@ -350,6 +367,10 @@
       if (!f.have_json) f.json_name = default_json_name(f.name);
     }
   }
+  std::vector<uint8_t> wkt(P.msgs.size());
+  for (size_t mi = 0; mi < P.msgs.size(); mi++) wkt[mi] = wkt_of(P.msgs[mi]);
+  std::map<std::string, uint32_t> name_id;
+  std::vector<std::pair<uint32_t, uint32_t>> members;
   for (size_t mi = 0; mi < P.msgs.size(); mi++) {
     MsgIn& m = P.msgs[mi];
     GgrMsg gm;
@@ -372,18 +393,7 @@
     gm.n_fields = (uint16_t)m.fields.size();
     gm.n_oneofs = (uint32_t)m.n_oneofs;
     if (m.map_entry) gm.flags |= GM_MAP_ENTRY;
-    if (m.full_name == "google.protobuf.Timestamp") gm.wkt = GGR_WKT_TIMESTAMP;
-    else if (m.full_name == "google.protobuf.Duration") gm.wkt = GGR_WKT_DURATION;
-    else if (m.full_name == "google.protobuf.Empty") gm.wkt = GGR_WKT_EMPTY;
-    else if (m.full_name == "google.protobuf.FieldMask" && m.fields.size() == 1 && m.fields[0].number == 1) gm.wkt = GGR_WKT_FIELDMASK;
-    else if (m.full_name.rfind("google.protobuf.", 0) == 0) {
-      static const char* wr[] = {"DoubleValue", "FloatValue", "Int64Value", "UInt64Value", "Int32Value", "UInt32Value", "BoolValue",
-                                 "StringValue", "BytesValue"};
-      for (const char* w : wr)
-        if (m.full_name == std::string("google.protobuf.") + w && m.fields.size() == 1 && m.fields[0].number == 1) gm.wkt = GGR_WKT_WRAPPER;
-      static const char* wk[] = {"Any", "Struct", "Value", "ListValue"};
-      for (const char* w : wk) if (m.full_name == std::string("google.protobuf.") + w) gm.wkt = GGR_WKT_UNSUPPORTED;
-    }
+    gm.wkt = wkt[mi];
     bool decl_is_emit = true;
     std::vector<uint16_t> decl_perm(m.fields.size());
     uint32_t max_num = 0;
@@ -412,6 +422,8 @@
       gf.oneof = real_oneof(f) ? (int16_t)f.oneof_index : (int16_t)-1;
       gf.decl_index = (uint16_t)f.decl;
       gf.child = f.child;
+      if ((f.type == GK_MESSAGE || f.type == GK_GROUP) && wkt[f.child] != GGR_WKT_NONE)
+        gf.flags |= wkt[f.child] == GGR_WKT_TIMESTAMP ? GF_CHILD_TS : GF_CHILD_WKT;
       std::string key = json_quote(f.json_name) + ":";
       gf.name_off = B.intern(key);
       gf.name_len = (uint16_t)key.size();
@@ -438,6 +450,11 @@
     for (auto& kv : by_json) items.push_back({kv.first, (int32_t)decl_perm[kv.second]});
     for (auto& kv : by_text) if (!by_json.count(kv.first)) items.push_back({kv.first, (int32_t)decl_perm[kv.second]});
     gm.key_hash_first = B.add_table(items, &gm.key_hash_mask);
+    for (auto& it : items) {
+      const auto ins = name_id.insert({it.first, (uint32_t)name_id.size()});
+      const uint32_t gfi = gm.field_first + (uint32_t)it.second;
+      members.push_back({((uint32_t)mi << 16) | (ins.first->second & 0xFFFFu), (uint32_t)it.second | ((gfi < 0xFFFFu ? gfi : 0xFFFFu) << 16)});
+    }
     B.msgs.push_back(gm);
     if (m.fields.size() > out->max_msg_fields) out->max_msg_fields = (uint32_t)m.fields.size();
     out->msg_index[m.full_name] = (int32_t)mi;
@@ -482,6 +499,24 @@
     for (auto& M : out->methods)
       B.u16.push_back((M.client_streaming || M.server_streaming || M.input_msg >= 0xFFFF) ? (uint16_t)0xFFFF : (uint16_t)M.input_msg);
   }
+  uint32_t name_hash_first, name_hash_mask;
+  std::vector<uint32_t> mtab;
+  {
+    const bool ids = name_id.size() <= GGR_MAX_NAME_IDS;
+    std::vector<std::pair<std::string, int32_t>> items;
+    if (ids)
+      for (auto& kv : name_id) items.push_back({kv.first, (int32_t)kv.second});
+    name_hash_first = B.add_table(items, &name_hash_mask);
+    uint32_t size = 4;
+    while (ids && size < members.size() * 2 + 1) size <<= 1;
+    mtab.assign(2 * (size_t)size, 0xFFFFFFFFu);
+    for (size_t j = 0; ids && j < members.size(); j++) {
+      uint32_t slot = GGR_MEMBER_HASH(members[j].first) & (size - 1);
+      while (mtab[2 * slot] != 0xFFFFFFFFu) slot = (slot + 1) & (size - 1);
+      mtab[2 * slot] = members[j].first;
+      mtab[2 * slot + 1] = members[j].second;
+    }
+  }
   GgrSchemaHdr h;
   memset(&h, 0, sizeof h);
   std::vector<uint8_t>& o = out->blob;
@@ -498,6 +533,10 @@
   h.evals_off = append_section(o, B.evals.data(), B.evals.size() * sizeof(GgrEnumValue));
   h.n_hash = (uint32_t)B.hash.size();
   h.hash_off = append_section(o, B.hash.data(), B.hash.size() * sizeof(GgrHashEnt));
+  h.name_hash_first = name_hash_first;
+  h.name_hash_mask = name_hash_mask;
+  h.member_mask = (uint32_t)(mtab.size() / 2 - 1);
+  h.members_off = append_section(o, mtab.data(), mtab.size() * sizeof(uint32_t));
   h.n_u16 = (uint32_t)B.u16.size();
   h.u16_off = append_section(o, B.u16.data(), B.u16.size() * sizeof(uint16_t));
   B.pool.append(32, '\0');
diff --git a/ggrmcp_b200/csrc/ggr_tables.h b/ggrmcp_b200/csrc/ggr_tables.h
--- a/ggrmcp_b200/csrc/ggr_tables.h
+++ b/ggrmcp_b200/csrc/ggr_tables.h
@@ -16,9 +16,15 @@
 #define GF_MAP 0x04u
 #define GF_PRESENCE 0x08u
 #define GF_PACKABLE 0x10u
+#define GF_CHILD_TS 0x20u
+#define GF_CHILD_WKT 0x40u
 
 #define GM_MAP_ENTRY 0x01u
 #define GM_DECL_IS_EMIT 0x02u
+
+#define GGR_NO_NAME_ID 0xFFFFu
+#define GGR_MAX_NAME_IDS 0xFFFEu
+#define GGR_MEMBER_HASH(k) (((k) * 0x9E3779B1u) ^ (((k) * 0x9E3779B1u) >> 16))
 
 struct GgrSchemaHdr {
   uint32_t magic;
@@ -30,6 +36,8 @@
   uint32_t n_hash, hash_off;
   uint32_t n_u16, u16_off;
   uint32_t pool_bytes, pool_off;
+  uint32_t name_hash_first, name_hash_mask;
+  uint32_t member_mask, members_off;
 };
 
 struct GgrToolsTrailer {
diff --git a/ggrmcp_b200/csrc/ggr_walk.cuh b/ggrmcp_b200/csrc/ggr_walk.cuh
--- a/ggrmcp_b200/csrc/ggr_walk.cuh
+++ b/ggrmcp_b200/csrc/ggr_walk.cuh
@@ -7,6 +7,12 @@
 #else
 extern int g_cw_why;
 #define CW_WHY(code) (g_cw_why = (code))
+#endif
+#if defined(__CUDA_ARCH__) || defined(__CUDACC__)
+#define CW_NOID() ((void)0)
+#else
+static int g_cw_noid = 0;
+#define CW_NOID() (g_cw_noid++)
 #endif
 #define CW_NONE 0xFFFFu
 
@@ -336,6 +342,111 @@
   }
 }
 
+GGR_DEVN bool cw_long_name_equals(const u8* in, u32 quote_pos, u32 end, const u8* pool, u32 off, u32 len) {
+  return str_equals_pool(in, quote_pos, end, pool, off, len);
+}
+GGR_DEV u32 cw_funnel(u32 lo, u32 hi, u32 sh) {
+#if defined(__CUDA_ARCH__)
+  return __funnelshift_r(lo, hi, sh);
+#else
+  return sh ? (lo >> sh) | (hi << (32u - sh)) : lo;
+#endif
+}
+GGR_DEV void cw_key_info(const u8* in, u32 p, u32 n, KeyInfo* k) {
+  const u8* base = in + (p & ~3u);
+  const u32 sh = (p & 3u) * 8u;
+  u32 h = GGR_KHASH_SEED;
+  u32 w[4] = {0, 0, 0, 0};
+  const u32 nw = (n + 3u) >> 2;
+  u32 lo = ggr_ld4(base);
+  for (u32 i = 0; i < nw; i++) {
+    const u32 hi = ggr_ld4(base + 4u * (i + 1u));
+    u32 x = cw_funnel(lo, hi, sh);
+    lo = hi;
+    const u32 left = n - 4u * i;
+    if (left < 4u) x &= 0xFFFFFFFFu >> (8u * (4u - left));
+    h = khash_mix(h, x);
+    if (i == 0) w[0] = x;
+    else if (i == 1) w[1] = x;
+    else if (i == 2) w[2] = x;
+    else if (i == 3) w[3] = x;
+  }
+  k->len = n;
+  k->hash = khash_finish(h, n);
+  k->w[0] = w[0];
+  k->w[1] = w[1];
+  k->w[2] = w[2];
+  k->w[3] = w[3];
+}
+GGR_DEV bool cw_hash_lookup(const Tables& t, u32 first, u32 mask, const KeyInfo& k, const u8* in, u32 quote_pos, u32 end, i32* value) {
+  u32 slot = k.hash & mask;
+  for (u32 probes = 0; probes <= mask; probes++) {
+    const u8* ep = t.hash + (size_t)(first + slot) * 32;
+    const U4 e = ggr_ld16(ep);
+    if (e.z == 0xFFFFFFFFu) return false;
+    if (e.x == k.hash && e.z == k.len) {
+      const U4 nm = ggr_ld16(ep + 16);
+      if (nm.x == k.w[0] && nm.y == k.w[1] && nm.z == k.w[2] && nm.w == k.w[3]) {
+        if (k.len <= 16 || cw_long_name_equals(in, quote_pos, end, t.pool, e.y, k.len)) {
+          *value = (i32)e.w;
+          return true;
+        }
+      }
+    }
+    slot = (slot + 1) & mask;
+  }
+  return false;
+}
+GGR_DEV u32 cw_name_id(const Tables& T, const u8* in, u32 end, const u8* qend, u32 kt) {
+  const u32 kp = K3_POS(kt) + 1u;
+  const U4 q = ggr_ld16(qend - 16u * ((kt >> 21) + 1u));
+  const u8* base = in + (kp & ~3u);
+  const u32 w0 = ggr_ld4(base), w1 = ggr_ld4(base + 4), w2 = ggr_ld4(base + 8), w3 = ggr_ld4(base + 12), w4 = ggr_ld4(base + 16);
+  const u32 n = ((q.x & 0xFFFFu) - kp) & 0xFFFFu;
+  if (q.y != q.w || (q.x >> 16) != (q.z >> 16) || n >= 0x8000u) return GGR_NO_NAME_ID;
+  const u32 sh = (kp & 3u) * 8u;
+  KeyInfo k;
+  k.len = n;
+  k.w[0] = cw_funnel(w0, w1, sh);
+  k.w[1] = cw_funnel(w1, w2, sh);
+  k.w[2] = cw_funnel(w2, w3, sh);
+  k.w[3] = cw_funnel(w3, w4, sh);
+  u32 h = GGR_KHASH_SEED;
+#pragma unroll
+  for (u32 i = 0; i < 4u; i++) {
+    const u32 left = n > 4u * i ? n - 4u * i : 0u;
+    if (left < 4u) k.w[i] &= left ? 0xFFFFFFFFu >> (8u * (4u - left)) : 0u;
+    if (left) h = khash_mix(h, k.w[i]);
+  }
+  if (n > 16u) {
+    u32 lo = w4;
+    for (u32 i = 4; 4u * i < n; i++) {
+      const u32 hi = ggr_ld4(base + 4u * (i + 1u));
+      u32 x = cw_funnel(lo, hi, sh);
+      lo = hi;
+      const u32 left = n - 4u * i;
+      if (left < 4u) x &= 0xFFFFFFFFu >> (8u * (4u - left));
+      h = khash_mix(h, x);
+    }
+  }
+  k.hash = khash_finish(h, n);
+  u32 slot = k.hash & T.name_mask;
+  for (u32 probes = 0; probes <= T.name_mask; probes++) {
+    const u8* ep = T.hash + (size_t)(T.name_first + slot) * 32;
+    const U4 e = ggr_ld16(ep), nm = ggr_ld16(ep + 16);
+    if (e.z == 0xFFFFFFFFu) break;
+    if (e.x == k.hash && e.z == n) {
+      if (nm.x == k.w[0] && nm.y == k.w[1] && nm.z == k.w[2] && nm.w == k.w[3]) {
+        u32 j = 16;
+        while (j < n && in[kp + j] == T.pool[e.y + j]) j++;
+        if (j >= n) return e.w;
+      }
+    }
+    slot = (slot + 1u) & T.name_mask;
+  }
+  return GGR_NO_NAME_ID;
+}
+
 struct CwPlaceSh {
   u32 lo[CW_LEVELS + 2];
 };
@@ -356,7 +467,8 @@
   return is_close ? r_close : (r_objval || r_key || r_elem);
 }
 
-GGR_DEV void cw_place_item(CwPlaceSh& S, u8* region, u32 cap, u32 max_rec) {
+template <bool IDS>
+GGR_DEV void cw_place_item_t(CwPlaceSh& S, const Tables& T, const u8* in, u32 end, u8* region, u32 cap, u32 max_rec) {
   const u32 lane = wp_lane();
   const u32 lt = (1u << lane) - 1u, le = lt | (1u << lane);
   if (cap < 8u) return;
@@ -365,6 +477,7 @@
   const u32 n = h.x;
   const u32* tok = reinterpret_cast<const u32*>(region) + 4;
   const u32 rec_off = cw_rec_off(n);
+  const u8* const qend = region + (size_t)cap * 16u;
   const u32 q_bytes = 8u * h.y;
   if (rec_off + q_bytes + 64u >= cap * 16u) return;
   u32 rec_cap = (cap * 16u - q_bytes - rec_off - 32u) / 8u;
@@ -374,7 +487,7 @@
   if (lane < CW_LEVELS + 2) S.lo[lane] = 0;
   WP_SYNC();
   i32 depth = 0;
-  u32 cnt = 0, c_pk = 0, c_pv = 0, c_x = CW_NONE, c_xk = 0, bad = 0;
+  u32 cnt = 0, c_t = 0, c_x = CW_NONE, c_xk = 0, bad = 0;
   for (u32 base = 0; base < n; base += 32) {
     const u32 i = base + lane;
     const bool act = i < n;
@@ -382,8 +495,9 @@
     const u32 k = K3_KIND(t), c = K3_C(t), v = K3_V(t);
     u32 nv = WP_SHFL(v, lane + 1u);
     if (lane == 31) nv = i + 1u < n ? K3_V(cw_ldg(tok + i + 1u)) : 0u;
-    u32 pk = WP_SHFL_UP(k, 1), pv = WP_SHFL_UP(v, 1);
-    if (lane == 0) { pk = c_pk; pv = c_pv; }
+    u32 pt = WP_SHFL_UP(t, 1);
+    if (lane == 0) pt = c_t;
+    const u32 pk = K3_KIND(pt), pv = K3_V(pt);
     const bool op = k == K3_LBRACE || k == K3_LBRACK, cl = k == K3_RBRACE || k == K3_RBRACK;
     const u32 OM = WP_BALLOT(op), CM = WP_BALLOT(cl);
     const i32 Ls = depth + (i32)wp_popc(OM & lt) - (i32)wp_popc(CM & lt);
@@ -439,22 +553,34 @@
       if (i == n - 1u && !(k == K3_RBRACE && e_rec == 0u)) bad = 1;
       if (isval && i != 0 && prec == CW_NONE) bad = 1;
     }
+    const bool member = isval && v && !c && pk == K3_STR && !pv;
+    const u32 id = IDS && member ? cw_name_id(T, in, end, qend, pt) : GGR_NO_NAME_ID;
     if (isval && r < rec_cap) {
       recs[2u * r] = i | (prec << 16);
-      recs[2u * r + 1u] = L;
+      recs[2u * r + 1u] = L | (id << 16);
     }
     if (op && act && L + 1u < CW_LEVELS && (m & OM & ~le) == 0u) S.lo[L + 1u] = (r & 0xFFFFu) | (k << 16);
     WP_SYNC();
     depth += (i32)wp_popc(OM) - (i32)wp_popc(CM);
     cnt += wp_popc(VM);
-    c_pk = WP_SHFL(k, 31);
-    c_pv = WP_SHFL(v, 31);
+    c_t = WP_SHFL(t, 31);
     c_x = WP_SHFL(x, 31);
     c_xk = WP_SHFL(xk, 31);
   }
   const bool fail = WP_ANY(bad != 0) || depth != 0 || cnt == 0 || cnt > rec_cap;
   if (lane == 0 && !fail) reinterpret_cast<u32*>(region)[3] = cnt;
 }
+
+GGR_DEV void cw_place_item(CwPlaceSh& S, const Tables& T, const u8* in, u32 end, u8* region, u32 cap, u32 max_rec) {
+  cw_place_item_t<true>(S, T, in, end, region, cap, max_rec);
+}
+#if !defined(__CUDACC__)
+inline void cw_place_item(CwPlaceSh& S, u8* region, u32 cap, u32 max_rec) {
+  Tables T;
+  memset(&T, 0, sizeof T);
+  cw_place_item_t<false>(S, T, nullptr, 0, region, cap, max_rec);
+}
+#endif
 
 enum {
   CW_MSG = 0, CW_LIST = 1, CW_LISTP = 2, CW_MAP = 3, CW_EMSG = 4,
@@ -481,63 +607,8 @@
 typedef CoopWalkT<1024> CoopWalkBig;
 typedef CoopWalkT<8192> CoopWalkHuge;
 
-GGR_DEVN bool cw_long_name_equals(const u8* in, u32 quote_pos, u32 end, const u8* pool, u32 off, u32 len) {
-  return str_equals_pool(in, quote_pos, end, pool, off, len);
-}
 GGR_DEVN int cw_cmp_decoded(const u8* in, u32 a_pos, u32 b_pos, u32 end) { return cmp_str_tokens(in, a_pos, b_pos, end); }
 
-GGR_DEV u32 cw_funnel(u32 lo, u32 hi, u32 sh) {
-#if defined(__CUDA_ARCH__)
-  return __funnelshift_r(lo, hi, sh);
-#else
-  return sh ? (lo >> sh) | (hi << (32u - sh)) : lo;
-#endif
-}
-GGR_DEV void cw_key_info(const u8* in, u32 p, u32 n, KeyInfo* k) {
-  const u8* base = in + (p & ~3u);
-  const u32 sh = (p & 3u) * 8u;
-  u32 h = GGR_KHASH_SEED;
-  u32 w[4] = {0, 0, 0, 0};
-  const u32 nw = (n + 3u) >> 2;
-  u32 lo = ggr_ld4(base);
-  for (u32 i = 0; i < nw; i++) {
-    const u32 hi = ggr_ld4(base + 4u * (i + 1u));
-    u32 x = cw_funnel(lo, hi, sh);
-    lo = hi;
-    const u32 left = n - 4u * i;
-    if (left < 4u) x &= 0xFFFFFFFFu >> (8u * (4u - left));
-    h = khash_mix(h, x);
-    if (i == 0) w[0] = x;
-    else if (i == 1) w[1] = x;
-    else if (i == 2) w[2] = x;
-    else if (i == 3) w[3] = x;
-  }
-  k->len = n;
-  k->hash = khash_finish(h, n);
-  k->w[0] = w[0];
-  k->w[1] = w[1];
-  k->w[2] = w[2];
-  k->w[3] = w[3];
-}
-GGR_DEV bool cw_hash_lookup(const Tables& t, u32 first, u32 mask, const KeyInfo& k, const u8* in, u32 quote_pos, u32 end, i32* value) {
-  u32 slot = k.hash & mask;
-  for (u32 probes = 0; probes <= mask; probes++) {
-    const u8* ep = t.hash + (size_t)(first + slot) * 32;
-    const U4 e = ggr_ld16(ep);
-    if (e.z == 0xFFFFFFFFu) return false;
-    if (e.x == k.hash && e.z == k.len) {
-      const U4 nm = ggr_ld16(ep + 16);
-      if (nm.x == k.w[0] && nm.y == k.w[1] && nm.z == k.w[2] && nm.w == k.w[3]) {
-        if (k.len <= 16 || cw_long_name_equals(in, quote_pos, end, t.pool, e.y, k.len)) {
-          *value = (i32)e.w;
-          return true;
-        }
-      }
-    }
-    slot = (slot + 1) & mask;
-  }
-  return false;
-}
 GGR_DEVN bool cw_enum_by_name(const Tables& T, const u8* in, u32 end, i32 child, u32 pos, u32 close, i32* num) {
   KeyInfo ki;
   cw_key_info(in, pos + 1u, close - pos - 1u, &ki);
@@ -883,6 +954,43 @@
 GGR_DEV u32 cw_keypart_of(const u8* ir, u32 x) {
   const u32 klen = node_load(ir, x).y;
   return 1u + varint_size(klen) + klen;
+}
+
+GGR_DEV u32 cw_member(const Tables& T, u32 key) {
+  u32 slot = GGR_MEMBER_HASH(key) & T.member_mask;
+  for (u32 probes = 0; probes <= T.member_mask; probes++) {
+    const u32* e = reinterpret_cast<const u32*>(T.members + (size_t)slot * 8u);
+#if defined(__CUDA_ARCH__)
+    const uint2 v = __ldg(reinterpret_cast<const uint2*>(e));
+#else
+    const struct { u32 x, y; } v = {e[0], e[1]};
+#endif
+    if (v.x == key) return v.y;
+    if (v.x == 0xFFFFFFFFu) break;
+    slot = (slot + 1u) & T.member_mask;
+  }
+  return 0xFFFFFFFFu;
+}
+GGR_DEVN u32 cw_member_by_key(const u8* msgs, const u8* hash, const u8* pool, const u32* tok, const u8* qend, const u8* in, u32 end,
+                              u32 msg, u32 i) {
+  CW_NOID();
+  Tables T;
+  T.msgs = msgs;
+  T.hash = hash;
+  T.pool = pool;
+  CwIndex X;
+  X.tok = tok;
+  X.qend = qend;
+  const u32 kinf = cw_key_pack(X, i);
+  if (!(kinf >> 31)) return (CW_WHY(101), 0xFFFFFFFFu);
+  const MsgD md = ggr_msg(T, msg);
+  KeyInfo ki;
+  const u32 kpos = kinf & 0xFFFFu;
+  cw_key_info(in, kpos, (kinf >> 16) & 0x7FFFu, &ki);
+  i32 ei;
+  if (!cw_hash_lookup(T, md.key_hash_first, md.key_hash_mask, ki, in, kpos - 1u, end, &ei)) return 0xFFFFFFFFu;
+  const u32 gf = md.field_first + (u32)ei;
+  return ((u32)ei & 0xFFFFu) | ((gf < 0xFFFFu ? gf : 0xFFFFu) << 16);
 }
 
 template <class SH, bool FULL>
@@ -927,10 +1035,11 @@
   {
     const u32* recs = reinterpret_cast<const u32*>(region + rec_off);
     for (u32 r = lane; r < n_rec; r += 32) {
-      const u32 a = cw_ldg(recs + 2u * r), l = cw_ldg(recs + 2u * r + 1u) & 15u;
+      const u32 a = cw_ldg(recs + 2u * r), b = cw_ldg(recs + 2u * r + 1u), l = b & 15u;
       S.gfield[r] = (u16)a;
       S.aux[r] = (u16)(a >> 16);
       S.cls[r] = (u8)l;
+      S.ssz[r] = b >> 16;
       wp_atomic_add(&S.lvl_cur[l], 1u);
     }
   }
@@ -968,6 +1077,7 @@
     if (act) {
       S.slot[r] = (u16)pos;
       S.vtok[pos] = S.gfield[r];
+      S.body[pos] = S.ssz[r];
     }
   }
   WP_SYNC();
@@ -997,6 +1107,7 @@
       u32 emit = 0, p = 0, pc = CW_SKIP;
       if (act) {
         const u32 i = S.vtok[r];
+        const u32 nid = S.body[r];
         p = S.par[r];
         pc = S.cls[p];
         const u32 t = cw_ldg(X.tok + i);
@@ -1009,21 +1120,13 @@
         bool key_slow = false;
         bool is_ts = false;
         if (pc == CW_MSG || pc == CW_EMSG) {
-          const u32 kinf = cw_key_pack(X, i);
-          if (!(kinf >> 31)) ok = (CW_WHY(101), false);
-          const MsgD md = ggr_msg(T, S.aux[p]);
-          i32 ei = 0;
+          const u32 mf = nid != GGR_NO_NAME_ID ? cw_member(T, ((u32)S.aux[p] << 16) | nid) : cw_member_by_key(T.msgs, T.hash, T.pool, X.tok, X.qend, in, end, S.aux[p], i);
+          if (mf == 0xFFFFFFFFu) ok = false;
+          if (ok && (mf & 0xFFFFu) >= 32u) ok = (CW_WHY(102), false);
           if (ok) {
-            KeyInfo ki;
-            const u32 kpos = kinf & 0xFFFFu;
-            cw_key_info(in, kpos, (kinf >> 16) & 0x7FFFu, &ki);
-            ok = cw_hash_lookup(T, md.key_hash_first, md.key_hash_mask, ki, in, kpos - 1u, end, &ei);
-          }
-          if (ok && (u32)ei >= 32u) ok = (CW_WHY(102), false);
-          if (ok) {
-            emit = (u32)ei;
-            gf = md.field_first + emit;
-            f = ggr_field(T, gf);
+            emit = mf & 0xFFFFu;
+            gf = mf >> 16;
+            if (gf < 0xFFFFu) f = ggr_field(T, gf);
             const u32 bit = 1u << emit;
             if (wp_atomic_or(&S.ssz[p], bit) & bit) ok = (CW_WHY(103), false);
           }
@@ -1044,17 +1147,14 @@
                 cls = CW_MAP;
               } else if (f.flags & GF_REPEATED) {
                 if (k != K3_LBRACK) ok = (CW_WHY(107), false);
-                if (f.kind == GK_MESSAGE) {
-                  const u32 w = ggr_msg(T, (u32)f.child).wkt;
-                  if (w != GGR_WKT_NONE && w != GGR_WKT_TIMESTAMP) ok = (CW_WHY(108), false);
-                }
+                if (f.kind == GK_MESSAGE && (f.flags & GF_CHILD_WKT)) ok = (CW_WHY(108), false);
                 cls = (f.flags & GF_PACKED) ? CW_LISTP : CW_LIST;
                 hdr = f.tag_len;
-              } else if (f.kind == GK_MESSAGE && ggr_msg(T, (u32)f.child).wkt == GGR_WKT_TIMESTAMP) {
+              } else if (f.kind == GK_MESSAGE && (f.flags & GF_CHILD_TS)) {
                 cls = CW_LEAF;
                 is_ts = true;
               } else if (f.kind == GK_MESSAGE) {
-                if (k != K3_LBRACE || (u32)f.child >= 0xFFFFu || ggr_msg(T, (u32)f.child).wkt != GGR_WKT_NONE) ok = (CW_WHY(109), false);
+                if (k != K3_LBRACE || (u32)f.child >= 0xFFFFu || (f.flags & GF_CHILD_WKT)) ok = (CW_WHY(109), false);
                 cls = CW_MSG;
                 aux = (u32)f.child;
                 hdr = f.tag_len;
@@ -1067,7 +1167,7 @@
           gf = S.gfield[p];
           f = ggr_field(T, gf);
           in_list = true;
-          if (f.kind == GK_MESSAGE && ggr_msg(T, (u32)f.child).wkt == GGR_WKT_TIMESTAMP) {
+          if (f.kind == GK_MESSAGE && (f.flags & GF_CHILD_TS)) {
             cls = CW_LEAF;
             is_ts = true;
           } else if (f.kind == GK_MESSAGE) {
@@ -1100,7 +1200,7 @@
           }
           in_list = true;
           if (f.kind == GK_MESSAGE) {
-            if (k != K3_LBRACE || (u32)f.child >= 0xFFFFu || ggr_msg(T, (u32)f.child).wkt != GGR_WKT_NONE) ok = (CW_WHY(114), false);
+            if (k != K3_LBRACE || (u32)f.child >= 0xFFFFu || (f.flags & (GF_CHILD_TS | GF_CHILD_WKT))) ok = (CW_WHY(114), false);
             cls = CW_EMSG;
             aux = (u32)f.child;
           } else {
```
